# ChenWu98/cycle-diffusion

Hardware: AMD Instinct MI355X
Metric: images/sec, SD-v1.4 512px CycleDiffusion 100+100 steps, 1/2/4/8 MI355X (higher is better)
Workload: dtype fp16; 1 GPU; C2: Stable-Diffusion-v1.4-shaped U-Net + KL-f8 VAE, 512x512, custom_steps=99 white_box_steps=100 eta=0.1 skip 0, 1 trial, encoder scale 1, decoder CFG 3; batch_per_gpu=4, global_batch=4, parallelism=dp1, steps_per_launch_set=5, launch_set_cap=16, launch_sets_in_flight_per_gpu=1, images_in_flight_per_gpu=20, distributed=single process, weights=synthetic(seed=0)

## Files before the change

cycle-diffusion_amd/_ffi.py:

```python
import ctypes as C
import os

import numpy as np

_HERE = os.path.dirname(os.path.abspath(__file__))
LIB_PATH = os.path.join(_HERE, "lib", "libcyclediff.so")

CD_NET_UNET_OPENAI, CD_NET_UNET_HO, CD_NET_VAE_KL, CD_NET_CLIP_TEXT, CD_NET_BERT_XTR = 1, 2, 3, 4, 5
CD_NET_OCLIP_TEXT, CD_NET_OCLIP_VISION, CD_NET_INCEPTION_FID = 6, 7, 8
CD_SCHED_DDIM, CD_SCHED_DDPM = 0, 1
CD_PREC_16, CD_PREC_F32, CD_PREC_F32X3 = 0, 1, 2
CD_MASK_QSAMPLE, CD_MASK_ENCODER = 0, 1
MASK_SOURCES = {"q_sample": CD_MASK_QSAMPLE, "encoder": CD_MASK_ENCODER}
ACT_NONE, ACT_SILU, ACT_GELU, ACT_GEGLU, ACT_QGELU, ACT_RELU = 0, 1, 2, 3, 4, 5


class NetDesc(C.Structure):
    _fields_ = [
        ("kind", C.c_int), ("image_size", C.c_int), ("in_channels", C.c_int), ("out_channels", C.c_int),
        ("model_channels", C.c_int), ("num_res_blocks", C.c_int),
        ("n_mult", C.c_int), ("channel_mult", C.c_int * 8),
        ("n_attn", C.c_int), ("attn", C.c_int * 8),
        ("num_heads", C.c_int), ("num_head_channels", C.c_int),
        ("use_spatial_transformer", C.c_int), ("context_dim", C.c_int), ("transformer_depth", C.c_int),
        ("use_scale_shift_norm", C.c_int), ("resblock_updown", C.c_int), ("conv_resample", C.c_int),
        ("z_channels", C.c_int), ("embed_dim", C.c_int), ("double_z", C.c_int),
        ("precision", C.c_int), ("n_embed", C.c_int), ("reserved", C.c_int * 6),
    ]


class StepCoef(C.Structure):
    _fields_ = [("sa", C.c_float), ("s1a", C.c_float), ("sap", C.c_float), ("dirc", C.c_float),
                ("sigma", C.c_float), ("r", C.c_float), ("t_mask", C.c_float), ("t", C.c_int32)]


STEP_COEF_DTYPE = np.dtype([("sa", "<f4"), ("s1a", "<f4"), ("sap", "<f4"), ("dirc", "<f4"), ("sigma", "<f4"),
                            ("r", "<f4"), ("t_mask", "<f4"), ("t", "<i4")])

_VP, _I, _F, _U64, _SZ, _I64 = C.c_void_p, C.c_int, C.c_float, C.c_uint64, C.c_size_t, C.c_int64

SIGNATURES = {
    "cd_last_error": [],
    "cd_version": [],
    "cd_act_format": [],
    "cd_engine_create": [_VP, _SZ, C.POINTER(_VP)],
    "cd_engine_destroy": [_VP],
    "cd_engine_synchronize": [_VP],
    "cd_engine_workspace_high_water": [_VP, C.POINTER(_SZ)],
    "cd_prof_enable": [_VP, _I],
    "cd_prof_collect": [_VP, C.POINTER(_I), C.POINTER(C.c_double), C.POINTER(C.c_double)],
    "cd_net_create": [_VP, C.POINTER(NetDesc), C.POINTER(_I)],
    "cd_net_param_count": [_VP, _I, C.POINTER(_I)],
    "cd_net_param_info": [_VP, _I, _I, C.c_char_p, _I, C.POINTER(_I), C.POINTER(_I64)],
    "cd_net_load_param": [_VP, _I, C.c_char_p, _VP, _I, C.POINTER(_I64)],
    "cd_net_missing_params": [_VP, _I, C.POINTER(_I), C.c_char_p, _I],
    "cd_unet_forward": [_VP, _I, _VP, _VP, _VP, _I, _I, _VP],
    "cd_text_encode": [_VP, _I, _VP, _I, _I, _VP],
    "cd_clip_text_features": [_VP, _I, _VP, _I, _I, _VP],
    "cd_clip_image_features": [_VP, _I, _VP, _I, _VP],
    "cd_inception_features": [_VP, _I, _VP, _I, _I, _VP],
    "cd_vae_encode": [_VP, _I, _VP, _VP, _U64, _I, _I, _I, _F, _VP],
    "cd_vae_decode": [_VP, _I, _VP, _I, _I, _F, _F, _F, _VP],
    "cd_dpm_encode": [_VP, _I, _I, _VP, _VP, _VP, _I, _F, _I, _I, _VP, _VP, _U64, _I, _VP],
    "cd_ddim_decode": [_VP, _I, _I, _VP, _I, _I, _VP, _VP, _I, _F, _I, _I, _VP, _VP, _U64, _VP],
    "cd_ddim_decode_v": [_VP, _I, _I, _VP, _I, _I, _VP, _VP, _I, _VP, _I, _I, _VP, _VP, _U64, _VP],
    "cd_ddim_invert": [_VP, _I, _I, _VP, _VP, _VP, _I, _F, _I, _I, _VP, _VP, _VP],
    "cd_cycle_translate": [_VP, _I, _I, _VP, _VP, _VP, _F, _VP, _VP, _F, _VP, _I, _I, _I, _I, _VP, _VP, _VP, _U64, _I, _VP,
                           _VP],
    "cd_ddim_decode_masked": [_VP, _I, _I, _VP, _I, _I, _VP, _VP, _I, _F, _VP, _I, _I, _VP, _VP, _U64, _VP, _VP, _I, _I, _VP, _VP,
                              _U64, _VP],
    "cd_cycle_translate_masked": [_VP, _I, _I, _VP, _VP, _VP, _F, _VP, _VP, _F, _VP, _I, _I, _I, _I, _VP, _VP, _VP, _U64, _I,
                                  _VP, _VP, _I, _I, _VP, _VP, _U64, _VP, _VP],
    "cd_cycle_translate_ctrl": [_VP, _I, _I, _VP, _VP, _VP, _F, _VP, _VP, _F, _VP, _I, _I, _I, _I, _VP, _VP, _VP, _U64, _I,
                                _VP, _VP, _I, _I, _VP, _VP, _U64, _VP, _VP, _VP, _I, _I, _VP, _VP],
    "cd_ilvr_decode": [_VP, _I, _I, _VP, _I, _I, _I, _I, _VP, _VP, _U64, _VP, _I, _I, _I, _VP, _VP, _U64, _VP],
    "cd_pix_refine": [_VP, _I, _I, _VP, _I, _I, _VP, _VP, _U64],
    "cd_op_pack_conv_weight": [_VP, _VP, _I, _I, _I, _I, _I, C.POINTER(_VP), C.POINTER(_I), C.POINTER(_I)],
    "cd_op_free": [_VP, _VP],
    "cd_op_conv2d": [_VP, _VP, _I, _VP, _I, _I, _I, _I, _VP, _I, _I, _I, _I, _I, _I, _I, _VP, _VP, _VP, _I, _I, _VP],
    "cd_op_conv2d_16": [_VP, _VP, _I, _VP, _I, _I, _I, _I, _VP, _I, _I, _I, _I, _I, _I, _I, _VP, _VP, _VP, _I, _I, _VP,
                        _VP],
    "cd_op_last_gemm_config": [_VP] + [C.POINTER(_I)] * 5,
    "cd_op_up_phase_reorder": [_VP, _VP, _I, _I, _I, _I, _VP],
    "cd_op_groupnorm": [_VP, _VP, _I, _I, _I, _I, _I, _F, _VP, _VP, _VP, _I, _VP],
    "cd_op_groupnorm_ex": [_VP, _VP, _I, _I, _VP, _I, _I, _I, _I, _I, _F, _VP, _VP, _VP, _I, _I, _VP, _VP, _I, _VP],
    "cd_op_pack_conv_weight_prec": [_VP, _VP, _I, _I, _I, _I, _I, C.POINTER(_VP)],
    "cd_op_conv2d_prec": [_VP, _VP, _I, _I, _VP, _I, _I, _I, _I, _I, _VP, _I, _I, _I, _I, _I, _I, _I, _VP, _VP, _I, _VP, _I, _I,
                          _I, _I, _I, _I, _F, _VP, _VP],
    "cd_op_attention_prec": [_VP, _VP, _VP, _VP, _I, _I, _I, _I, _I, _I, _I, _I, _F, _I, _VP, _I, _I, _VP],
    "cd_op_rows_prec": [_VP, _I, _VP, _I64, _I, _I, _VP, _I, _I, _VP, _VP, _I, _VP],
    "cd_op_resample_prec": [_VP, _I, _VP, _I, _I, _I, _I, _I, _VP],
    "cd_op_layernorm": [_VP, _VP, _I, _I, _VP, _VP, _F, _VP],
    "cd_op_attention": [_VP, _VP, _VP, _VP, _I, _I, _I, _I, _I, _F, _I, _VP],
    "cd_op_cross_attention_ctrl": [_VP, _VP, _VP, _VP, _VP, _VP, _VP, _VP, _VP, _I, _I, _I, _I, _I, _I, _I, _I, _F, _VP],
    "cd_op_lowpass": [_VP, _VP, _I, _I, _I, _I, _VP],
    "cd_op_softmax_rows": [_VP, _VP, _I64, _I, _VP],
    "cd_op_timestep_embedding": [_VP, _VP, _I, _I, _I, _VP],
    "cd_op_sched_step": [_VP, _I, _I, _VP, _VP, _VP, _VP, _I, _F, _VP, _VP, _I, _I, _I, _I, _VP],
    "cd_op_sched_step_masked": [_VP, _I, _VP, _VP, _VP, _I, _F, _VP, _VP, _VP, _I, _I, _F, _F, _VP, _I, _I, _I, _I, _VP, _I],
    "cd_op_bench_conv": [_VP, _I, _I, _I, _I, _I, _I, _I, _I, _I, _I, _I, _I, C.POINTER(C.c_float)],
    "cd_op_bench_mfma_sustained": [_VP, _I, C.POINTER(C.c_float), C.POINTER(C.c_float)],
    "cd_op_probe": [_VP, _I, _VP, _VP, _SZ],
}
_RESTYPES = {"cd_last_error": C.c_char_p}

_lib = None


class EngineError(RuntimeError):
    pass


def load_library(build_if_missing=True):
    global _lib
    if _lib is not None:
        return _lib
    if not os.path.exists(LIB_PATH):
        if not build_if_missing:
            raise EngineError("libcyclediff.so has not been built: run `python -c 'import __graft_entry__ as g; g.build()'`")
        import importlib.util
        spec = importlib.util.spec_from_file_location("_cd_build", os.path.join(_HERE, "build.py"))
        mod = importlib.util.module_from_spec(spec)
        spec.loader.exec_module(mod)
        mod.build()
    os.environ.setdefault("CYCLEDIFF_TUNE_DEFAULT", os.path.join(_HERE, "tune_gfx950.txt"))
    lib = C.CDLL(os.environ.get("CYCLEDIFF_LIB") or LIB_PATH)
    for name, args in SIGNATURES.items():
        fn = getattr(lib, name)
        fn.argtypes = args
        fn.restype = _RESTYPES.get(name, C.c_int)
    _lib = lib
    return lib


def check(rc):
    if rc != 0:
        raise EngineError(load_library().cd_last_error().decode("utf-8", "replace"))


def ptr(t):
    if t is None:
        return None
    if not t.is_contiguous():
        raise EngineError("tensor crossing the C ABI must be contiguous")
    return C.c_void_p(t.data_ptr())


def coef_array(rows):
    arr = np.zeros(len(rows), dtype=STEP_COEF_DTYPE)
    for i, r in enumerate(rows):
        arr[i] = tuple(r)
    return arr
```

cycle-diffusion_amd/csrc/capi.hip:

```cpp
#include <stdlib.h>
#include <string.h>
#include <unistd.h>

#include <algorithm>

#include "engine.h"

using namespace cd;

struct StepPacer {
  static constexpr int kAhead = 2, kRing = kAhead + 1;
  hipEvent_t ev[kRing] = {nullptr, nullptr, nullptr};
  long n = 0;
  bool enabled = true;
  void init() {
    const char* e = getenv("CYCLEDIFF_HOST_PACING");
    enabled = !(e && e[0] == '0');
    for (auto& x : ev) HIP_CHECK(hipEventCreateWithFlags(&x, hipEventBlockingSync | hipEventDisableTiming));
  }
  static void sleep_until_done(hipEvent_t e) {
    for (;;) {
      const hipError_t q = hipEventQuery(e);
      if (q == hipSuccess) return;
      if (q != hipErrorNotReady) HIP_CHECK(q);
// ... 1021 lines not shown
    ConvW* pw = (ConvW*)const_cast<void*>(packed_w);
    h->op_params.add_up_phase(pw);
    h->op_params.refresh_up_phase(h->st, pw);
  }
  ConvW w = *(const ConvW*)packed_w;
  CD_CHECK(w.N == N && w.KH == KH && w.KW == KW, "packed weight does not match the call");
  w.b = const_cast<float*>(bias);
  const int c0p = x1 ? C0 : round_up(C0, 32);
  Act a0 = alloc_act(c, B, H, W, c0p);
  launch_nchw_to_nhwc(h->st, x0, a0.p, B, C0, H * W, c0p, 1.f, 0.f, 0);
  Act a1;
  if (x1) {
    a1 = alloc_act(c, B, H, W, C1);
    launch_nchw_to_nhwc(h->st, x1, a1.p, B, C1, H * W, C1, 1.f, 0.f, 0);
  }
  ConvOpts o; o.stride = stride; o.pad = pad; o.asym = asym_pad != 0; o.up = up != 0; o.tile = tile;
  if (act & 0x400) {
    CD_CHECK(out16 && conv_ln_fold_available(c, w, (int64_t)B * H * W) , "LayerNorm fold needs tile 30 shapes");
    o.ln_fold = true;
    act &= ~0x400;
  }
  o.act = act;
  o.out_f32 = !out16;
  o.want_stats = stats != nullptr;
  const int Hin = up ? 2 * H : H, Win = up ? 2 * W : W;
  const int Ho = asym_pad ? (Hin + 1 - KH) / stride + 1 : (Hin + 2 * pad - KH) / stride + 1;
  const int Wo = asym_pad ? (Win + 1 - KW) / stride + 1 : (Win + 2 * pad - KW) / stride + 1;
  const int Nout = w.geglu ? N / 2 : N;
  if (rowvec) { o.rowvec = rowvec; o.rowvec_ld = N; o.rows_per_vec = Ho * Wo; }
  Act r;
  if (resid) {
    r = alloc_act(c, B, Ho, Wo, Nout);
    launch_nchw_to_nhwc(h->st, resid, r.p, B, Nout, Ho * Wo, Nout, 1.f, 0.f, 0);
    o.resid = &r;
  }
  Act out = conv_fwd(c, w, a0, x1 ? &a1 : nullptr, o);
  launch_nhwc_to_nchw(h->st, out.p, out16 ? 0 : 1, out.ld, y, B, Nout, Ho * Wo, 1.f, 0.f);
  if (stats) {
    CD_CHECK(out.stats, "this convolution produces no GroupNorm statistics (GEGLU, or rows %% 32 != 0)");
    HIP_CHECK(hipMemcpyAsync(stats, out.stats, (size_t)(out.rows() / 32) * 2 * Nout * sizeof(float),
                             hipMemcpyDeviceToDevice, h->st));
  }
}

int cd_op_conv2d(cd_handle h, const float* x0, int C0, const float* x1, int C1, int B, int H, int W,
                 const void* packed_w, int N, int KH, int KW, int stride, int pad, int asym_pad, int up,
                 const float* bias, const float* rowvec, const float* resid, int act, int tile, float* y) {
  CD_API_BEGIN
  enter_engine(h);
  op_conv2d(h, x0, C0, x1, C1, B, H, W, packed_w, N, KH, KW, stride, pad, asym_pad, up, bias, rowvec, resid, act, tile,
            false, y, nullptr);
  CD_API_END
}

int cd_op_conv2d_16(cd_handle h, const float* x0, int C0, const float* x1, int C1, int B, int H, int W,
                    const void* packed_w, int N, int KH, int KW, int stride, int pad, int asym_pad, int up,
                    const float* bias, const float* rowvec, const float* resid, int act, int tile, float* y,
                    float* stats) {
  CD_API_BEGIN
  enter_engine(h);
  op_conv2d(h, x0, C0, x1, C1, B, H, W, packed_w, N, KH, KW, stride, pad, asym_pad, up, bias, rowvec, resid, act, tile,
            true, y, stats);
  CD_API_END
}

int cd_op_up_phase_reorder(cd_handle h, const float* x, int B, int C, int H, int W, float* y) {
  CD_API_BEGIN
  enter_engine(h);
  CD_CHECK(h && x && y && B > 0 && H > 0 && W > 0 && C > 0 && C % 8 == 0, "bad argument");
  ArenaScope arena_scope(h->arena);
  Ctx c = h->ctx();
  Act a = alloc_act(c, 4 * B, H, W, C);
  launch_nchw_to_nhwc(h->st, x, a.p, 4 * B, C, H * W, C, 1.f, 0.f, 0);
  Act o = alloc_act(c, B, 2 * H, 2 * W, C);
  launch_up_phase_reorder(h->st, a.p, o.p, B, H, W, C, o.ld);
  launch_nhwc_to_nchw(h->st, o.p, 0, o.ld, y, B, C, 4 * H * W, 1.f, 0.f);
  CD_API_END
}

int cd_op_last_gemm_config(cd_handle h, int* tile_id, int* bk, int* splitk, int* chm, int* tile_group) {
  CD_API_BEGIN
  CD_CHECK(h, "bad argument");
  const GemmLaunchInfo li = conv_gemm_last_launch();
  if (tile_id) *tile_id = li.tile_id;
  if (bk) *bk = li.bk;
  if (splitk) *splitk = li.splitk;
  if (chm) *chm = li.chm;
  if (tile_group) *tile_group = li.tile_group;
  CD_API_END
}

int cd_op_groupnorm(cd_handle h, const float* x, int B, int C, int H, int W, int G, float eps,
                    const float* gamma, const float* beta, const float* film, int silu, float* y) {
  CD_API_BEGIN
  enter_engine(h);
  CD_CHECK(h && x && y && G == 32, "bad argument (G must be 32)");
  ArenaScope arena_scope(h->arena);
  Ctx c = h->ctx();
  Act a = alloc_act(c, B, H, W, C);
  launch_nchw_to_nhwc(h->st, x, a.p, B, C, H * W, C, 1.f, 0.f, 0);
  GNW w; w.g = const_cast<float*>(gamma); w.b = const_cast<float*>(beta); w.C = C; w.eps = eps;
  Act o = groupnorm_fwd(c, w, a, nullptr, silu != 0, film, film ? 2 * C : 0);
  launch_nhwc_to_nchw(h->st, o.p, 0, o.ld, y, B, C, H * W, 1.f, 0.f);
  CD_API_END
}

int cd_op_groupnorm_ex(cd_handle h, const float* x0, int C0, int pad0, const float* x1, int C1, int pad1, int B, int H,
                       int W, float eps, const float* gamma, const float* beta, const float* film, int film_ld, int silu,
                       const float* stats0, const float* stats1, int precision, void* y) {
  CD_API_BEGIN
  enter_engine(h);
  CD_CHECK(h && x0 && gamma && beta && y && B > 0 && H > 0 && W > 0 && C0 > 0 && pad0 >= 0 && pad1 >= 0, "bad argument");
  CD_CHECK(x1 ? C1 > 0 : (C1 == 0 && !stats1), "bad argument (second source)");
  CD_CHECK(precision >= 0 && precision <= 2 && film_ld >= 0, "bad argument (precision 0 = 16-bit, 1 = fp32, 2 = fp32 split)");
  const int align = precision ? 4 : 8;
  CD_CHECK((C0 + pad0) % align == 0 && (C1 + pad1) % align == 0, "row strides must be multiples of %d elements", align);
  ArenaScope arena_scope(h->arena);
  Ctx c = h->ctx();
  c.f32 = precision != 0; c.x3 = precision == 2;
  const int HW = H * W, C = C0 + C1;
  auto upload = [&](const float* x, int Cs, int pad, const float* stats) {
    Act a; a.B = B; a.H = H; a.W = W; a.C = Cs; a.ld = Cs + pad; a.f32 = c.f32;
    a.p = (bf16_t*)h->arena.alloc((size_t)B * HW * a.ld * (c.f32 ? sizeof(float) : sizeof(bf16_t)));
    const float* src = x;
    if (pad) {
      const size_t n = (size_t)B * a.ld * HW;
      float* t = (float*)h->arena.alloc(n * sizeof(float));
      launch_fill_f32(h->st, t, __builtin_nanf(""), (int64_t)n);
      HIP_CHECK(hipMemcpy2DAsync(t, (size_t)a.ld * HW * 4, x, (size_t)Cs * HW * 4, (size_t)Cs * HW * 4, B,
                                 hipMemcpyDeviceToDevice, h->st));
      src = t;
    }
    if (c.f32) launch_nchw_to_nhwc_f32(h->st, src, a.pf(), B, a.ld, HW, a.ld, 1.f, 0.f);
    else launch_nchw_to_nhwc(h->st, src, a.p, B, a.ld, HW, a.ld, 1.f, 0.f, 0);
    a.stats = const_cast<float*>(stats);
    return a;
  };
  Act a0 = upload(x0, C0, pad0, stats0);
  Act a1;
  if (x1) a1 = upload(x1, C1, pad1, stats1);
  GNW w; w.g = const_cast<float*>(gamma); w.b = const_cast<float*>(beta); w.C = C; w.eps = eps;
  Act o = groupnorm_fwd(c, w, a0, x1 ? &a1 : nullptr, silu != 0, film, film_ld);
  if (precision == 2) {
    CD_CHECK(o.split && o.ld == 2 * C, "groupnorm: split output expected");
    HIP_CHECK(hipMemcpyAsync(y, o.p, (size_t)B * HW * 2 * C * sizeof(bf16_t), hipMemcpyDeviceToDevice, h->st));
    HIP_CHECK(hipStreamSynchronize(h->st));
    h->check_overflow();
  } else {
    launch_nhwc_to_nchw(h->st, o.p, c.f32 ? 1 : 0, o.ld, (float*)y, B, C, HW, 1.f, 0.f);
  }
  CD_API_END
}

int cd_op_layernorm(cd_handle h, const float* x, int rows, int C, const float* gamma, const float* beta,
                    float eps, float* y) {
  CD_API_BEGIN
  enter_engine(h);
  CD_CHECK(h && x && y, "bad argument");
  ArenaScope arena_scope(h->arena);
  bf16_t* a = (bf16_t*)h->arena.alloc((size_t)rows * C * 2);
  bf16_t* o = (bf16_t*)h->arena.alloc((size_t)rows * C * 2);
  launch_nchw_to_nhwc(h->st, x, a, rows, C, 1, C, 1.f, 0.f, 0);
  launch_layernorm(h->st, a, C, o, C, rows, C, gamma, beta, eps);
  launch_nhwc_to_nchw(h->st, o, 0, C, y, rows, C, 1, 1.f, 0.f);
  CD_API_END
}

int cd_op_attention(cd_handle h, const float* q, const float* k, const float* v, int B, int H, int Tq,
                    int Tk, int D, float scale, int use_transpose_kernel, float* o) {
  CD_API_BEGIN
  enter_engine(h);
  CD_CHECK(h && q && k && v && o, "bad argument");
  ArenaScope arena_scope(h->arena);
  const int C = H * D, Tpad = round_up(Tk, 64);
  bf16_t* qb = (bf16_t*)h->arena.alloc((size_t)B * Tq * C * 2);
  bf16_t* kb = (bf16_t*)h->arena.alloc((size_t)B * Tk * C * 2);
  bf16_t* vb = (bf16_t*)h->arena.alloc((size_t)B * Tk * C * 2);
  bf16_t* ob = (bf16_t*)h->arena.alloc((size_t)B * Tq * C * 2);
  launch_nchw_to_nhwc(h->st, q, qb, B * Tq, C, 1, C, 1.f, 0.f, 0);
  launch_nchw_to_nhwc(h->st, k, kb, B * Tk, C, 1, C, 1.f, 0.f, 0);
  launch_nchw_to_nhwc(h->st, v, vb, B * Tk, C, 1, C, 1.f, 0.f, 0);
  AttnParams p;
  p.q = qb; p.k = kb; p.o = ob; p.B = B; p.H = H; p.Tq = Tq; p.Tk = Tk; p.D = D;
  p.ldq = C; p.ldk = C; p.ldo = C; p.q_bs = (int64_t)Tq * C; p.k_bs = (int64_t)Tk * C; p.o_bs = (int64_t)Tq * C;
  p.scale = scale;
  if (use_transpose_kernel) {
    bf16_t* vt = (bf16_t*)h->arena.alloc((size_t)B * C * Tpad * 2);
    launch_transpose_v(h->st, vb, C, (int64_t)Tk * C, vt, B, H, Tk, D, D, Tpad);
    p.vt = vt; p.vt_dpad = D; p.vt_tpad = Tpad;
  } else {
    p.v = vb; p.ldv = C; p.v_bs = (int64_t)Tk * C;
  }
  launch_attention(h->st, p);
  launch_nhwc_to_nchw(h->st, ob, 0, C, o, B * Tq, C, 1, 1.f, 0.f);
  CD_API_END
}

int cd_op_cross_attention_ctrl(cd_handle h, const float* q_own, const float* q_src, const float* k_own, const float* k_src,
                               const float* v_own, const float* mapper, const float* alpha, const float* weight, int B,
                               int B_src, int B_ctrl, int H, int Tq, int L, int L_buf, int D, float scale, float* o) {
  CD_API_BEGIN
  enter_engine(h);
  CD_CHECK(h && q_own && q_src && k_own && k_src && v_own && mapper && alpha && weight && o, "bad argument");
  CD_CHECK(B > 0 && B_src > 0 && B_ctrl > 0 && H > 0 && Tq > 0 && D > 0 && L > 0 && L_buf >= L, "bad argument");
  ArenaScope arena_scope(h->arena);
  const int C = H * D;
  auto to16 = [&](const float* src, int64_t rows) {
    bf16_t* d = (bf16_t*)h->arena.alloc((size_t)rows * C * 2);
    launch_nchw_to_nhwc(h->st, src, d, (int)rows, C, 1, C, 1.f, 0.f, 0);
    return d;
  };
  CtrlAttnParams p;
  p.q_own = to16(q_own, (int64_t)B * Tq); p.q_src = to16(q_src, (int64_t)B_src * Tq);
  p.k_own = to16(k_own, (int64_t)B * L_buf); p.k_src = to16(k_src, (int64_t)B_src * L_buf);
  const bf16_t* vb16 = to16(v_own, (int64_t)B * L);
  bf16_t* va = (bf16_t*)h->arena.alloc((size_t)B * L * C * 2);
  bf16_t* vb = (bf16_t*)h->arena.alloc((size_t)B * L * C * 2);
  launch_ctrl_values(h->st, vb16, mapper, alpha, weight, B, B_ctrl, L, C, va, vb);
  bf16_t* ob = (bf16_t*)h->arena.alloc((size_t)B * Tq * C * 2);
  p.va = va; p.vb = vb; p.o = ob;
  p.B = B; p.B_src = B_src; p.H = H; p.Tq = Tq; p.L = L; p.D = D;
  p.ldq = C; p.ldk = C; p.ldv = C; p.ldo = C;
  p.q_bs = (int64_t)Tq * C; p.k_bs = (int64_t)L_buf * C; p.v_bs = (int64_t)L * C; p.o_bs = (int64_t)Tq * C;
  p.scale = scale;
  launch_cross_attention_ctrl(h->st, p);
  launch_nhwc_to_nchw(h->st, ob, 0, C, o, B * Tq, C, 1, 1.f, 0.f);
  CD_API_END
}

int cd_op_lowpass(cd_handle h, const float* x, int B, int C, int R, int down_n, float* y) {
  CD_API_BEGIN
  enter_engine(h);
  CD_CHECK(h && x && y && B > 0 && C > 0 && R > 0, "bad argument");
  check_lowpass_geometry(R, down_n);
  ArenaScope arena_scope(h->arena);
  const int r = R / down_n;
  IlvrArgs iv;
  iv.out = y; iv.y = x; iv.y_bmod = B;
  iv.B = B; iv.C = C; iv.R = R;
  iv.D = upload_taps(h, R, r);
  iv.U = upload_taps(h, r, R);
  iv.T = (float*)h->arena.alloc((size_t)B * C * r * r * sizeof(float));
  iv.vec4 = (R % 4 == 0 && aligned16(x) && aligned16(y)) ? 1 : 0;
  launch_ilvr_down(h->st, iv);
  launch_ilvr_up_add(h->st, iv);
  HIP_CHECK(hipStreamSynchronize(h->st));
  CD_API_END
}

int cd_op_softmax_rows(cd_handle h, const float* s, int64_t rows, int cols, float* p) {
  CD_API_BEGIN
  enter_engine(h);
  CD_CHECK(h && s && p, "bad argument");
  ArenaScope arena_scope(h->arena);
  bf16_t* pb = (bf16_t*)h->arena.alloc((size_t)rows * cols * 2);
  launch_softmax_rows(h->st, s, cols, pb, cols, rows, cols);
  launch_nhwc_to_nchw(h->st, pb, 0, cols, p, (int)rows, cols, 1, 1.f, 0.f);
  CD_API_END
}

int cd_op_timestep_embedding(cd_handle h, const float* t, int B, int dim, int mode, float* out) {
  CD_API_BEGIN
  enter_engine(h);
  CD_CHECK(h && t && out, "bad argument");
  launch_timestep_embedding(h->st, nullptr, 0, t, out, B, dim, mode);
  CD_API_END
}

int cd_op_sched_step(cd_handle h, int mode, int sched_kind, const cd_step_coef* coef_host, const float* x0,
                     float* xt, const float* eps_hat, int cfg, float guidance, const float* noise,
                     const float* eps_in, int is_last, int B, int C, int HW, float* z_slot) {
  CD_API_BEGIN
  enter_engine(h);
  CD_CHECK(h && coef_host && xt, "bad argument");
  ArenaScope arena_scope(h->arena);
  const int64_t chw = (int64_t)C * HW;
  StepArgs a;
  a.x0 = x0; a.xt = xt;
  a.eh.p = eps_hat; a.eh.sb = chw; a.eh.sc = HW; a.eh.sp = 1; a.eh.cfg = cfg; a.eh.g = guidance;
  a.geom.B = B; a.geom.C = C; a.geom.HW = HW; a.geom.tab = upload_coef(h, coef_host, 1);
  a.gauss.noise = noise;
  a.eps.p = eps_in; a.eps.bstride = chw;
  a.z.p = z_slot; a.z.bstride = chw;
  a.is_last = is_last;
  if (mode == 0) launch_init_xt(h->st, a);
  else if (mode == 1) launch_encode_step(h->st, sched_kind, a);
  else launch_decode_step(h->st, sched_kind, a);
  HIP_CHECK(hipStreamSynchronize(h->st));
  CD_API_END
}

int cd_op_sched_step_masked(cd_handle h, int mode, const cd_step_coef* coef_host, float* x, const float* eps_hat, int cfg,
                            float guidance, const float* eps_in, const float* mask, const float* src, int B_mask,
                            int mask_source, float qa, float qb, const float* mask_noise, int blend, int B, int C, int HW,
                            void* xin16_out, int cfg_dup) {
  CD_API_BEGIN
  enter_engine(h);
  CD_CHECK(h && x && mask && src && B > 0 && C > 0 && HW > 0, "bad argument");
  CD_CHECK(B_mask > 0 && B % B_mask == 0, "mask shape mismatch: %d mask rows for a batch of %d", B_mask, B);
  CD_CHECK(mode == 0 || (coef_host && eps_hat), "bad argument");
  ArenaScope arena_scope(h->arena);
  const int64_t chw = (int64_t)C * HW;
  MaskBlend mk;
  mk.mask = mask; mk.src = src; mk.mask_bmod = mk.src_bmod = B_mask; mk.gauss.noise = mask_noise;
  if (mask_source == CD_MASK_QSAMPLE) {
    CD_CHECK(mask_noise, "q_sample mode needs the noise tensor here");
// ... 412 lines not shown
```

cycle-diffusion_amd/csrc/engine.h:

```cpp
#pragma once
#include <map>
#include <memory>
#include <string>
#include <vector>

#include "common.h"
#include "kernels.h"
#include "../../include/cyclediff.h"

namespace cd {

class Arena {
 public:
  ~Arena();
  void init(size_t bytes);
  void* alloc(size_t bytes);
  size_t mark() const { return off_; }
  void release(size_t m) { off_ = m; }
  void reset() { off_ = 0; }
  size_t capacity() const { return cap_; }
  size_t high_water() const { return high_; }
 private:
  char* base_ = nullptr;
  size_t cap_ = 0, off_ = 0, high_ = 0;
};

struct Act {
  bf16_t* p = nullptr;
  int B = 0, H = 0, W = 0, C = 0;
  int ld = 0;
  bool f32 = false;
  bool split = false;
  float* pf() const { return (float*)p; }
  float* stats = nullptr;
  float* stats_buf = nullptr;
  int64_t rows() const { return (int64_t)B * H * W; }
};

struct ConvW {
  bf16_t* w = nullptr;
  bf16_t* wfrag = nullptr;
  bf16_t* w3 = nullptr;
  bf16_t* wphase = nullptr;
  int wphase_version = -1;
  bool f32 = false;
  float* b = nullptr;
  int N = 0, Cin = 0, Cpad = 0, KH = 1, KW = 1, Npad = 0;
  bool geglu = false;
  int Ktot() const { return KH * KW * Cpad; }
};

struct PackTarget {
  enum Kind { MATRIX_BF16, VECTOR_F32, MATRIX_F32 } kind;
  ConvW* conv = nullptr;
  int dst_row0 = 0, rows = 0, src_base = 0, grp = 0, grp_stride = 0;
  float* fdst = nullptr;
  int dst_off = 0, K = 1;
  bool geglu = false;
  int geglu_N = 0;
  float scale = 1.f;
};

struct ParamDecl {
  std::string name;
  std::vector<int64_t> shape;
  std::vector<PackTarget> targets;
  bool loaded = false;
  bool transposed = false;
};

class ParamStore {
 public:
  ~ParamStore();
  bool f32 = false;
  bool x3 = false;
  int* overflow = nullptr;
  int version = 0;
  ConvW* new_conv(int N, int Cin, int KH, int KW, bool bias, bool geglu = false);
  float* new_vec(int n, float init = 0.f);
  void add_up_phase(ConvW* c);
  void refresh_up_phase(hipStream_t st, ConvW* c);
  ParamDecl& declare(const std::string& name, std::vector<int64_t> shape);
  void conv_weight(const std::string& name, ConvW* c, int ref_ndim = 0, float scale = 1.f);
  void conv_weight_t(const std::string& name, ConvW* c);
  void conv_bias(const std::string& name, ConvW* c);
  void conv_rows(const std::string& name, std::vector<int64_t> shape, ConvW* c, int dst_row0, int rows,
                 int src_base, int grp, int grp_stride, float scale = 1.f);
  void bias_rows(const std::string& name, int64_t n_total, float* dst, int dst_off, int rows, int src_base,
                 int grp, int grp_stride);
  void vec(const std::string& name, float* dst, int n);
  void mat_f32(const std::string& name, float* dst, int N, int K, int dst_row0 = 0);

  void load(hipStream_t st, const std::string& name, const float* host, int ndim, const int64_t* shape);
  int missing(std::string* first = nullptr) const;
  const std::vector<std::unique_ptr<ParamDecl>>& decls() const { return decls_; }
  size_t device_bytes() const { return dev_bytes_; }
 private:
  std::vector<std::unique_ptr<ParamDecl>> decls_;
  std::map<std::string, ParamDecl*> by_name_;
  std::vector<std::unique_ptr<ConvW>> convs_;
  std::vector<void*> allocs_;
  float* staging_ = nullptr;
  size_t staging_bytes_ = 0;
  size_t dev_bytes_ = 0;
  void* dmalloc(size_t bytes);
};

struct Ctx {
  hipStream_t st = nullptr;
  Arena* arena = nullptr;
  const bf16_t* zeros = nullptr;
  float* gn_partial = nullptr;
  size_t gn_partial_floats = 0;
  bool f32 = false;
  bool x3 = false;
  int* overflow = nullptr;
};

struct ConvOpts {
  int stride = 1;
  int pad = 1;
  bool asym = false;
  bool up = false;
  const float* rowvec = nullptr; int rowvec_ld = 0; int rows_per_vec = 1;
  const Act* resid = nullptr;
  int act = ACT_NONE;
  float alpha = 1.f;
  bool out_f32 = false;
  void* out = nullptr;
  int out_ld = 0;
  bool ln_fold = false;
  float ln_eps = 1e-5f;
  bool raw_geglu = false;
  bool want_stats = false;
  float* out_stats = nullptr;
  int tile = 0;
};
Act attention_flash_f32_fwd(Ctx& c, const float* q, int ldq, const float* k, int ldk, int64_t k_bs, const float* v, int ldv,
                            int64_t v_bs, int B, int H, int Tq, int Tk, int D, float scale, int Himg, int Wimg, bool q_log2);
Act geglu_f32_fwd(Ctx& c, const Act& h);
Act split_rows_f32_fwd(Ctx& c, const Act& x, const Act* x2 = nullptr);
Act alloc_act(Ctx& c, int B, int H, int W, int C, bool with_stats = false);
Act conv_fwd(Ctx& c, const ConvW& w, const Act& x, const Act* x2, const ConvOpts& o);
bool conv_up_phase_taken(const Ctx& c, const ConvW& w, const Act& x, const Act* x2, const ConvOpts& o);
bool conv_ln_fold_available(const Ctx& c, const ConvW& w, int64_t rows);

struct GNW { float* g = nullptr; float* b = nullptr; int C = 0; float eps = 1e-5f; };
Act groupnorm_fwd(Ctx& c, const GNW& w, const Act& x, const Act* x2, bool silu, const float* film = nullptr,
                  int film_ld = 0);
struct LNW { float* g = nullptr; float* b = nullptr; int C = 0; };
Act layernorm_fwd(Ctx& c, const LNW& w, const Act& x);

Act avgpool2_fwd(Ctx& c, const Act& x);
Act upsample2_fwd(Ctx& c, const Act& x);
Act attention_f32_fwd(Ctx& c, const Act& qk, const Act& v, int H, int D, float scale, const float* obias);

Act attention_fwd(Ctx& c, const bf16_t* q, int ldq, const bf16_t* k, int ldk, const bf16_t* v, int ldv, int B,
                  int H, int Tq, int Tk, int D, float scale, int Himg, int Wimg, bool q_log2 = false);
Act attention_vt_fwd(Ctx& c, const bf16_t* q, int ldq, const bf16_t* k, int ldk, const bf16_t* vt, int B,
                     int H, int Tq, int Tk, int Tpad, int D, float scale, int Himg, int Wimg, bool q_log2 = false);

class Net {
 public:
  virtual ~Net() {}
  ParamStore params;
  cd_net_desc desc;
  bool f32 = false;
  bool x3 = false;
  virtual int kind() const = 0;
};

struct TimeEmb {
  int mode = 0, dim = 0, hidden = 0;
  float *w0 = nullptr, *b0 = nullptr, *w1 = nullptr, *b1 = nullptr;
  float* proj_w = nullptr; float* proj_b = nullptr;
  int proj_total = 0;
};

struct AttnCtrl {
  std::vector<const bf16_t*> va, vb;
  int row0 = 0, rows = 0;
  int src_b0 = 0, B_src = 0;
};

struct UNetIO {
  const bf16_t* xin = nullptr;
  int B = 0;
  const StepCoef* tab = nullptr; int step = 0;
  const float* t_explicit = nullptr;
  bool t_shared = true;
  bool cfg_dup = false;
  int dup_tail = 0;
  const AttnCtrl* ctrl = nullptr;
  float* out = nullptr;
  int out_ld = 0;
};

class UNet : public Net {
 public:
  virtual void forward(Ctx& c, const UNetIO& io) = 0;
  virtual void set_context(Ctx& c, const bf16_t* ctx, int B, int L) { (void)c; (void)ctx; (void)B; (void)L; }
  virtual void build_attn_control(Ctx&, const float*, const float*, const float*, int, AttnCtrl&) {
    CD_CHECK(false, "cross-attention control: the network has no text cross-attention");
  }
  int in_cpad = 32;
  int out_channels = 0;
  int image_size = 0;
  virtual size_t workspace_hint(int B) const = 0;
};

std::unique_ptr<UNet> make_unet_openai(const cd_net_desc& d);
std::unique_ptr<UNet> make_unet_ho(const cd_net_desc& d);

class VAE : public Net {
 public:
  int kind() const override { return CD_NET_VAE_KL; }
  virtual void encode_moments(Ctx& c, const bf16_t* img_nhwc, int B, int R, float* moments) = 0;
  virtual void decode(Ctx& c, const bf16_t* z_nhwc, int B, int h, float* img) = 0;
  int z_channels = 4, factor = 8;
  int moments_channels = 8;
  const float* codebook = nullptr;
  int n_embed = 0;
};
std::unique_ptr<VAE> make_vae_kl(const cd_net_desc& d);

class TextEncoder : public Net {
 public:
  virtual void encode(Ctx& c, const int* ids_dev, int B, int L, float* out) = 0;
  virtual void text_features(Ctx&, const int*, int, int, float*) { CD_CHECK(false, "net has no pooled text features"); }
  virtual void image_features(Ctx&, const float*, int, float*) { CD_CHECK(false, "net has no image tower"); }
  virtual int width() const = 0;
  virtual int max_positions() const = 0;
};
std::unique_ptr<TextEncoder> make_clip_text(const cd_net_desc& d);

std::unique_ptr<Net> make_inception_fid(const cd_net_desc& d);
void inception_fid_features(Net* n, Ctx& c, const float* img, int B, int stop_block, float* out);

}
```

cycle-diffusion_amd/csrc/engine.hip:

```cpp
#include <stdlib.h>

#include "engine.h"

#include <string.h>

namespace cd {

Arena::~Arena() { if (base_) (void)hipFree(base_); }
void Arena::init(size_t bytes) {
  if (base_) { (void)hipFree(base_); base_ = nullptr; }
  HIP_CHECK(hipMalloc((void**)&base_, bytes));
  cap_ = bytes; off_ = 0; high_ = 0;
}
void* Arena::alloc(size_t bytes) {
  size_t a = (off_ + 255) & ~(size_t)255;
  CD_CHECK(a + bytes <= cap_, "workspace arena exhausted: need %zu more bytes (capacity %zu); "
           "create the engine with a larger workspace", a + bytes - cap_, cap_);
  off_ = a + bytes;
  if (off_ > high_) high_ = off_;
  return base_ + a;
}

ParamStore::~ParamStore() {
  for (void* p : allocs_) (void)hipFree(p);
  if (staging_) (void)hipFree(staging_);
}
void* ParamStore::dmalloc(size_t bytes) {
  void* p = nullptr;
  HIP_CHECK(hipMalloc(&p, bytes < 256 ? 256 : bytes));
  HIP_CHECK(hipMemset(p, 0, bytes < 256 ? 256 : bytes));
  allocs_.push_back(p);
  dev_bytes_ += bytes;
  return p;
}
ConvW* ParamStore::new_conv(int N, int Cin, int KH, int KW, bool bias, bool geglu) {
  convs_.emplace_back(new ConvW());
  ConvW* c = convs_.back().get();
  c->N = N; c->Cin = Cin; c->KH = KH; c->KW = KW; c->geglu = geglu;
  c->Cpad = round_up(Cin, 32);
  c->Npad = round_up(N, 128);
  c->f32 = f32;
  c->w = (bf16_t*)dmalloc((size_t)c->Npad * c->Ktot() * (f32 ? sizeof(float) : sizeof(bf16_t)));
  if (!f32 && KH == 1 && KW == 1 && c->Cpad == 320)
    c->wfrag = (bf16_t*)dmalloc((size_t)c->Npad * c->Cpad * sizeof(bf16_t));
  if (f32 && x3) c->w3 = (bf16_t*)dmalloc((size_t)c->Npad * c->Ktot() * 3 * sizeof(bf16_t));
  if (bias) c->b = (float*)dmalloc((size_t)c->Npad * sizeof(float));
  return c;
}
void ParamStore::add_up_phase(ConvW* c) {
  if (f32 || c->wphase || c->KH != 3 || c->KW != 3 || c->geglu) return;
  c->wphase = (bf16_t*)dmalloc((size_t)4 * c->Npad * 4 * c->Cpad * sizeof(bf16_t));
  c->wphase_version = -1;
}
void ParamStore::refresh_up_phase(hipStream_t st, ConvW* c) {
  if (!c->wphase || c->wphase_version == version) return;
  launch_up_phase_weights(st, c->w, c->wphase, c->Npad, c->Cpad);
  c->wphase_version = version;
}
float* ParamStore::new_vec(int n, float init) {
  float* p = (float*)dmalloc((size_t)n * sizeof(float));
  if (init != 0.f) {
    std::vector<float> h(n, init);
    HIP_CHECK(hipMemcpy(p, h.data(), (size_t)n * sizeof(float), hipMemcpyHostToDevice));
  }
  return p;
}
ParamDecl& ParamStore::declare(const std::string& name, std::vector<int64_t> shape) {
  auto it = by_name_.find(name);
  if (it != by_name_.end()) {
    CD_CHECK(it->second->shape == shape, "parameter %s declared twice with different shapes", name.c_str());
    return *it->second;
  }
  decls_.emplace_back(new ParamDecl());
  ParamDecl* d = decls_.back().get();
  d->name = name; d->shape = std::move(shape);
  by_name_[name] = d;
  return *d;
}
void ParamStore::conv_weight(const std::string& name, ConvW* c, int ref_ndim, float scale) {
  std::vector<int64_t> shape;
  if (ref_ndim == 0) ref_ndim = (c->KH == 1 && c->KW == 1) ? 2 : 4;
  if (ref_ndim == 2) shape = {c->N, c->Cin};
  else if (ref_ndim == 3) shape = {c->N, c->Cin, 1};
  else shape = {c->N, c->Cin, c->KH, c->KW};
  ParamDecl& d = declare(name, shape);
  PackTarget t; t.kind = PackTarget::MATRIX_BF16; t.conv = c; t.dst_row0 = 0; t.rows = c->N;
  t.src_base = 0; t.grp = c->N; t.grp_stride = 0; t.geglu = c->geglu; t.scale = scale;
  d.targets.push_back(t);
}
void ParamStore::conv_weight_t(const std::string& name, ConvW* c) {
  CD_CHECK(c->KH == 1 && c->KW == 1, "transposed weights are linear layers");
  ParamDecl& d = declare(name, {c->Cin, c->N});
  d.transposed = true;
  PackTarget t; t.kind = PackTarget::MATRIX_BF16; t.conv = c; t.dst_row0 = 0; t.rows = c->N;
  t.src_base = 0; t.grp = c->N; t.grp_stride = 0; t.geglu = false;
  d.targets.push_back(t);
}
void ParamStore::conv_bias(const std::string& name, ConvW* c) {
  CD_CHECK(c->b, "conv %s has no bias storage", name.c_str());
  ParamDecl& d = declare(name, {c->N});
  PackTarget t; t.kind = PackTarget::VECTOR_F32; t.fdst = c->b; t.dst_off = 0; t.rows = c->N;
  t.src_base = 0; t.grp = c->N; t.grp_stride = 0; t.geglu = c->geglu; t.geglu_N = c->N;
  d.targets.push_back(t);
}
void ParamStore::conv_rows(const std::string& name, std::vector<int64_t> shape, ConvW* c, int dst_row0,
                           int rows, int src_base, int grp, int grp_stride, float scale) {
  ParamDecl& d = declare(name, std::move(shape));
  PackTarget t; t.kind = PackTarget::MATRIX_BF16; t.conv = c; t.dst_row0 = dst_row0; t.rows = rows;
  t.src_base = src_base; t.grp = grp; t.grp_stride = grp_stride; t.scale = scale;
  d.targets.push_back(t);
}
void ParamStore::bias_rows(const std::string& name, int64_t n_total, float* dst, int dst_off, int rows,
                           int src_base, int grp, int grp_stride) {
  ParamDecl& d = declare(name, {n_total});
  PackTarget t; t.kind = PackTarget::VECTOR_F32; t.fdst = dst; t.dst_off = dst_off; t.rows = rows;
  t.src_base = src_base; t.grp = grp; t.grp_stride = grp_stride;
  d.targets.push_back(t);
}
void ParamStore::vec(const std::string& name, float* dst, int n) {
  bias_rows(name, n, dst, 0, n, 0, n, 0);
}
void ParamStore::mat_f32(const std::string& name, float* dst, int N, int K, int dst_row0) {
  ParamDecl& d = declare(name, {N, K});
  PackTarget t; t.kind = PackTarget::MATRIX_F32; t.fdst = dst; t.dst_off = dst_row0; t.rows = N; t.K = K;
  t.src_base = 0; t.grp = N; t.grp_stride = 0;
  d.targets.push_back(t);
}

template <typename OutT>
__global__ void k_pack_rows(const float* __restrict__ w, OutT* __restrict__ out, int rows, int Cin,
                            int KH, int KW, int Cpad, int dst_row0, int src_base, int grp,
                            int grp_stride, int geglu, int Ntot, float scale) {
  const int64_t total = (int64_t)rows * KH * KW * Cpad;
  for (int64_t i = blockIdx.x * (int64_t)blockDim.x + threadIdx.x; i < total;
       i += (int64_t)gridDim.x * blockDim.x) {
    const int c = (int)(i % Cpad);
    int64_t t = i / Cpad;
    const int s = (int)(t % KW); t /= KW;
    const int r = (int)(t % KH); t /= KH;
    const int j = (int)t;
    int jj = j;
    if (geglu) {
      const int blk = j / 64, within = j % 64;
      jj = (within < 32) ? blk * 32 + within : Ntot / 2 + blk * 32 + (within - 32);
    }
    const int src = src_base + (jj / grp) * grp_stride + (jj % grp);
    float v = 0.f;
    if (c < Cin) v = w[(((int64_t)src * Cin + c) * KH + r) * KW + s] * scale;
    const int64_t o = ((int64_t)(dst_row0 + j) * KH * KW + (int64_t)r * KW + s) * Cpad + c;
    if constexpr (sizeof(OutT) == 4) out[o] = v;
    else out[o] = f2bf(v);
  }
}
// ... 9 lines not shown
  for (auto s : d.shape) nd *= s;
  bool ok = (n == nd) && ndim >= 1 && shape[0] == d.shape[0];
  if (ok && d.shape.size() >= 2 && ndim >= 2) ok = (shape[1] == d.shape[1]);
  CD_CHECK(ok, "parameter %s: shape mismatch (got %lld elements, ndim %d; expected %lld)", name.c_str(),
           (long long)n, ndim, (long long)nd);
  const size_t bytes = (size_t)n * sizeof(float);
  if (bytes > staging_bytes_) {
    if (staging_) HIP_CHECK(hipFree(staging_));
    staging_bytes_ = bytes < (1u << 20) ? (1u << 20) : bytes;
    HIP_CHECK(hipMalloc((void**)&staging_, staging_bytes_));
  }
  HIP_CHECK(hipStreamSynchronize(st));
  if (d.transposed) {
    const int64_t K = d.shape[0], N = d.shape[1];
    std::vector<float> tr((size_t)n);
    for (int64_t k = 0; k < K; ++k)
      for (int64_t j = 0; j < N; ++j) tr[(size_t)j * K + k] = host[(size_t)k * N + j];
    HIP_CHECK(hipMemcpy(staging_, tr.data(), bytes, hipMemcpyHostToDevice));
  } else {
    HIP_CHECK(hipMemcpy(staging_, host, bytes, hipMemcpyHostToDevice));
  }
  for (const PackTarget& t : d.targets) {
    if (t.kind == PackTarget::MATRIX_BF16) {
      const ConvW* c = t.conv;
      const int64_t total = (int64_t)t.rows * c->KH * c->KW * c->Cpad;
      int grid = (int)((total + 255) / 256);
      if (grid > 8192) grid = 8192;
      if (c->f32)
        hipLaunchKernelGGL(k_pack_rows<float>, dim3(grid), dim3(256), 0, st, staging_, (float*)c->w, t.rows, c->Cin,
                           c->KH, c->KW, c->Cpad, t.dst_row0, t.src_base, t.grp, t.grp_stride, t.geglu ? 1 : 0, c->N,
                           t.scale);
      else
        hipLaunchKernelGGL(k_pack_rows<bf16_t>, dim3(grid), dim3(256), 0, st, staging_, c->w, t.rows, c->Cin, c->KH,
                           c->KW, c->Cpad, t.dst_row0, t.src_base, t.grp, t.grp_stride, t.geglu ? 1 : 0, c->N, t.scale);
      if (c->wfrag) launch_pack_wfrag(st, c->w, c->Ktot(), c->wfrag, c->Npad);
      if (c->w3) launch_pack_w3(st, (const float*)c->w, c->w3, c->Npad, c->KH * c->KW, c->Cpad, overflow);
    } else {
      const int K = (t.kind == PackTarget::MATRIX_F32) ? t.K : 1;
      std::vector<float> tmp((size_t)t.rows * K);
      for (int j = 0; j < t.rows; ++j) {
        int jj = j;
        if (t.geglu) {
          const int blk = j / 64, within = j % 64;
          jj = (within < 32) ? blk * 32 + within : t.geglu_N / 2 + blk * 32 + (within - 32);
        }
        const int src = t.src_base + (jj / t.grp) * t.grp_stride + (jj % t.grp);
        memcpy(&tmp[(size_t)j * K], host + (size_t)src * K, (size_t)K * sizeof(float));
      }
      HIP_CHECK(hipMemcpy(t.fdst + (size_t)t.dst_off * K, tmp.data(), tmp.size() * sizeof(float),
                          hipMemcpyHostToDevice));
    }
  }
  HIP_CHECK(hipStreamSynchronize(st));
  d.loaded = true;
}

int ParamStore::missing(std::string* first) const {
  int n = 0;
  for (auto& d : decls_)
    if (!d->loaded) {
      if (n == 0 && first) *first = d->name;
      ++n;
    }
  return n;
}

Act alloc_act(Ctx& c, int B, int H, int W, int C, bool with_stats) {
  Act a; a.B = B; a.H = H; a.W = W; a.C = C; a.ld = C; a.f32 = c.f32;
  a.p = (bf16_t*)c.arena->alloc((size_t)B * H * W * C * (c.f32 ? sizeof(float) : sizeof(bf16_t)));
  if ((!c.f32 || c.x3) && with_stats && ((H * W) % 32) == 0)
    a.stats_buf = (float*)c.arena->alloc((size_t)(B * H * W / 32) * 2 * C * sizeof(float));
  return a;
}

static Act conv_split_fwd(Ctx& c, const ConvW& w, const Act& x, const ConvOpts& o) {
  CD_CHECK(c.f32 && c.x3 && w.w3 && (!w.geglu || o.raw_geglu), "conv: split input outside the split-fp16 mode");
  CD_CHECK(x.C == w.Cpad && x.ld == 2 * x.C, "conv: split input of %d channels (ld %d) against Cpad %d", x.C, x.ld, w.Cpad);
  CD_CHECK(!o.ln_fold && (!o.resid || (o.resid->f32 && !o.resid->split)), "conv: split-mode operands");
  ConvGemmParams p;
  p.src0 = x.p; p.C0 = 2 * x.C; p.ld0 = x.ld;
  p.src1 = x.p; p.C1 = x.C; p.ld1 = x.ld;
  p.B = x.B; p.Hs = x.H; p.Ws = x.W; p.up = o.up ? 1 : 0;
  p.Hin = o.up ? x.H * 2 : x.H; p.Win = o.up ? x.W * 2 : x.W;
  p.KH = w.KH; p.KW = w.KW; p.stride = o.stride;
  if (o.asym) { p.pad_t = 0; p.pad_l = 0; p.Hout = (p.Hin + 1 - w.KH) / o.stride + 1; p.Wout = (p.Win + 1 - w.KW) / o.stride + 1; }
  else {
    p.pad_t = o.pad; p.pad_l = o.pad;
    p.Hout = (p.Hin + 2 * o.pad - w.KH) / o.stride + 1;
    p.Wout = (p.Win + 2 * o.pad - w.KW) / o.stride + 1;
  }
  p.M = x.B * p.Hout * p.Wout;
  p.wgt = w.w3; p.Ktot = 3 * w.Ktot(); p.N = w.N;
  p.alpha = o.alpha * (1.0f / (kX3ActScale * kX3WgtScale)); p.bias = w.b;
  p.rowvec = o.rowvec; p.rowvec_ld = o.rowvec_ld; p.rows_per_vec = o.rows_per_vec;
  p.act = o.act;
  Act y; y.B = x.B; y.H = p.Hout; y.W = p.Wout; y.C = w.N; y.f32 = true;
  if (o.out) { y.p = (bf16_t*)o.out; y.ld = o.out_ld; }
  else { y.ld = w.N; y.p = (bf16_t*)c.arena->alloc((size_t)p.M * w.N * 4); }
  if (o.resid) {
    CD_CHECK(o.resid->rows() == p.M && o.resid->C == w.N, "conv: residual shape mismatch");
    p.resid = o.resid->p; p.resid_ld = o.resid->ld; p.resid_f32 = 1;
  }
  p.out = y.p; p.out_ld = y.ld; p.out_f32 = 1;
  p.zeros = c.zeros; p.tile = o.tile;
  p.prof_flop_scale = 1.0f / 3.0f;
  if (((p.Hout * p.Wout) % 32) == 0) {
    if (o.out && o.out_stats) y.stats_buf = o.out_stats;
    else if (!o.out && o.want_stats)
      y.stats_buf = (float*)c.arena->alloc((size_t)(p.M / 32) * 2 * w.N * sizeof(float));
    p.stats = y.stats_buf;
    y.stats = y.stats_buf;
  }
  launch_conv_gemm(c.st, p);
  return y;
}

bool conv_up_phase_taken(const Ctx& c, const ConvW& w, const Act& x, const Act* x2, const ConvOpts& o) {
  if (!o.up || c.f32 || x.split || x2 || !w.wphase || w.KH != 3 || w.KW != 3 || o.stride != 1 || o.pad != 1 || o.asym ||
      o.resid || o.out_f32 || o.ln_fold || w.geglu || o.act != ACT_NONE)
    return false;
  if ((x.H * x.W) % 256 != 0 || w.N % 8 != 0 || (o.out && o.out_ld % 8 != 0)) return false;
  const char* e = getenv("CYCLEDIFF_UP_PHASE");
  return !(e && e[0] == '0');
}

static Act conv_up_phase_fwd(Ctx& c, const ConvW& w, const Act& x, const ConvOpts& o) {
  ConvGemmParams p;
  p.src0 = x.p; p.C0 = round_up(x.C, 32); p.ld0 = x.ld;
  CD_CHECK(p.C0 == w.Cpad && x.ld >= p.C0, "conv: input channels %d do not match weight Cpad %d", p.C0, w.Cpad);
  p.B = x.B; p.Hs = x.H; p.Ws = x.W; p.Hin = x.H; p.Win = x.W; p.Hout = x.H; p.Wout = x.W;
  p.KH = 2; p.KW = 2; p.stride = 1; p.pad_t = 1; p.pad_l = 1;
  p.up_phase = 1; p.w_ps = w.Npad * 4 * w.Cpad;
  p.M = 4 * x.B * x.H * x.W;
  p.wgt = w.wphase; p.Ktot = 4 * w.Cpad; p.N = w.N;
  p.alpha = o.alpha; p.bias = w.b;
  p.rowvec = o.rowvec; p.rowvec_ld = o.rowvec_ld; p.rows_per_vec = o.rows_per_vec;
  Act y; y.B = x.B; y.H = 2 * x.H; y.W = 2 * x.W; y.C = w.N; y.f32 = false;
  if (o.out) { y.p = (bf16_t*)o.out; y.ld = o.out_ld; }
  else { y.ld = w.N; y.p = (bf16_t*)c.arena->alloc((size_t)p.M * w.N * 2); }
  if (o.out && o.out_stats) y.stats_buf = o.out_stats;
  else if (!o.out && o.want_stats) y.stats_buf = (float*)c.arena->alloc((size_t)(p.M / 32) * 2 * w.N * sizeof(float));
  p.stats = y.stats_buf;
  y.stats = y.stats_buf;
  const size_t mk = c.arena->mark();
  bf16_t* tmp = (bf16_t*)c.arena->alloc((size_t)p.M * w.N * 2);
  p.out = tmp; p.out_ld = w.N;
  p.zeros = c.zeros; p.tile = o.tile;
  launch_conv_gemm(c.st, p);
  launch_up_phase_reorder(c.st, tmp, y.p, x.B, x.H, x.W, w.N, y.ld);
  c.arena->release(mk);
  return y;
}

Act conv_fwd(Ctx& c, const ConvW& w, const Act& x, const Act* x2, const ConvOpts& o) {
  if (conv_up_phase_taken(c, w, x, x2, o)) return conv_up_phase_fwd(c, w, x, o);
  if (x.split) {
    CD_CHECK(!x2, "conv: a split activation cannot be concatenated");
    return conv_split_fwd(c, w, x, o);
  }
  ConvGemmParams p;
  CD_CHECK(w.f32 == c.f32 && x.f32 == c.f32 && (!x2 || x2->f32 == c.f32) && (!o.resid || o.resid->f32 == c.f32),
           "conv: operand precision does not match the running network");
  CD_CHECK((!x2 || !x2->split) && (!o.resid || !o.resid->split), "conv: split activation as a second source / residual");
  p.src0 = x.p; p.C0 = round_up(x.C, 32); p.ld0 = x.ld;
  if (x2) {
    CD_CHECK(x2->B == x.B && x2->H == x.H && x2->W == x.W, "conv: concat sources differ in shape");
    p.src1 = x2->p; p.C1 = x2->C; p.ld1 = x2->ld;
    CD_CHECK(x.C % 32 == 0 && x2->C % 32 == 0, "conv: concat channels must be multiples of 32");
  }
  CD_CHECK(p.C0 + p.C1 == w.Cpad, "conv: input channels %d+%d do not match weight Cpad %d", p.C0, p.C1, w.Cpad);
  CD_CHECK(x.ld >= p.C0, "conv: source row shorter than padded channel count");
  p.B = x.B; p.Hs = x.H; p.Ws = x.W; p.up = o.up ? 1 : 0;
  p.Hin = o.up ? x.H * 2 : x.H; p.Win = o.up ? x.W * 2 : x.W;
  p.KH = w.KH; p.KW = w.KW; p.stride = o.stride;
  if (o.asym) { p.pad_t = 0; p.pad_l = 0; p.Hout = (p.Hin + 1 - w.KH) / o.stride + 1; p.Wout = (p.Win + 1 - w.KW) / o.stride + 1; }
  else {
    p.pad_t = o.pad; p.pad_l = o.pad;
    p.Hout = (p.Hin + 2 * o.pad - w.KH) / o.stride + 1;
    p.Wout = (p.Win + 2 * o.pad - w.KW) / o.stride + 1;
  }
  p.M = x.B * p.Hout * p.Wout;
  p.wgt = w.w; p.wgt_frag = w.wfrag; p.Ktot = w.Ktot(); p.N = w.N;
  p.alpha = o.alpha; p.bias = w.b;
  p.rowvec = o.rowvec; p.rowvec_ld = o.rowvec_ld; p.rows_per_vec = o.rows_per_vec;
  const bool fuse_geglu = w.geglu && !o.raw_geglu;
  p.act = fuse_geglu ? ACT_GEGLU : o.act;
  const int Nout = fuse_geglu ? w.N / 2 : w.N;
  Act y; y.B = x.B; y.H = p.Hout; y.W = p.Wout; y.C = Nout; y.f32 = c.f32;
  if (o.out) { y.p = (bf16_t*)o.out; y.ld = o.out_ld; }
  else {
    y.ld = Nout;
    y.p = (bf16_t*)c.arena->alloc((size_t)p.M * Nout * ((o.out_f32 || c.f32) ? 4 : 2));
  }
  if (o.resid) {
    CD_CHECK(o.resid->rows() == p.M && o.resid->C == Nout, "conv: residual shape mismatch");
    p.resid = o.resid->p; p.resid_ld = o.resid->ld;
  }
  p.out = y.p; p.out_ld = y.ld; p.out_f32 = o.out_f32 ? 1 : 0;
  p.zeros = c.zeros; p.tile = o.tile;
  if (o.ln_fold) { p.ln_fold = 1; p.ln_eps = o.ln_eps; p.tile = kLinStreamTile; }
  if (c.f32) {
    p.out_f32 = 1;
    launch_conv_gemm_f32(c.st, p);
    return y;
  }
  if (!w.geglu && !o.out_f32 && ((p.Hout * p.Wout) % 32) == 0) {
    if (o.out && o.out_stats) y.stats_buf = o.out_stats;
    else if (!o.out && o.want_stats)
      y.stats_buf = (float*)c.arena->alloc((size_t)(p.M / 32) * 2 * Nout * sizeof(float));
    p.stats = y.stats_buf;
    y.stats = y.stats_buf;
  }
  launch_conv_gemm(c.st, p);
  return y;
}

bool conv_ln_fold_available(const Ctx& c, const ConvW& w, int64_t rows) {
  static const bool on = [] { const char* e = getenv("CYCLEDIFF_LN_FOLD"); return !(e && e[0] == '0'); }();
  static const int64_t min_rows = [] { const char* e = getenv("CYCLEDIFF_LN_FOLD_MIN_ROWS"); return e ? atoll(e) : 32768ll; }();
  return on && !c.f32 && w.wfrag && w.KH == 1 && w.KW == 1 && w.Cpad == 320 && rows >= min_rows && rows % 32 == 0 &&
         w.N % 64 == 0 && w.N <= 2560;
}

Act groupnorm_fwd(Ctx& c, const GNW& w, const Act& x, const Act* x2, bool silu, const float* film,
                  int film_ld) {
  GroupNormParams p;
  p.x = x.p; p.C0 = x.C; p.ld0 = x.ld;
  if (x2) { p.x1 = x2->p; p.C1 = x2->C; p.ld1 = x2->ld; }
  const int C = p.C0 + p.C1;
  CD_CHECK(C == w.C, "groupnorm: channels %d != weight %d", C, w.C);
  p.B = x.B; p.HW = x.H * x.W; p.G = 32; p.eps = w.eps; p.gamma = w.g; p.beta = w.b;
  p.film = film; p.film_ld = film_ld; p.silu = silu ? 1 : 0;
  Act y = alloc_act(c, x.B, x.H, x.W, C);
  p.y = y.p;
  if (c.f32) {
    CD_CHECK(x.f32 && (!x2 || x2->f32) && !x.split && (!x2 || !x2->split), "groupnorm: operand precision");
    if (c.x3) { p.split_out = 1; p.overflow = c.overflow; y.split = true; y.ld = 2 * C; }
    if (x.stats && x.ld == x.C && (!x2 || (x2->stats && x2->ld == x2->C))) {
      p.pre0 = x.stats;
      p.pre1 = x2 ? x2->stats : nullptr;
    }
    const size_t mk = c.arena->mark();
    void* ws = c.arena->alloc(groupnorm_f32_workspace(p.B, p.HW, C));
    launch_groupnorm_f32(c.st, p, ws);
    c.arena->release(mk);
    return y;
  }
  p.S = groupnorm_slabs(p.B, p.HW, C);
  const size_t part_floats = round_up((size_t)p.B * p.S * p.G * 2, (size_t)64);
  CD_CHECK(part_floats + (size_t)p.B * 2 * C <= c.gn_partial_floats, "groupnorm: workspace too small");
  p.partial = c.gn_partial;
  p.coef = c.gn_partial + part_floats;
  if (x.stats && x.ld == x.C && (!x2 || (x2->stats && x2->ld == x2->C))) {
    p.pre0 = x.stats;
    p.pre1 = x2 ? x2->stats : nullptr;
  }
  launch_groupnorm(c.st, p);
  return y;
}

Act avgpool2_fwd(Ctx& c, const Act& x) {
  if (x.split) {
    Act y = alloc_act(c, x.B, x.H / 2, x.W / 2, x.C);
    y.split = true; y.ld = 2 * x.C;
    launch_avgpool2_split(c.st, x.p, y.p, x.B, x.H, x.W, x.C, c.overflow);
    return y;
  }
  CD_CHECK(x.ld == x.C, "avgpool: dense input expected");
  Act y = alloc_act(c, x.B, x.H / 2, x.W / 2, x.C);
  if (c.f32) launch_avgpool2_f32(c.st, x.pf(), y.pf(), x.B, x.H, x.W, x.C);
  else launch_avgpool2(c.st, x.p, y.p, x.B, x.H, x.W, x.C);
  return y;
}
Act upsample2_fwd(Ctx& c, const Act& x) {
  CD_CHECK(x.ld == x.C && !x.split, "upsample: dense input expected");
  Act y = alloc_act(c, x.B, x.H * 2, x.W * 2, x.C);
  if (c.f32) launch_upsample2_f32(c.st, x.pf(), y.pf(), x.B, x.H, x.W, x.C);
  else launch_upsample2(c.st, x.p, y.p, x.B, x.H, x.W, x.C);
  return y;
}
Act attention_f32_fwd(Ctx& c, const Act& qk, const Act& v, int H, int D, float scale, const float* obias) {
  CD_CHECK(c.f32 && qk.f32 && v.f32 && !qk.split && !v.split && qk.C == 2 * H * D && v.C == H * D,
           "attention_f32: operands");
  Act o = alloc_act(c, qk.B, qk.H, qk.W, H * D);
  const int T = qk.H * qk.W;
  if (D <= 160 && (D % 4) == 0 && (qk.ld % 4) == 0 && (v.ld % 4) == 0) {
    launch_flash_f32(c.st, qk.pf(), qk.ld, (int64_t)T * qk.ld, qk.pf() + H * D, qk.ld, (int64_t)T * qk.ld, v.pf(), v.ld,
                     (int64_t)T * v.ld, o.pf(), o.ld, (int64_t)T * o.ld, qk.B, H, T, T, D, scale * 1.44269504088896340736f, 0,
                     c.overflow, obias);
    return o;
  }
  launch_attention_f32(c.st, qk.pf(), qk.ld, qk.pf() + H * D, qk.ld, v.pf(), v.ld, o.pf(), o.ld, qk.B, H, T, D, scale, obias);
  return o;
}

Act layernorm_fwd(Ctx& c, const LNW& w, const Act& x) {
  CD_CHECK(x.C == w.C, "layernorm: channels");
  if (c.f32) {
    CD_CHECK(x.f32 && !x.split, "layernorm_f32: operand precision");
    Act y = alloc_act(c, x.B, x.H, x.W, x.C);
    if (c.x3) { y.split = true; y.ld = 2 * x.C; }
    launch_layernorm_f32(c.st, x.pf(), x.ld, y.pf(), x.rows(), x.C, w.g, w.b, 1e-5f, c.x3 ? 1 : 0, c.overflow);
    return y;
  }
  Act y = alloc_act(c, x.B, x.H, x.W, x.C);
  launch_layernorm(c.st, x.p, x.ld, y.p, y.ld, (int)x.rows(), x.C, w.g, w.b, 1e-5f);
  return y;
}

Act attention_fwd(Ctx& c, const bf16_t* q, int ldq, const bf16_t* k, int ldk, const bf16_t* v, int ldv, int B,
                  int H, int Tq, int Tk, int D, float scale, int Himg, int Wimg, bool q_log2) {
  CD_CHECK(!c.f32, "attention: 16-bit kernel called on the fp32 path");
  Act o = alloc_act(c, B, Himg, Wimg, H * D);
  AttnParams p;
  p.q = q; p.k = k; p.v = v; p.o = o.p;
  p.B = B; p.H = H; p.Tq = Tq; p.Tk = Tk; p.D = D;
  p.ldq = ldq; p.ldk = ldk; p.ldv = ldv; p.ldo = o.ld;
  p.q_bs = (int64_t)Tq * ldq; p.k_bs = (int64_t)Tk * ldk; p.v_bs = (int64_t)Tk * ldv; p.o_bs = (int64_t)Tq * o.ld;
  p.scale = scale; p.q_log2 = q_log2 ? 1 : 0;
  launch_attention(c.st, p);
  return o;
}

Act attention_vt_fwd(Ctx& c, const bf16_t* q, int ldq, const bf16_t* k, int ldk, const bf16_t* vt, int B,
                     int H, int Tq, int Tk, int Tpad, int D, float scale, int Himg, int Wimg, bool q_log2) {
  CD_CHECK(!c.f32, "attention: 16-bit kernel called on the fp32 path");
  Act o = alloc_act(c, B, Himg, Wimg, H * D);
  AttnParams p;
  p.q = q; p.k = k; p.vt = vt; p.o = o.p;
  p.B = B; p.H = H; p.Tq = Tq; p.Tk = Tk; p.D = D;
  p.ldq = ldq; p.ldk = ldk; p.ldo = o.ld;
  p.q_bs = (int64_t)Tq * ldq; p.k_bs = (int64_t)Tk * ldk; p.o_bs = (int64_t)Tq * o.ld;
  p.vt_dpad = D; p.vt_tpad = Tpad;
  p.scale = scale; p.q_log2 = q_log2 ? 1 : 0;
  launch_attention(c.st, p);
  return o;
}

Act attention_flash_f32_fwd(Ctx& c, const float* q, int ldq, const float* k, int ldk, int64_t k_bs, const float* v, int ldv,
                            int64_t v_bs, int B, int H, int Tq, int Tk, int D, float scale, int Himg, int Wimg, bool q_log2) {
  CD_CHECK(c.f32, "attention_flash_f32: fp32 path only");
  Act o = alloc_act(c, B, Himg, Wimg, H * D);
  launch_flash_f32(c.st, q, ldq, (int64_t)Tq * ldq, k, ldk, k_bs, v, ldv, v_bs, o.pf(), o.ld, (int64_t)Tq * o.ld, B, H, Tq,
                   Tk, D, q_log2 ? 1.0f : scale * 1.44269504088896340736f, c.x3 ? 1 : 0, c.overflow);
  if (c.x3) { o.split = true; o.ld = 2 * o.C; }
  return o;
}

Act geglu_f32_fwd(Ctx& c, const Act& h) {
  CD_CHECK(c.f32 && h.f32 && !h.split && h.ld == h.C && (h.C % 64) == 0, "geglu_f32: operand");
  Act y = alloc_act(c, h.B, h.H, h.W, h.C / 2);
  launch_geglu_f32(c.st, h.pf(), y.pf(), h.rows(), h.C / 2, c.x3 ? 1 : 0, c.overflow);
  if (c.x3) { y.split = true; y.ld = 2 * y.C; }
  return y;
}

Act split_rows_f32_fwd(Ctx& c, const Act& x, const Act* x2) {
  CD_CHECK(c.f32 && c.x3 && x.f32 && !x.split && (!x2 || (x2->f32 && !x2->split && x2->rows() == x.rows())),
           "split_rows_f32: operand");
  const int C = x.C + (x2 ? x2->C : 0);
  Act y = alloc_act(c, x.B, x.H, x.W, C);
  launch_split_rows_f32(c.st, x.pf(), x.ld, x.C, x2 ? x2->pf() : nullptr, x2 ? x2->ld : 4, x2 ? x2->C : 0, y.p, x.rows(),
                        c.overflow);
  y.split = true; y.ld = 2 * C;
  return y;
}

}
```

cycle-diffusion_amd/csrc/kernels.h:

```cpp
#pragma once
#include <map>
#include <string>
#include <vector>

#include "common.h"

namespace cd {

struct StepCoef {
  float sa, s1a, sap, dirc, sigma, r, t_mask;
  int t;
};
enum { SCHED_DDIM = 0, SCHED_DDPM = 1 };

struct EpsHat {
  const float* p = nullptr;
  int64_t sb = 0, sc = 0, sp = 0;
  int cfg = 0;
  float g = 1.f;
  const float* gvec = nullptr;
};

struct StepGeom {
  int B = 0, C = 0, HW = 0;
  const StepCoef* tab = nullptr;
  int step = 0;
};
struct GaussSrc {
  const float* noise = nullptr;
  uint64_t seed = 0;
  uint32_t stream = 0;
};
struct XinOut {
  bf16_t* xin = nullptr;
  int cpad = 0;
  int dup = 0;
};
struct EpsIn {
  const float* p = nullptr;
  int64_t bstride = 0;
  int bmod = 0;
};
struct ZSlot {
  float* p = nullptr;
  int64_t bstride = 0;
};
struct StepArgs {
  const float* x0 = nullptr;
  float* xt = nullptr;
  EpsHat eh;
  StepGeom geom;
  GaussSrc gauss;
  XinOut xin;
  EpsIn eps;
  ZSlot z;
  int is_last = 0;
};

struct MaskBlend {
  const float* mask = nullptr;
  const float* src = nullptr;
  int mask_bmod = 1, src_bmod = 1;
  const float2* qtab = nullptr;
  int qrow = 0;
  GaussSrc gauss;
};

void launch_init_xt(hipStream_t st, const StepArgs& a);
void launch_encode_step(hipStream_t st, int kind, const StepArgs& a);
void launch_decode_step(hipStream_t st, int kind, const StepArgs& a, const MaskBlend* mk = nullptr, bool blend = false);
void launch_mask_blend_init(hipStream_t st, const StepArgs& a, const MaskBlend& mk);

struct LowpassTaps {
  const float* w = nullptr;
  const int* first = nullptr;
  int n_out = 0, n_in = 0, P = 0;
};
struct IlvrArgs {
  const float* xp = nullptr;
  float* out = nullptr;
  const float* y = nullptr;
  int y_bmod = 1;
  const float2* qtab = nullptr;
  int qrow = 0;
  GaussSrc gauss;
  float* T = nullptr;
  int B = 0, C = 0, R = 0;
  LowpassTaps D, U;
  XinOut xin;
  int vec4 = 0;
};
constexpr int kIlvrMaxR = 1024;
void build_lowpass_taps(int n_in, int n_out, std::vector<float>& w, std::vector<int>& first, int& P);
void launch_ilvr_down(hipStream_t st, const IlvrArgs& a);
void launch_ilvr_up_add(hipStream_t st, const IlvrArgs& a);

enum { ACT_NONE = 0, ACT_SILU = 1, ACT_GELU = 2, ACT_GEGLU = 3, ACT_QGELU = 4, ACT_RELU = 5 };

struct ConvGemmParams {
  const bf16_t* src0 = nullptr;
  const bf16_t* src1 = nullptr;
  int C0 = 0, C1 = 0;
  int ld0 = 0, ld1 = 0;
  int B = 1, Hs = 1, Ws = 1;
  int up = 0;
  int Hin = 1, Win = 1;
  int KH = 1, KW = 1, stride = 1, pad_t = 0, pad_l = 0;
  int Hout = 1, Wout = 1;
  int M = 0;
  const bf16_t* wgt = nullptr;
  const bf16_t* wgt_frag = nullptr;
  int Ktot = 0, N = 0;
  int ldw = 0;
  int nbatch = 1;
  int64_t a_bs = 0, w_bs = 0, o_bs = 0;
  float alpha = 1.0f;
  const float* bias = nullptr;
  const float* rowvec = nullptr;
  int rowvec_ld = 0, rows_per_vec = 1;
  const bf16_t* resid = nullptr;
  int resid_ld = 0;
  int resid_f32 = 0;
  int act = ACT_NONE;
  void* out = nullptr;
  int out_ld = 0;
  int out_f32 = 0;
  float* stats = nullptr;
  const bf16_t* zeros = nullptr;
  int ln_fold = 0;
  float ln_eps = 1e-5f;
  int tile = 0;
  float prof_flop_scale = 1.f;
  int splitk = 0;
  float* sk_scratch = nullptr;
  int* sk_flags = nullptr;
  unsigned long long* probe = nullptr;
  int korder = 1;
  int tile_group = 0;
  int dephase_ticks = 0;
  int num_cus = 256;
  int dbg = 0;
  int up_phase = 0;
  int w_ps = 0;
};
constexpr int kProbeWords = 48;
extern thread_local unsigned long long* g_conv_probe;
struct SplitKWorkspace {
  float* scratch = nullptr;
  size_t scratch_bytes = 0;
  int* flags = nullptr;
  int nflags = 0;
};
extern thread_local SplitKWorkspace g_conv_splitk;
void launch_conv_gemm(hipStream_t st, const ConvGemmParams& p);
const char* conv_gemm_last_config();
struct GemmLaunchInfo {
  int tile_id = 0;
  int bk = 0;
  int splitk = 1;
  int chm = 0;
  int tile_group = 0;
};
GemmLaunchInfo conv_gemm_last_launch();
void launch_up_phase_weights(hipStream_t st, const bf16_t* w, bf16_t* out, int Npad, int Cpad);
int conv_gemm_num_configs();
const char* conv_gemm_config_name(int id);

struct LinStreamParams {
  const bf16_t* a = nullptr; int lda = 0;
  const bf16_t* wfrag = nullptr;
  const float* bias = nullptr;
  const bf16_t* resid = nullptr; int ldr = 0;
  bf16_t* out = nullptr; int ldo = 0;
  float* stats = nullptr;
  int M = 0, N = 0;
  float ln_eps = 1e-5f;
  int geglu_direct = 0;
};
constexpr int kLinStreamTile = 30;
bool lin_stream_supports(const ConvGemmParams& p);
void launch_lin_stream(hipStream_t st, const ConvGemmParams& p);
void launch_fold_ln(hipStream_t st, const bf16_t* w, int ldw, const float* gamma, const float* beta, const float* bias,
                    bf16_t* w_out, float* bias_out, int N, int Kc);
void launch_pack_wfrag(hipStream_t st, const bf16_t* w, int ldw, bf16_t* out, int N);

struct KernelProfiler {
  bool enabled = false;
  std::vector<hipEvent_t> events;
  std::vector<double> flops;
  std::vector<std::string> labels;
  int used = 0;
  bool verbose = false;
  struct Entry { int n = 0; double ms = 0, flops = 0; };
  std::map<std::string, Entry> per_shape;
  void next_pair(hipEvent_t* a, hipEvent_t* b, double fl, const std::string& what);
  void collect(int* launches, double* total_ms, double* total_flops);
  ~KernelProfiler();
};
extern thread_local KernelProfiler* g_conv_prof;

struct ConvTuner {
  bool enabled = false;
  void* scratch = nullptr;
  size_t scratch_bytes = 0;
  int shapes_tuned = 0;
};
extern ConvTuner g_conv_tuner;

void launch_repack_weight(hipStream_t st, const float* w, bf16_t* out, int N, int Cin, int KH,
                          int KW, int Npad, int Cpad, int geglu, int64_t src_row_offset);

struct GroupNormParams {
  const bf16_t* x = nullptr;
  const bf16_t* x1 = nullptr;
  int C0 = 0, C1 = 0, ld0 = 0, ld1 = 0;
  int B = 0, HW = 0, G = 32;
  float eps = 1e-5f;
  const float* gamma = nullptr;
  const float* beta = nullptr;
  const float* film = nullptr;
  int film_ld = 0;
  int silu = 0;
  int split_out = 0;
  int* overflow = nullptr;
  bf16_t* y = nullptr;
  float* partial = nullptr;
  int S = 0;
  float* coef = nullptr;
  const float* pre0 = nullptr;
  const float* pre1 = nullptr;
};
int groupnorm_slabs(int B, int HW, int C);
void launch_groupnorm(hipStream_t st, const GroupNormParams& p);

void launch_layernorm(hipStream_t st, const bf16_t* x, int ldx, bf16_t* y, int ldy, int rows,
                      int C, const float* gamma, const float* beta, float eps);
void launch_softmax_rows(hipStream_t st, const float* s, int lds, bf16_t* p, int ldp, int64_t rows,
                         int cols);

struct AttnParams {
  const bf16_t* q = nullptr;
  const bf16_t* k = nullptr;
  const bf16_t* v = nullptr;
  const bf16_t* vt = nullptr;
  int ldv = 0; int64_t v_bs = 0;
  bf16_t* o = nullptr;
  int B = 0, H = 0, Tq = 0, Tk = 0, D = 0;
  int ldq = 0, ldk = 0, ldo = 0;
  int64_t q_bs = 0, k_bs = 0, o_bs = 0;
  int vt_dpad = 0, vt_tpad = 0;
  float scale = 1.0f;
  int q_log2 = 0;
  const float* obias = nullptr;
  int causal = 0;
};
void launch_attention(hipStream_t st, const AttnParams& p);
constexpr int kCtrlKeys = 96;
struct CtrlAttnParams {
  const bf16_t* q_own = nullptr;
  const bf16_t* q_src = nullptr;
  const bf16_t* k_own = nullptr;
  const bf16_t* k_src = nullptr;
  const bf16_t* va = nullptr;
  const bf16_t* vb = nullptr;
  bf16_t* o = nullptr;
  int B = 0, B_src = 0, H = 0, Tq = 0, L = 0, D = 0;
  int ldq = 0, ldk = 0, ldv = 0, ldo = 0;
  int64_t q_bs = 0, k_bs = 0, v_bs = 0, o_bs = 0;
  float scale = 1.0f;
  int q_log2 = 0;
};
void launch_cross_attention_ctrl(hipStream_t st, const CtrlAttnParams& p);
void launch_ctrl_values(hipStream_t st, const bf16_t* v, const float* M, const float* alpha, const float* w, int rows,
                        int B_ctrl, int L, int C, bf16_t* va, bf16_t* vb);
void launch_transpose_v(hipStream_t st, const bf16_t* v, int ldv, int64_t v_bs, bf16_t* vt, int B,
                        int H, int Tk, int D, int Dpad, int Tpad);

void launch_mfma_sustained(hipStream_t st, int target_ms, float* tflops, float* ghz);

void launch_nchw_to_nhwc(hipStream_t st, const float* x, bf16_t* y, int B, int C, int HW, int Cpad,
                         float scale, float shift, int dup);
void launch_nhwc_to_nchw(hipStream_t st, const void* x, int x_f32, int ldx, float* y, int B, int C,
                         int HW, float scale, float shift);
void launch_timestep_embedding(hipStream_t st, const StepCoef* tab, int step, const float* t_explicit,
                               float* out, int B, int dim, int mode);
void launch_vec_linear(hipStream_t st, const float* x, int ldx, const float* W, const float* bias,
                       float* y, int ldy, int B, int K, int N, int silu_in, int silu_out);
void launch_avgpool2(hipStream_t st, const bf16_t* x, bf16_t* y, int B, int H, int W, int C);
void launch_upsample2(hipStream_t st, const bf16_t* x, bf16_t* y, int B, int H, int W, int C);
void launch_up_phase_reorder(hipStream_t st, const bf16_t* x, bf16_t* y, int B, int H, int W, int C, int ldy);
void launch_posterior_sample(hipStream_t st, const float* mom, int ld, const float* noise,
                             uint64_t seed, float* z, int B, int zc, int HW, float scale,
                             int use_mean);
void launch_vq_quantize(hipStream_t st, const float* z, float in_mul, const float* codebook, int n_embed, int zc,
                        int B, int HW, bf16_t* out, int Cpad);
void launch_fill_f32(hipStream_t st, float* p, float v, int64_t n);
void launch_vit_tokens(hipStream_t st, const bf16_t* patch, const float* cls, const float* pos, bf16_t* out, int B,
                       int T, int D);
void launch_gather_eot(hipStream_t st, const bf16_t* x, const int* ids, bf16_t* out, int B, int L, int D);
void launch_embed_tokens(hipStream_t st, const int* ids, const float* tok, const float* pos, bf16_t* out, int B,
                         int L, int D, int vocab);
void launch_conv_gemm_f32(hipStream_t st, const ConvGemmParams& p);
size_t groupnorm_f32_workspace(int B, int HW, int C);
void launch_groupnorm_f32(hipStream_t st, const GroupNormParams& p, void* workspace);
void launch_attention_f32(hipStream_t st, const float* q, int ldq, const float* k, int ldk, const float* v, int ldv,
                          float* o, int ldo, int B, int H, int T, int D, float scale, const float* obias);
void launch_nchw_to_nhwc_f32(hipStream_t st, const float* x, float* y, int B, int C, int HW, int Cpad, float scale,
                             float shift, int split = 0, int* overflow = nullptr);
void launch_avgpool2_f32(hipStream_t st, const float* x, float* y, int B, int H, int W, int C);
void launch_flash_f32(hipStream_t st, const float* q, int ldq, int64_t q_bs, const float* k, int ldk, int64_t k_bs,
                      const float* v, int ldv, int64_t v_bs, float* o, int ldo, int64_t o_bs, int B, int H, int Tq, int Tk,
                      int D, float qmul, int split, int* overflow, const float* obias = nullptr);
void launch_layernorm_f32(hipStream_t st, const float* x, int ldx, float* y, int64_t rows, int C, const float* gamma,
                          const float* beta, float eps, int split, int* overflow);
void launch_geglu_f32(hipStream_t st, const float* h, float* y, int64_t rows, int Nout, int split, int* overflow);
void launch_split_rows_f32(hipStream_t st, const float* x0, int ld0, int C0, const float* x1, int ld1, int C1, bf16_t* y,
                           int64_t rows, int* overflow);
void launch_upsample2_f32(hipStream_t st, const float* x, float* y, int B, int H, int W, int C);
constexpr float kX3ActScale = 16.f;
constexpr float kX3WgtScale = 256.f;
void launch_pack_w3(hipStream_t st, const float* w, bf16_t* w3, int Npad, int taps, int Cpad, int* overflow);
void launch_avgpool2_split(hipStream_t st, const bf16_t* x, bf16_t* y, int B, int H, int W, int C, int* overflow);

void launch_copy_strided_bf16(hipStream_t st, const bf16_t* src, int lds, bf16_t* dst, int ldd,
                              int64_t rows, int cols);

}
```

cycle-diffusion_amd/csrc/lin_stream.hip:

```cpp
#include <stdlib.h>

#include <mutex>

#include "common.h"
#include "kernels.h"

namespace cd {
namespace lin_detail {

typedef __attribute__((address_space(3))) void* lptr_t;
typedef __attribute__((ext_vector_type(4))) unsigned int u32x4;

constexpr int K = 320, NKS = K / 16, KSH = NKS / 2;
constexpr int WPIECE = 2 * KSH * 1024, WSLOTS = 3;
constexpr int APIECE = 128 * 128, ASLOTS = 3;
constexpr int NAP = 10;
constexpr int ST_LD = 36, ST_BYTES = 32 * ST_LD * 4;
constexpr int BIAS_MAX = 2560;
constexpr int OFF_A = WSLOTS * WPIECE, OFF_ST = OFF_A + ASLOTS * APIECE, OFF_BIAS = OFF_ST + 8 * ST_BYTES;
constexpr int LDS_BYTES = OFF_BIAS + BIAS_MAX * 4;
static_assert(LDS_BYTES <= 160 * 1024, "LDS");
constexpr unsigned kNoLoad = 0x80000000u;
constexpr int kGegluDirectDefault = 1;

__device__ __forceinline__ void wait_vmcnt_le(int n) {
  n = n < 0 ? 0 : (n > 60 ? 60 : n);
  switch (n >> 2) {
    case 0: asm volatile("s_waitcnt vmcnt(0)" ::: "memory"); break;
    case 1: asm volatile("s_waitcnt vmcnt(4)" ::: "memory"); break;
    case 2: asm volatile("s_waitcnt vmcnt(8)" ::: "memory"); break;
    case 3: asm volatile("s_waitcnt vmcnt(12)" ::: "memory"); break;
    case 4: asm volatile("s_waitcnt vmcnt(16)" ::: "memory"); break;
    case 5: asm volatile("s_waitcnt vmcnt(20)" ::: "memory"); break;
    case 6: asm volatile("s_waitcnt vmcnt(24)" ::: "memory"); break;
    case 7: asm volatile("s_waitcnt vmcnt(28)" ::: "memory"); break;
    case 8: asm volatile("s_waitcnt vmcnt(32)" ::: "memory"); break;
    case 9: asm volatile("s_waitcnt vmcnt(36)" ::: "memory"); break;
    case 10: asm volatile("s_waitcnt vmcnt(40)" ::: "memory"); break;
    case 11: asm volatile("s_waitcnt vmcnt(44)" ::: "memory"); break;
    case 12: asm volatile("s_waitcnt vmcnt(48)" ::: "memory"); break;
    case 13: asm volatile("s_waitcnt vmcnt(52)" ::: "memory"); break;
    case 14: asm volatile("s_waitcnt vmcnt(56)" ::: "memory"); break;
    default: asm volatile("s_waitcnt vmcnt(60)" ::: "memory"); break;
  }
}

__device__ __forceinline__ u32x4 load16_hidden(u32x4 rsrc, unsigned voff) {
  u32x4 r;
  asm volatile("buffer_load_dwordx4 %0, %1, %2, 0 offen" : "=v"(r) : "v"(voff), "s"(rsrc) : "memory");
  return r;
}
__device__ __forceinline__ uint4 pack8_sat(const float* f) {
#if CD_ACT_FP16
  typedef __attribute__((ext_vector_type(2))) _Float16 h2;
  uint32_t w[4];
#pragma unroll
  for (int i = 0; i < 4; ++i) {
    const h2 v = {(_Float16)__builtin_amdgcn_fmed3f(f[2 * i], -65504.0f, 65504.0f),
                  (_Float16)__builtin_amdgcn_fmed3f(f[2 * i + 1], -65504.0f, 65504.0f)};
    w[i] = __builtin_bit_cast(uint32_t, v);
  }
  return make_uint4(w[0], w[1], w[2], w[3]);
#else
  return pack8(f);
#endif
}
__device__ __forceinline__ void touch4(u32x4& a, u32x4& b, u32x4& c, u32x4& d) {
  asm volatile("" : "+v"(a), "+v"(b), "+v"(c), "+v"(d)::"memory");
}

template <int ACT, bool RESID, bool STATS, bool LNF = false>
__global__ __launch_bounds__(512, 2) void k_lin_stream(LinStreamParams p) {
#if defined(__HIP_DEVICE_COMPILE__)
  constexpr bool GEGLU = (ACT == ACT_GEGLU);
  static_assert(!(GEGLU && (RESID || STATS)), "GEGLU has neither residual nor statistics");
  extern __shared__ __attribute__((aligned(16))) char smem[];
  char* wring = smem;
  char* aring = smem + OFF_A;
  const int tid = threadIdx.x, lane = tid & 63;
  const int wave = __builtin_amdgcn_readfirstlane(tid >> 6);
  float* stage = (float*)(smem + OFF_ST + wave * ST_BYTES);
  float* bias_s = (float*)(smem + OFF_BIAS);
  const int mi = lane & 31, half = lane >> 5;
  const bool w_issuer = wave < 4;
  const int wq = wave & 3;

  const int NT = p.N >> 6;
  const int I = 2 * NT;
  const int nstrips = (p.M + 255) >> 8;
  const int G = gridDim.x;
  const int my_count = (nstrips - (int)blockIdx.x + G - 1) / G;
  if (my_count <= 0) return;
  const int cs = I >= 80 ? 4 : (I >= 40 ? 2 : 1);

  const __amdgpu_buffer_rsrc_t rs_a =
      __builtin_amdgcn_make_buffer_rsrc((void*)p.a, 0, (unsigned)((size_t)p.M * p.lda * 2), 0x00020000);
  const __amdgpu_buffer_rsrc_t rs_w =
      __builtin_amdgcn_make_buffer_rsrc((void*)p.wfrag, 0, (unsigned)((size_t)p.N * K * 2), 0x00020000);
  const __amdgpu_buffer_rsrc_t rs_o = __builtin_amdgcn_make_buffer_rsrc(
      (void*)p.out, 0, (unsigned)((size_t)p.M * p.ldo * 2), 0x00020000);
  u32x4 rs_r = {0u, 0u, 0u, 0x00020000u};
  if (RESID) {
    const uint64_t ra = (uint64_t)p.resid;
    rs_r[0] = (unsigned)ra; rs_r[1] = (unsigned)(ra >> 32) & 0xffffu;
    rs_r[2] = (unsigned)((size_t)p.M * p.ldr * 2);
  }

  for (int i = tid; i < p.N; i += 512) bias_s[i] = p.bias ? p.bias[i] : 0.f;

  auto issue_a = [&](int row0, int j, int slot) {
    const unsigned a_row = (unsigned)((lane >> 3) * p.lda * 2);
#pragma unroll
    for (int u = 0; u < 4; ++u) {
      const int x = wq * 4 + u;
      const unsigned a_lane = a_row + (unsigned)(((lane & 7) ^ ((4 * u + (lane >> 4)) & 7)) * 16);
      const unsigned base = (unsigned)(((row0 + 128 * (j & 1) + 8 * x) * p.lda + (j >> 1) * 64) * 2);
      __builtin_amdgcn_raw_ptr_buffer_load_lds(rs_a, (lptr_t)(aring + slot * APIECE + x * 1024), 16, a_lane + base, 0,
                                               0, 0);
    }
  };
  int w_boff[5];
#pragma unroll
  for (int u = 0; u < 5; ++u) {
    const int x = wq + 4 * u;
    w_boff[u] = ((x / KSH) * NKS + (x % KSH)) * 1024;
  }
  auto issue_w = [&](int piece, bool valid, int slot) {
    const int base = ((piece >> 1) * 2 * NKS + (piece & 1) * KSH) * 1024;
    const unsigned voff = valid ? (unsigned)(lane * 16) : kNoLoad;
#pragma unroll
    for (int u = 0; u < 5; ++u)
      __builtin_amdgcn_raw_ptr_buffer_load_lds(rs_w, (lptr_t)(wring + slot * WPIECE + (wq + 4 * u) * 1024), 16, voff,
                                               base + w_boff[u], 0, 0);
  };

  bf16x8 af[NKS], afn[NKS];
  auto normalise_rows = [&]() __attribute__((always_inline)) {
    float s1 = 0.f, s2 = 0.f;
#pragma unroll
    for (int ks = 0; ks < NKS; ++ks) {
      float f[8];
      unpack8(__builtin_bit_cast(uint4, af[ks]), f);
#pragma unroll
      for (int e = 0; e < 8; ++e) { s1 += f[e]; s2 = __builtin_fmaf(f[e], f[e], s2); }
      __builtin_amdgcn_sched_barrier(0);
    }
    s1 += __shfl_xor(s1, 32);
    s2 += __shfl_xor(s2, 32);
    const float mean = s1 * (1.0f / K);
    const float var = fmaxf(s2 * (1.0f / K) - mean * mean, 0.f);
    const float rstd = __builtin_amdgcn_rsqf(var + p.ln_eps);
    const float nmr = -mean * rstd;
#pragma unroll
    for (int ks = 0; ks < NKS; ++ks) {
      float f[8];
      unpack8(__builtin_bit_cast(uint4, af[ks]), f);
#pragma unroll
      for (int e = 0; e < 8; ++e) f[e] = __builtin_fmaf(f[e], rstd, nmr);
      af[ks] = __builtin_bit_cast(bf16x8, pack8_sat(f));
      __builtin_amdgcn_sched_barrier(0);
    }
  };
  auto take_a = [&](int j, int slot) {
    if ((j & 1) != (wave >> 2)) return;
    const int row = wq * 32 + mi;
    const int sw = (row >> 1) & 7;
    unsigned base = (unsigned)(OFF_A + slot * APIECE + row * 128 + ((half ^ sw) << 4));
    asm volatile("" : "+v"(base));
    const int kb = j >> 1;
#pragma unroll
    for (int c = 0; c < 5; ++c) {
      if (kb == c) {
#pragma unroll
        for (int f = 0; f < 4; ++f) afn[4 * c + f] = *(const bf16x8*)(smem + (base ^ (unsigned)(32 * f)));
        asm volatile("" ::: "memory");
      }
    }
  };

  int seq = 0;
  int wm0 = 0, wm1 = 0;
  int am0 = 0, am1 = 0, a_fly = 0;
  int rmark = 0;

  int e_issue = 0, e_cons = 0;
  int is_o = 0, is_j = 0, is_gi = -NAP - 2;
  int is_slot = 0, is_row0 = (int)blockIdx.x * 256;
  int cn_o = 0, cn_j = 0, cn_gi = -NAP, cn_slot = 0;
  auto a_step_issue = [&](int gi) {
    if (is_o < my_count && is_gi <= gi) {
      if (!w_issuer) {
        issue_a(is_row0, is_j, is_slot);
        seq += 4;
        am0 = a_fly == 0 ? seq : am0;
        am1 = a_fly == 0 ? am1 : seq;
      }
      const bool wrap = is_j == NAP - 1;
      const int step_in = is_o == 0 ? 1 : cs, step_wrap = is_o == 0 ? I - 12 * cs + 3 : I - 9 * cs;
      ++a_fly;
      ++e_issue;
      is_slot = is_slot == ASLOTS - 1 ? 0 : is_slot + 1;
      is_gi += wrap ? step_wrap : step_in;
      is_j = wrap ? 0 : is_j + 1;
      is_o += wrap ? 1 : 0;
      is_row0 += wrap ? G * 256 : 0;
    }
  };
  auto a_due = [&](int gi) { return e_cons < e_issue && cn_gi <= gi; };
  int ce_j = 0, ce_slot = 0;
  auto a_consume_step = [&]() {
    const bool wrap = cn_j == NAP - 1;
    const int step_in = cn_o == 0 ? 1 : cs, step_wrap = cn_o == 0 ? I - 10 * cs + 1 : I - 9 * cs;
    ce_j = cn_j; ce_slot = cn_slot;
    am0 = am1; --a_fly; ++e_cons;
    cn_slot = cn_slot == ASLOTS - 1 ? 0 : cn_slot + 1;
    cn_gi += wrap ? step_wrap : step_in;
    cn_j = wrap ? 0 : cn_j + 1;
    cn_o += wrap ? 1 : 0;
  };

  if (w_issuer) {
    issue_w(0, true, 0); seq += 5; wm0 = seq;
    issue_w(1, true, 1); seq += 5; wm1 = seq;
  }
  a_step_issue(-NAP - 2);
  a_step_issue(-NAP - 1);
  for (int gi = -NAP; gi < 0; ++gi) {
    const bool due = a_due(gi);
    if (due && !w_issuer) wait_vmcnt_le(seq - am0);
    asm volatile("s_waitcnt lgkmcnt(0)\n\ts_barrier" ::: "memory");
    if (due) a_consume_step();
    a_step_issue(gi);
    if (due) take_a(ce_j, ce_slot);
  }
#pragma unroll
  for (int ks = 0; ks < NKS; ++ks) af[ks] = afn[ks];
  if (LNF) normalise_rows();

  f32x16 acc[2];
  u32x4 rres[4];
  auto issue_resid = [&](int row0, int t) {
    if (!RESID || row0 + wave * 32 >= p.M) return;
    int l2 = lane;
    asm volatile("" : "+v"(l2));
    const unsigned r_lane = (unsigned)(((wave * 32 + (l2 >> 2)) * p.ldr + (l2 & 3) * 8) * 2);
#pragma unroll
    for (int nb = 0; nb < 2; ++nb)
#pragma unroll
      for (int ps = 0; ps < 2; ++ps) {
        const int soff = ((row0 + 16 * ps) * p.ldr + t * 64 + nb * 32) * 2;
        asm volatile("buffer_load_dwordx4 %0, %1, %2, %3 offen"
                     : "=v"(rres[nb * 2 + ps]) : "v"(r_lane), "s"(rs_r), "s"(soff) : "memory");
      }
    seq += 4;
    rmark = seq;
  };
  issue_resid((int)blockIdx.x * 256, 0);

  int gi = 0;
  int wslot = 0;
  for (int ord = 0; ord < my_count; ++ord) {
    const int row0 = ((int)blockIdx.x + ord * G) * 256;
    const bool has_next = ord + 1 < my_count;
    const bool rows_ok = row0 + wave * 32 < p.M;
    for (int t = 0; t < NT; ++t) {
#pragma unroll
      for (int r = 0; r < 16; ++r) { acc[0][r] = 0.f; acc[1][r] = 0.f; }
#pragma unroll
      for (int kh = 0; kh < 2; ++kh) {
        const int i = 2 * t + kh;
        if (w_issuer) wait_vmcnt_le(seq - wm0);
        const bool due = a_due(gi);
        if (due && !w_issuer) wait_vmcnt_le(seq - am0);
        asm volatile("s_waitcnt lgkmcnt(0)\n\ts_barrier" ::: "memory");
        if (w_issuer) {
          const int nxt = i + 2;
          const int slot2 = wslot == 0 ? 2 : wslot - 1;
          issue_w(nxt < I ? nxt : nxt - I, nxt < I || has_next, slot2);
          seq += 5;
          wm0 = wm1; wm1 = seq;
        }
        if (due) a_consume_step();
        a_step_issue(gi);
        const char* wp = wring + wslot * WPIECE + lane * 16;
        if (RESID) {
#pragma unroll
          for (int ksl = 0; ksl < KSH; ++ksl) {
            const bf16x8 w0 = *(const bf16x8*)(wp + ksl * 1024), w1 = *(const bf16x8*)(wp + (KSH + ksl) * 1024);
            acc[0] = CD_MFMA_32x32x16(w0, af[kh * KSH + ksl], acc[0]);
            acc[1] = CD_MFMA_32x32x16(w1, af[kh * KSH + ksl], acc[1]);
            __builtin_amdgcn_sched_barrier(0);
          }
        } else {
          constexpr int PFD = 2;
          bf16x8 wf[PFD + 1][2];
#pragma unroll
          for (int d = 0; d < PFD; ++d) {
            wf[d][0] = *(const bf16x8*)(wp + d * 1024);
            wf[d][1] = *(const bf16x8*)(wp + (KSH + d) * 1024);
          }
#pragma unroll
          for (int ksl = 0; ksl < KSH; ++ksl) {
            if (ksl + PFD < KSH) {
              wf[(ksl + PFD) % (PFD + 1)][0] = *(const bf16x8*)(wp + (ksl + PFD) * 1024);
              wf[(ksl + PFD) % (PFD + 1)][1] = *(const bf16x8*)(wp + (KSH + ksl + PFD) * 1024);
            }
            acc[0] = CD_MFMA_32x32x16(wf[ksl % (PFD + 1)][0], af[kh * KSH + ksl], acc[0]);
            acc[1] = CD_MFMA_32x32x16(wf[ksl % (PFD + 1)][1], af[kh * KSH + ksl], acc[1]);
            __builtin_amdgcn_sched_barrier(0);
          }
        }
        if (due) take_a(ce_j, ce_slot);
        wslot = wslot == 2 ? 0 : wslot + 1;
        ++gi;
      }
      if (RESID && rows_ok) {
        wait_vmcnt_le(seq - rmark);
        touch4(rres[0], rres[1], rres[2], rres[3]);
      }
      float vv[2][8];
      int l2 = lane;
      asm volatile("" : "+v"(l2));
      const int prow = l2 >> 2, pcol = (l2 & 3) * 8, mi2 = l2 & 31, half2 = l2 >> 5;
      const unsigned o_lane = (unsigned)(((wave * 32 + prow) * p.ldo + pcol) * 2);
      if (GEGLU && p.geglu_direct) {
        const unsigned od_lane = (unsigned)(((wave * 32 + mi2) * p.ldo + 4 * half2) * 2);
#pragma unroll
        for (int q = 0; q < 4; ++q) {
          const float* bp = bias_s + t * 64 + 8 * q + 4 * half2;
          const f32x4 bv = *(const f32x4*)bp, bg = *(const f32x4*)(bp + 32);
          float val[4], gate[4], o4[4];
#pragma unroll
          for (int j = 0; j < 4; ++j) { val[j] = acc[0][4 * q + j] + bv[j]; gate[j] = acc[1][4 * q + j] + bg[j]; }
          mul_gelu4(val, gate, o4);
          if (rows_ok) {
            typedef __attribute__((ext_vector_type(2))) unsigned int u32x2;
            const u32x2 o = {pack2(o4[0], o4[1]), pack2(o4[2], o4[3])};
            __builtin_amdgcn_raw_buffer_store_b64(o, rs_o, od_lane, (row0 * p.ldo + t * 32 + 8 * q) * 2, 0);
          }
          __builtin_amdgcn_sched_barrier(0);
        }
      } else {
#pragma unroll
      for (int nb = 0; nb < 2; ++nb) {
        __builtin_amdgcn_wave_barrier();
#pragma unroll
        for (int q = 0; q < 4; ++q) {
          const f32x4 v4 = {acc[nb][4 * q], acc[nb][4 * q + 1], acc[nb][4 * q + 2], acc[nb][4 * q + 3]};
          *(f32x4*)(stage + mi2 * ST_LD + 8 * q + 4 * half2) = v4;
        }
        asm volatile("s_waitcnt lgkmcnt(0)" ::: "memory");
        __builtin_amdgcn_wave_barrier();
        const int ncol0 = t * 64 + nb * 32;
        const f32x4 b0 = *(const f32x4*)(bias_s + ncol0 + pcol), b1 = *(const f32x4*)(bias_s + ncol0 + pcol + 4);
#pragma unroll
        for (int ps = 0; ps < 2; ++ps) {
          float* srow = stage + (prow + 16 * ps) * ST_LD + pcol;
          const f32x4 lo = *(const f32x4*)srow, hi = *(const f32x4*)(srow + 4);
          float v[8] = {lo[0] + b0[0], lo[1] + b0[1], lo[2] + b0[2], lo[3] + b0[3],
                        hi[0] + b1[0], hi[1] + b1[1], hi[2] + b1[2], hi[3] + b1[3]};
          if (GEGLU) {
            if (nb == 0) {
#pragma unroll
              for (int e = 0; e < 8; ++e) vv[ps][e] = v[e];
            } else {
              mul_gelu8(vv[ps], v, v);
              if (rows_ok) {
                const uint4 o = pack8_sat(v);
                __builtin_amdgcn_raw_buffer_store_b128(__builtin_bit_cast(u32x4, o), rs_o, o_lane,
                                                       ((row0 + 16 * ps) * p.ldo + t * 32) * 2, 0);
              }
            }
          } else {
            if (RESID && rows_ok) {
              float rr[8];
              unpack8(__builtin_bit_cast(uint4, rres[nb * 2 + ps]), rr);
#pragma unroll
              for (int e = 0; e < 8; ++e) v[e] += rr[e];
            }
            if (rows_ok) {
              const uint4 o = pack8_sat(v);
              __builtin_amdgcn_raw_buffer_store_b128(__builtin_bit_cast(u32x4, o), rs_o, o_lane,
                                                     ((row0 + 16 * ps) * p.ldo + ncol0) * 2, 0);
            }
            if (STATS) {
              *(f32x4*)srow = (f32x4){v[0], v[1], v[2], v[3]};
              *(f32x4*)(srow + 4) = (f32x4){v[4], v[5], v[6], v[7]};
              asm volatile("s_waitcnt lgkmcnt(0)" ::: "memory");
            }
          }
          __builtin_amdgcn_sched_barrier(0);
        }
        if (STATS) {
          __builtin_amdgcn_wave_barrier();
          float s1 = 0.f, s2 = 0.f;
#pragma unroll
          for (int r = 0; r < 16; ++r) {
            const float x = stage[(16 * half2 + r) * ST_LD + mi2];
            s1 += x; s2 += x * x;
          }
          s1 += __shfl_xor(s1, 32); s2 += __shfl_xor(s2, 32);
          if (rows_ok && half2 == 0) {
            float* sp = p.stats + (int64_t)((row0 + wave * 32) >> 5) * 2 * p.N + ncol0 + mi2;
            sp[0] = s1; sp[p.N] = s2;
          }
        }
      }
      }
      if (RESID) {
        const bool last = t + 1 == NT;
        if (!last || has_next) issue_resid(last ? row0 + G * 256 : row0, last ? 0 : t + 1);
      }
    }
    if (has_next) {
#pragma unroll
      for (int ks = 0; ks < NKS; ++ks) af[ks] = afn[ks];
      if (LNF) normalise_rows();
    }
  }
  asm volatile("s_waitcnt vmcnt(0)" ::: "memory");
#endif
}

__global__ void k_pack_wfrag(const bf16_t* __restrict__ w, int ldw, bf16_t* __restrict__ out, int N) {
  const int64_t total = (int64_t)(N / 32) * NKS * 64;
  for (int64_t i = blockIdx.x * (int64_t)blockDim.x + threadIdx.x; i < total; i += (int64_t)gridDim.x * blockDim.x) {
    const int l = (int)(i & 63);
    const int ks = (int)((i >> 6) % NKS), nb = (int)((i >> 6) / NKS);
    const uint4 v = *(const uint4*)(w + (int64_t)(32 * nb + (l & 31)) * ldw + 16 * ks + 8 * (l >> 5));
    *(uint4*)(out + i * 8) = v;
  }
}

__global__ void k_fold_ln(const bf16_t* __restrict__ w, int ldw, const float* __restrict__ gamma,
                          const float* __restrict__ beta, const float* __restrict__ bias, bf16_t* __restrict__ w_out,
                          float* __restrict__ bias_out, int N, int Kc) {
  const int n = blockIdx.x * (blockDim.x >> 6) + (threadIdx.x >> 6), lane = threadIdx.x & 63;
  if (n >= N) return;
  float acc = 0.f;
  for (int k = lane; k < Kc; k += 64) {
    const float x = bf2f(w[(int64_t)n * ldw + k]);
    acc = __builtin_fmaf(x, beta[k], acc);
    w_out[(int64_t)n * ldw + k] = f2bf(x * gamma[k]);
  }
  acc = wave_allsum(acc);
  if (lane == 0) bias_out[n] = (bias ? bias[n] : 0.f) + acc;
}

template <int ACT, bool RESID, bool STATS, bool LNF = false>
void launch_variant(hipStream_t st, const LinStreamParams& p, int grid) {
  static PerDeviceOnce attr_once;
  auto kern = k_lin_stream<ACT, RESID, STATS, LNF>;
  attr_once([&]() {
    HIP_CHECK(hipFuncSetAttribute((const void*)kern, hipFuncAttributeMaxDynamicSharedMemorySize, LDS_BYTES));
  });
  hipLaunchKernelGGL(kern, dim3(grid), dim3(512), LDS_BYTES, st, p);
}

}

bool lin_stream_supports(const ConvGemmParams& p) {
  if (p.KH != 1 || p.KW != 1 || p.stride != 1 || p.up || p.src1 || p.C1 != 0) return false;
  if (p.Ktot != lin_detail::K || p.C0 != lin_detail::K || p.nbatch != 1 || p.out_f32 || p.rowvec) return false;
  if (p.alpha != 1.0f || p.splitk > 1 || !p.wgt_frag) return false;
  if (p.N % 64 != 0 || p.N > lin_detail::BIAS_MAX || p.N < 320) return false;
  if (p.act != ACT_NONE && p.act != ACT_GEGLU) return false;
  if (p.act == ACT_GEGLU && (p.resid || p.stats)) return false;
  if (p.M % 32 != 0) return false;
  if ((p.ld0 % 8) != 0 || (p.out_ld % 8) != 0 || (p.resid && (p.resid_ld % 8) != 0)) return false;
  const int nout = p.act == ACT_GEGLU ? p.N / 2 : p.N;
  if ((int64_t)p.M * p.ld0 * 2 >= (1ll << 31) || (int64_t)p.M * p.out_ld * 2 >= (1ll << 31)) return false;
  if (p.resid && (int64_t)p.M * p.resid_ld * 2 >= (1ll << 31)) return false;
  (void)nout;
  return true;
}

void launch_lin_stream(hipStream_t st, const ConvGemmParams& c) {
  using namespace lin_detail;
  CD_CHECK(lin_stream_supports(c), "lin_stream: unsupported problem (M %d N %d K %d)", c.M, c.N, c.Ktot);
  LinStreamParams p;
  p.a = c.src0; p.lda = c.ld0; p.wfrag = c.wgt_frag; p.bias = c.bias;
  p.resid = c.resid; p.ldr = c.resid_ld; p.out = (bf16_t*)c.out; p.ldo = c.out_ld;
  p.stats = c.stats; p.M = c.M; p.N = c.N;
  static std::atomic<int> ncu_of[64];
  int dev = 0;
  HIP_CHECK(hipGetDevice(&dev));
  int ncu = ncu_of[dev & 63].load(std::memory_order_relaxed);
  if (!ncu) {
    hipDeviceProp_t prop;
    HIP_CHECK(hipGetDeviceProperties(&prop, dev));
    ncu = prop.multiProcessorCount > 0 ? prop.multiProcessorCount : 256;
    ncu_of[dev & 63].store(ncu, std::memory_order_relaxed);
  }
  const int nstrips = (p.M + 255) / 256;
  const int grid = nstrips < ncu ? nstrips : ncu;
  static const int geglu_direct = [] { const char* e = getenv("CYCLEDIFF_GEGLU_DIRECT"); return e && e[0] ? atoi(e) : kGegluDirectDefault; }();
  p.geglu_direct = geglu_direct;
  if (c.ln_fold) {
    p.ln_eps = c.ln_eps;
    CD_CHECK(!c.resid && !c.stats, "lin_stream: a LayerNorm-folded layer has neither residual nor statistics");
    if (c.act == ACT_GEGLU) launch_variant<ACT_GEGLU, false, false, true>(st, p, grid);
    else launch_variant<ACT_NONE, false, false, true>(st, p, grid);
    return;
  }
  if (c.act == ACT_GEGLU) launch_variant<ACT_GEGLU, false, false>(st, p, grid);
  else if (c.resid && c.stats) launch_variant<ACT_NONE, true, true>(st, p, grid);
  else if (c.resid) launch_variant<ACT_NONE, true, false>(st, p, grid);
  else if (c.stats) launch_variant<ACT_NONE, false, true>(st, p, grid);
  else launch_variant<ACT_NONE, false, false>(st, p, grid);
}

void launch_fold_ln(hipStream_t st, const bf16_t* w, int ldw, const float* gamma, const float* beta, const float* bias,
                    bf16_t* w_out, float* bias_out, int N, int Kc) {
  hipLaunchKernelGGL(lin_detail::k_fold_ln, dim3((N + 3) / 4), dim3(256), 0, st, w, ldw, gamma, beta, bias, w_out,
                     bias_out, N, Kc);
}

void launch_pack_wfrag(hipStream_t st, const bf16_t* w, int ldw, bf16_t* out, int N) {
  CD_CHECK(N % 32 == 0 && ldw >= lin_detail::K, "pack_wfrag: N %% 32, ldw >= 320");
  const int64_t total = (int64_t)(N / 32) * lin_detail::NKS * 64;
  int grid = (int)((total + 255) / 256);
  if (grid > 2048) grid = 2048;
  hipLaunchKernelGGL(lin_detail::k_pack_wfrag, dim3(grid), dim3(256), 0, st, w, ldw, out, N);
}

}
```

cycle-diffusion_amd/csrc/norm.hip:

```cpp
#include "common.h"
#include "kernels.h"

namespace cd {

namespace {

constexpr int GN_MAX_VPT = 4;

__device__ inline const bf16_t* gn_src(const GroupNormParams& p, int b, int row, int c, int& off) {
  if (c < p.C0) { off = c; return p.x + ((int64_t)b * p.HW + row) * p.ld0; }
  off = c - p.C0;
  return p.x1 + ((int64_t)b * p.HW + row) * p.ld1;
}

__device__ inline void gn_write_coef(const GroupNormParams& p, int b, int c, float sum, float sumsq, int cpg) {
  const int C = p.C0 + p.C1;
  const float n = (float)cpg * (float)p.HW;
  const float mean = sum / n;
  float var = sumsq / n - mean * mean;
  var = var < 0.f ? 0.f : var;
  const float rstd = 1.0f / sqrtf(var + p.eps);
  float a = rstd * p.gamma[c];
  float bb = p.beta[c] - mean * a;
  if (p.film) {
// ... 132 lines not shown
  int rif, vpt;
  if (nvec <= 256) { rif = 256 / nvec; vpt = 1; }
  else { rif = 1; vpt = (nvec + 255) >> 8; }
  const int r0 = (nvec <= 256) ? tid / nvec : 0;
  const int v0 = (nvec <= 256) ? tid % nvec : tid;
  if (nvec <= 256 && tid >= nvec * rif) return;
  const float* coef = p.coef + (int64_t)b * 2 * C;
  for (int j = 0; j < vpt; ++j) {
    const int v = v0 + j * 256;
    if (v >= nvec) break;
    const int c = v * 8;
    float ca[8], cb[8];
    {
      const f32x4 a0 = *(const f32x4*)(coef + c), a1 = *(const f32x4*)(coef + c + 4);
      const f32x4 b0 = *(const f32x4*)(coef + C + c), b1 = *(const f32x4*)(coef + C + c + 4);
#pragma unroll
      for (int e = 0; e < 4; ++e) { ca[e] = a0[e]; ca[4 + e] = a1[e]; cb[e] = b0[e]; cb[4 + e] = b1[e]; }
    }
    for (int row = row_begin + r0; row < row_end; row += 4 * rif) {
      uint4 raw[4];
#pragma unroll
      for (int u = 0; u < 4; ++u) {
        const int r = row + u * rif;
        raw[u] = make_uint4(0, 0, 0, 0);
        if (r < row_end) {
          int off;
          const bf16_t* base = gn_src(p, b, r, c, off);
          raw[u] = *(const uint4*)(base + off);
        }
      }
#pragma unroll
      for (int u = 0; u < 4; ++u) {
        const int r = row + u * rif;
        if (r < row_end) {
          float f[8];
          unpack8(raw[u], f);
#pragma unroll
          for (int e = 0; e < 8; ++e) {
            float y = f[e] * ca[e] + cb[e];
            if (p.silu) y = silu_f(y);
            f[e] = y;
          }
          *(uint4*)(p.y + ((int64_t)b * p.HW + r) * C + c) = pack8(f);
        }
      }
    }
  }
}

template <int VPL, int R>
__global__ __launch_bounds__(256) void k_layernorm(const bf16_t* __restrict__ x, int ldx,
                                                   bf16_t* __restrict__ y, int ldy, int rows, int C,
                                                   const float* __restrict__ gamma,
                                                   const float* __restrict__ beta, float eps) {
  const int lane = threadIdx.x & 63;
  const int row0 = (blockIdx.x * 4 + (threadIdx.x >> 6)) * R;
  if (row0 >= rows) return;
  const int nvec = C >> 3;
  uint4 raw[R][VPL];
#pragma unroll
  for (int r = 0; r < R; ++r)
#pragma unroll
    for (int j = 0; j < VPL; ++j) {
      const int v = lane + j * 64 < nvec ? lane + j * 64 : 0;
      const int row = row0 + r < rows ? row0 + r : rows - 1;
      raw[r][j] = *(const uint4*)(x + (int64_t)row * ldx + v * 8);
    }
  float ga[VPL][8], be[VPL][8];
#pragma unroll
  for (int j = 0; j < VPL; ++j) {
    const int v = lane + j * 64 < nvec ? lane + j * 64 : 0;
    {
      const f32x4 g0 = *(const f32x4*)(gamma + v * 8), g1 = *(const f32x4*)(gamma + v * 8 + 4);
      const f32x4 b0 = *(const f32x4*)(beta + v * 8), b1 = *(const f32x4*)(beta + v * 8 + 4);
#pragma unroll
      for (int e = 0; e < 4; ++e) { ga[j][e] = g0[e]; ga[j][4 + e] = g1[e]; be[j][e] = b0[e]; be[j][4 + e] = b1[e]; }
    }
  }
#pragma unroll
  for (int r = 0; r < R; ++r) {
    const int row = row0 + r;
    if (row >= rows) break;
    float f[VPL][8];
    float s = 0.f;
#pragma unroll
    for (int j = 0; j < VPL; ++j) {
      unpack8(raw[r][j], f[j]);
      if (lane + j * 64 < nvec) {
#pragma unroll
        for (int e = 0; e < 8; ++e) s += f[j][e];
      }
    }
    s = wave_allsum(s);
    const float mean = s / (float)C;
    float q = 0.f;
#pragma unroll
    for (int j = 0; j < VPL; ++j) {
      if (lane + j * 64 < nvec) {
#pragma unroll
        for (int e = 0; e < 8; ++e) { const float d = f[j][e] - mean; q += d * d; }
      }
    }
    q = wave_allsum(q);
    const float rstd = 1.0f / sqrtf(q / (float)C + eps);
#pragma unroll
    for (int j = 0; j < VPL; ++j) {
      const int v = lane + j * 64;
      if (v < nvec) {
        float o8[8];
#pragma unroll
        for (int e = 0; e < 8; ++e) o8[e] = (f[j][e] - mean) * rstd * ga[j][e] + be[j][e];
        *(uint4*)(y + (int64_t)row * ldy + v * 8) = pack8(o8);
      }
    }
  }
}

__global__ __launch_bounds__(256) void k_softmax_rows(const float* __restrict__ s, int lds_,
                                                      bf16_t* __restrict__ p, int ldp, int cols) {
  __shared__ float red[4];
  const int64_t row = blockIdx.x;
  const float* sr = s + row * lds_;
  bf16_t* pr = p + row * ldp;
  const int tid = threadIdx.x, lane = tid & 63, w = tid >> 6;
  float mx = -INFINITY;
  for (int i = tid; i < cols; i += 256) mx = fmaxf(mx, sr[i]);
#pragma unroll
  for (int o = 32; o > 0; o >>= 1) mx = fmaxf(mx, __shfl_xor(mx, o));
  if (lane == 0) red[w] = mx;
  __syncthreads();
  mx = fmaxf(fmaxf(red[0], red[1]), fmaxf(red[2], red[3]));
  __syncthreads();
  float sum = 0.f;
  for (int i = tid; i < cols; i += 256) sum += __expf(sr[i] - mx);
#pragma unroll
  for (int o = 32; o > 0; o >>= 1) sum += __shfl_xor(sum, o);
  if (lane == 0) red[w] = sum;
  __syncthreads();
  sum = (red[0] + red[1]) + (red[2] + red[3]);
  const float inv = 1.0f / sum;
  for (int i = tid; i < cols; i += 256) pr[i] = f2bf(__expf(sr[i] - mx) * inv);
}

}

int groupnorm_slabs(int B, int HW, int C) {
  (void)B; (void)C;
  int S = HW / 64;
  if (S < 1) S = 1;
  if (S > 64) S = 64;
  return S;
}

void launch_groupnorm(hipStream_t st, const GroupNormParams& p) {
  const int C = p.C0 + p.C1;
  CD_CHECK(C % 8 == 0 && C % p.G == 0 && p.G <= 64, "groupnorm: C=%d G=%d unsupported", C, p.G);
  CD_CHECK(p.C0 % 8 == 0, "groupnorm: concat split must be a multiple of 8");
  CD_CHECK((C >> 3) <= 256 * GN_MAX_VPT, "groupnorm: C too large");
  CD_CHECK(p.partial && p.S > 0, "groupnorm: workspace missing");
  const int nvec = C >> 3;
  const int rif = nvec <= 256 ? 256 / nvec : 1;
  CD_CHECK(p.coef, "groupnorm: coefficient workspace missing");
  CD_CHECK(C / p.G <= 256, "groupnorm: more than 256 channels per group");
  GroupNormParams q = p;
  if (p.pre0 && (p.C1 == 0 || p.pre1) && (p.HW % 32) == 0) {
    q.S = 1;
    hipLaunchKernelGGL(k_gn_fold, dim3(p.G, p.B), dim3(256), 0, st, q);
  } else {
    const int rows_per_slab = ceil_div(p.HW, p.S);
    const size_t lds = (size_t)rif * C * 2 * sizeof(float);
    hipLaunchKernelGGL(k_gn_stats, dim3(p.S, p.B), dim3(256), lds, st, p, rows_per_slab);
    hipLaunchKernelGGL(k_gn_coef, dim3(p.B), dim3(256), 0, st, p);
  }
  int rows_per_block = (int)(((int64_t)p.HW * p.B + 2047) / 2048);
  const int unit = 4 * rif;
  rows_per_block = ceil_div(rows_per_block, unit) * unit;
  hipLaunchKernelGGL(k_gn_apply, dim3(ceil_div(p.HW, rows_per_block), p.B), dim3(256), 0, st, q, rows_per_block);
}

void launch_layernorm(hipStream_t st, const bf16_t* x, int ldx, bf16_t* y, int ldy, int rows,
                      int C, const float* gamma, const float* beta, float eps) {
  CD_CHECK(C % 8 == 0 && C <= 2048, "layernorm: C=%d unsupported", C);
  CD_CHECK((ldx & 7) == 0 && (ldy & 7) == 0, "layernorm: row strides must be multiples of 8 elements");
#define CD_LN(VPL, R)                                                                                              \
  hipLaunchKernelGGL((k_layernorm<VPL, R>), dim3(ceil_div(rows, 4 * R)), dim3(256), 0, st, x, ldx, y, ldy, rows, C, \
                     gamma, beta, eps)
  if (C <= 512) CD_LN(1, 4);
  else if (C <= 1024) CD_LN(2, 4);
  else if (C <= 1536) CD_LN(3, 2);
  else CD_LN(4, 2);
#undef CD_LN
}

void launch_softmax_rows(hipStream_t st, const float* s, int lds_, bf16_t* p, int ldp, int64_t rows,
                         int cols) {
  hipLaunchKernelGGL(k_softmax_rows, dim3((unsigned)rows), dim3(256), 0, st, s, lds_, p, ldp, cols);
}

}
```

cycle-diffusion_amd/csrc/unet_openai.hip:

```cpp
#include <limits.h>

#include <algorithm>

#include "engine.h"

namespace cd {

namespace {

struct ResW {
  int cin = 0, cout = 0;
  bool up = false, down = false, film = false;
  GNW gn1, gn2;
  ConvW *conv1 = nullptr, *conv2 = nullptr, *skip = nullptr;
  int emb_off = 0;
};

struct STW {
  int C = 0, heads = 0, dh = 0, ctx = 0;
  GNW norm;
  ConvW *proj_in = nullptr, *proj_out = nullptr;
  LNW ln1, ln2, ln3;
  ConvW *qkv1 = nullptr, *qk1 = nullptr, *v1 = nullptr, *o1 = nullptr;
  ConvW *q2 = nullptr, *k2 = nullptr, *v2 = nullptr, *o2 = nullptr;
  ConvW *ff1 = nullptr, *ff2 = nullptr;
  ConvW *q2_ln = nullptr, *ff1_ln = nullptr;
  bf16_t* k2c = nullptr;
  bf16_t* v2c = nullptr;
};

struct ABW {
  int C = 0, heads = 0, dh = 0;
  GNW norm;
  ConvW *qk = nullptr, *v = nullptr, *proj = nullptr;
  float* vbias = nullptr;
};

struct Layer {
  enum Kind { CONV_IN, RES, ST, AB, DOWN_CONV, UP_CONV } kind;
  int idx = 0;
  ConvW* conv = nullptr;
};
struct Block { std::vector<Layer> layers; };

class UNetOpenAI : public UNet {
 public:
  explicit UNetOpenAI(const cd_net_desc& d);
  int kind() const override { return CD_NET_UNET_OPENAI; }
  void forward(Ctx& c, const UNetIO& io) override;
  void set_context(Ctx& c, const bf16_t* ctx, int B, int L) override;
  void build_attn_control(Ctx& c, const float* mapper, const float* alpha, const float* weight, int B_ctrl,
                          AttnCtrl& ctrl) override;
  size_t workspace_hint(int B) const override;

 private:
  int mc_, hidden_;
  TimeEmb te_;
  std::vector<ResW> res_;
  std::vector<STW> st_;
  std::vector<ABW> ab_;
  std::vector<Block> in_blocks_, out_blocks_;
  Block mid_;
  GNW out_norm_;
  ConvW* out_conv_ = nullptr;
  int ctx_B_ = 0, ctx_L_ = 0;
  std::vector<void*> ctx_allocs_;
  const AttnCtrl* ctrl_ = nullptr;

  int add_res(const std::string& pfx, int cin, int cout, bool up, bool down);
  int add_st(const std::string& pfx, int C, int heads, int dh);
  int add_ab(const std::string& pfx, int C, int heads);
  int folded_version_ = -1;
  void refresh_ln_folds(Ctx& c);
  Act run_block(Ctx& c, const Block& b, Act h, const Act* skip, const float* proj, int proj_ld, bool t_shared);
  Act res_fwd(Ctx& c, const ResW& r, const Act& x, const Act* x2, const float* proj, int proj_ld, bool t_shared);
  Act st_fwd(Ctx& c, STW& s, const Act& x, int dup_tail = 0);
  void st_core16(Ctx& c, STW& s, const Act& x_in, const Act& x_resid, Act& out, int b0, int dup_tail);
  Act ab_fwd(Ctx& c, const ABW& a, const Act& x);
 public:
  ~UNetOpenAI() override { for (void* p : ctx_allocs_) (void)hipFree(p); }
};

GNW make_gn(ParamStore& ps, const std::string& pfx, int C, float eps) {
  GNW g; g.C = C; g.eps = eps;
  g.g = ps.new_vec(C, 1.f); g.b = ps.new_vec(C, 0.f);
  ps.vec(pfx + ".weight", g.g, C);
  ps.vec(pfx + ".bias", g.b, C);
  return g;
}
LNW make_ln(ParamStore& ps, const std::string& pfx, int C) {
  LNW g; g.C = C;
  g.g = ps.new_vec(C, 1.f); g.b = ps.new_vec(C, 0.f);
  ps.vec(pfx + ".weight", g.g, C);
  ps.vec(pfx + ".bias", g.b, C);
  return g;
}
ConvW* make_conv(ParamStore& ps, const std::string& pfx, int N, int Cin, int k, bool bias, bool geglu = false,
                 int ref_ndim = 4, float wscale = 1.f) {
  CD_CHECK(!(bias && wscale != 1.f), "a folded weight scale needs the bias scaled too");
  ConvW* c = ps.new_conv(N, Cin, k, k, bias, geglu);
  ps.conv_weight(pfx + ".weight", c, ref_ndim, wscale);
  if (bias) ps.conv_bias(pfx + ".bias", c);
  return c;
}

int UNetOpenAI::add_res(const std::string& pfx, int cin, int cout, bool up, bool down) {
  ResW r; r.cin = cin; r.cout = cout; r.up = up; r.down = down; r.film = desc.use_scale_shift_norm != 0;
  r.gn1 = make_gn(params, pfx + ".in_layers.0", cin, 1e-5f);
  r.conv1 = make_conv(params, pfx + ".in_layers.2", cout, cin, 3, true);
  r.gn2 = make_gn(params, pfx + ".out_layers.0", cout, 1e-5f);
  r.conv2 = make_conv(params, pfx + ".out_layers.3", cout, cout, 3, true);
  if (cin != cout) r.skip = make_conv(params, pfx + ".skip_connection", cout, cin, 1, true);
  r.emb_off = te_.proj_total;
  te_.proj_total += r.film ? 2 * cout : cout;
  res_.push_back(r);
  return (int)res_.size() - 1;
}

int UNetOpenAI::add_st(const std::string& pfx, int C, int heads, int dh) {
  STW s; s.C = C; s.heads = heads; s.dh = dh; s.ctx = desc.context_dim;
  CD_CHECK(heads * dh == C, "spatial transformer: inner dim %d != channels %d", heads * dh, C);
  CD_CHECK(desc.transformer_depth == 1, "only transformer_depth=1 is supported");
  s.norm = make_gn(params, pfx + ".norm", C, 1e-6f);
  s.proj_in = make_conv(params, pfx + ".proj_in", C, C, 1, true);
  s.proj_out = make_conv(params, pfx + ".proj_out", C, C, 1, true);
  const std::string tb = pfx + ".transformer_blocks.0";
  s.ln1 = make_ln(params, tb + ".norm1", C);
  s.ln2 = make_ln(params, tb + ".norm2", C);
  s.ln3 = make_ln(params, tb + ".norm3", C);
  const float qscale = 1.44269504088896340736f / sqrtf((float)dh);
  if (dh == 40) {
    s.qk1 = params.new_conv(2 * C, C, 1, 1, false);
    params.conv_rows(tb + ".attn1.to_q.weight", {C, C}, s.qk1, 0, C, 0, C, 0, qscale);
    params.conv_rows(tb + ".attn1.to_k.weight", {C, C}, s.qk1, C, C, 0, C, 0);
    s.v1 = make_conv(params, tb + ".attn1.to_v", C, C, 1, false, false, 2);
  } else {
    s.qkv1 = params.new_conv(3 * C, C, 1, 1, false);
    params.conv_rows(tb + ".attn1.to_q.weight", {C, C}, s.qkv1, 0, C, 0, C, 0, qscale);
    params.conv_rows(tb + ".attn1.to_k.weight", {C, C}, s.qkv1, C, C, 0, C, 0);
    params.conv_rows(tb + ".attn1.to_v.weight", {C, C}, s.qkv1, 2 * C, C, 0, C, 0);
  }
  s.o1 = make_conv(params, tb + ".attn1.to_out.0", C, C, 1, true, false, 2);
  s.q2 = make_conv(params, tb + ".attn2.to_q", C, C, 1, false, false, 2, qscale);
  s.k2 = make_conv(params, tb + ".attn2.to_k", C, s.ctx, 1, false, false, 2);
  s.v2 = make_conv(params, tb + ".attn2.to_v", C, s.ctx, 1, false, false, 2);
  s.o2 = make_conv(params, tb + ".attn2.to_out.0", C, C, 1, true, false, 2);
  s.ff1 = make_conv(params, tb + ".ff.net.0.proj", 8 * C, C, 1, true, true, 2);
  s.ff2 = make_conv(params, tb + ".ff.net.2", C, 4 * C, 1, true, false, 2);
  if (s.q2->wfrag) {
    s.q2_ln = params.new_conv(C, C, 1, 1, true);
    s.ff1_ln = params.new_conv(8 * C, C, 1, 1, true, true);
  }
  st_.push_back(s);
  return (int)st_.size() - 1;
}

int UNetOpenAI::add_ab(const std::string& pfx, int C, int heads) {
  ABW a; a.C = C; a.heads = heads; a.dh = C / heads;
  a.norm = make_gn(params, pfx + ".norm", C, 1e-5f);
  const int ch = a.dh;
  a.qk = params.new_conv(2 * C, C, 1, 1, true);
  a.v = params.new_conv(C, C, 1, 1, false);
  a.vbias = params.new_vec(C);
  const std::string wn = pfx + ".qkv.weight", bn = pfx + ".qkv.bias";
  params.conv_rows(wn, {3 * C, C, 1}, a.qk, 0, C, 0, ch, 3 * ch);
  params.conv_rows(wn, {3 * C, C, 1}, a.qk, C, C, ch, ch, 3 * ch);
  params.conv_rows(wn, {3 * C, C, 1}, a.v, 0, C, 2 * ch, ch, 3 * ch);
  params.bias_rows(bn, 3 * C, a.qk->b, 0, C, 0, ch, 3 * ch);
  params.bias_rows(bn, 3 * C, a.qk->b, C, C, ch, ch, 3 * ch);
  params.bias_rows(bn, 3 * C, a.vbias, 0, C, 2 * ch, ch, 3 * ch);
  a.proj = make_conv(params, pfx + ".proj_out", C, C, 1, true, false, 3);
  ab_.push_back(a);
  return (int)ab_.size() - 1;
}

UNetOpenAI::UNetOpenAI(const cd_net_desc& d) {
  desc = d;
  f32 = d.precision == CD_PREC_F32 || d.precision == CD_PREC_F32X3;
  x3 = d.precision == CD_PREC_F32X3;
  params.f32 = f32; params.x3 = x3;

  mc_ = d.model_channels; hidden_ = 4 * mc_;
  image_size = d.image_size; out_channels = d.out_channels;
  in_cpad = round_up(d.in_channels, 32);
  CD_CHECK(mc_ % 32 == 0, "model_channels must be a multiple of 32");
  const bool use_st = d.use_spatial_transformer != 0;
  auto has_attn = [&](int ds) { for (int i = 0; i < d.n_attn; ++i) if (d.attn[i] == ds) return true; return false; };
  auto heads_for = [&](int ch, int& heads, int& dh) {
    if (d.num_head_channels == -1) { heads = d.num_heads; dh = ch / heads; }
    else { heads = ch / d.num_head_channels; dh = d.num_head_channels; }
  };
  std::vector<std::string> res_pfx;
  auto add_res_named = [&](const std::string& pfx, int cin, int cout, bool up, bool down) {
    res_pfx.push_back(pfx);
    return add_res(pfx, cin, cout, up, down);
  };
  auto add_attn = [&](Block& blk, const std::string& pfx, int ch) {
    int heads, dh; heads_for(ch, heads, dh);
    Layer l;
    if (use_st) { l.kind = Layer::ST; l.idx = add_st(pfx, ch, heads, dh); }
    else { l.kind = Layer::AB; l.idx = add_ab(pfx, ch, heads); }
    blk.layers.push_back(l);
  };

  {
    Block b; Layer l; l.kind = Layer::CONV_IN;
    l.conv = make_conv(params, "input_blocks.0.0", mc_, d.in_channels, 3, true);
    b.layers.push_back(l); in_blocks_.push_back(b);
  }
  std::vector<int> chans{mc_};
  int ch = mc_, ds = 1, bi = 1;
  for (int level = 0; level < d.n_mult; ++level) {
    const int mult = d.channel_mult[level];
    for (int r = 0; r < d.num_res_blocks; ++r) {
      Block b; Layer l; l.kind = Layer::RES;
      const std::string pfx = "input_blocks." + std::to_string(bi);
      l.idx = add_res_named(pfx + ".0", ch, mult * mc_, false, false);
      b.layers.push_back(l);
      ch = mult * mc_;
      if (has_attn(ds)) add_attn(b, pfx + ".1", ch);
      in_blocks_.push_back(b); chans.push_back(ch); ++bi;
    }
    if (level != d.n_mult - 1) {
      Block b; Layer l;
      const std::string pfx = "input_blocks." + std::to_string(bi) + ".0";
      if (d.resblock_updown) { l.kind = Layer::RES; l.idx = add_res_named(pfx, ch, ch, false, true); }
      else {
        CD_CHECK(d.conv_resample, "Downsample without conv (avg-pool) only exists inside resblock_updown");
        l.kind = Layer::DOWN_CONV; l.conv = make_conv(params, pfx + ".op", ch, ch, 3, true);
      }
      b.layers.push_back(l); in_blocks_.push_back(b); chans.push_back(ch); ++bi; ds *= 2;
    }
  }
  {
    Layer l; l.kind = Layer::RES; l.idx = add_res_named("middle_block.0", ch, ch, false, false);
    mid_.layers.push_back(l);
    add_attn(mid_, "middle_block.1", ch);
    Layer l2; l2.kind = Layer::RES; l2.idx = add_res_named("middle_block.2", ch, ch, false, false);
    mid_.layers.push_back(l2);
  }
  int oi = 0;
  for (int level = d.n_mult - 1; level >= 0; --level) {
    const int mult = d.channel_mult[level];
    for (int i = 0; i <= d.num_res_blocks; ++i) {
      const int ich = chans.back(); chans.pop_back();
      Block b; Layer l; l.kind = Layer::RES;
      const std::string pfx = "output_blocks." + std::to_string(oi);
      l.idx = add_res_named(pfx + ".0", ch + ich, mc_ * mult, false, false);
      b.layers.push_back(l);
      ch = mc_ * mult;
      int sub = 1;
      if (has_attn(ds)) { add_attn(b, pfx + "." + std::to_string(sub), ch); ++sub; }
      if (level && i == d.num_res_blocks) {
        Layer u;
        const std::string up = pfx + "." + std::to_string(sub);
        if (d.resblock_updown) { u.kind = Layer::RES; u.idx = add_res_named(up, ch, ch, true, false); }
        else { u.kind = Layer::UP_CONV; u.conv = make_conv(params, up + ".conv", ch, ch, 3, true); params.add_up_phase(u.conv); }
        b.layers.push_back(u);
        ds /= 2;
      }
      out_blocks_.push_back(b); ++oi;
    }
  }
  out_norm_ = make_gn(params, "out.0", ch, 1e-5f);
  out_conv_ = make_conv(params, "out.2", d.out_channels, mc_, 3, true);
  CD_CHECK(ch == mc_, "channel bookkeeping: final channels %d != model_channels %d", ch, mc_);

  te_.mode = 0; te_.dim = mc_; te_.hidden = hidden_;
  te_.w0 = params.new_vec(hidden_ * mc_); te_.b0 = params.new_vec(hidden_);
  te_.w1 = params.new_vec(hidden_ * hidden_); te_.b1 = params.new_vec(hidden_);
  params.mat_f32("time_embed.0.weight", te_.w0, hidden_, mc_);
  params.vec("time_embed.0.bias", te_.b0, hidden_);
  params.mat_f32("time_embed.2.weight", te_.w1, hidden_, hidden_);
  params.vec("time_embed.2.bias", te_.b1, hidden_);
  te_.proj_w = params.new_vec(te_.proj_total * hidden_);
  te_.proj_b = params.new_vec(te_.proj_total);
  for (size_t i = 0; i < res_.size(); ++i) {
    const int n = res_[i].film ? 2 * res_[i].cout : res_[i].cout;
    params.mat_f32(res_pfx[i] + ".emb_layers.1.weight", te_.proj_w, n, hidden_, res_[i].emb_off);
    params.bias_rows(res_pfx[i] + ".emb_layers.1.bias", n, te_.proj_b, res_[i].emb_off, n, 0, n, 0);
  }
}

size_t UNetOpenAI::workspace_hint(int B) const {
  const size_t hw = (size_t)image_size * image_size;
  size_t widest = 0;
  for (auto& r : res_) widest = std::max(widest, (size_t)std::max(r.cin, r.cout));
  return (size_t)B * hw * std::max(widest, (size_t)8 * mc_) * 2 * 24 + (64u << 20);
}

Act UNetOpenAI::res_fwd(Ctx& c, const ResW& r, const Act& x, const Act* x2, const float* proj, int proj_ld,
                        bool t_shared) {
  const int Ho = r.up ? x.H * 2 : (r.down ? x.H / 2 : x.H);
  const int Wo = r.up ? x.W * 2 : (r.down ? x.W / 2 : x.W);
  Act out = alloc_act(c, x.B, Ho, Wo, r.cout, true);
  const int rpv = t_shared ? INT_MAX : Ho * Wo;
  const size_t mk = c.arena->mark();
  Act h = groupnorm_fwd(c, r.gn1, x, x2, true);
  Act xs = x;
  const Act* xs2 = x2;
  bool up_in_conv = false;
  if (r.down) {
    CD_CHECK(!x2, "resblock_updown with concat input is not produced by the reference");
    h = avgpool2_fwd(c, h);
    xs = avgpool2_fwd(c, x); xs2 = nullptr;
  } else if (r.up) {
    CD_CHECK(!x2, "resblock_updown with concat input is not produced by the reference");
    up_in_conv = true;
    xs = upsample2_fwd(c, x); xs2 = nullptr;
  }
  ConvOpts o1; o1.up = up_in_conv; o1.want_stats = true;
  const float* pr = proj + r.emb_off;
  if (!r.film) { o1.rowvec = pr; o1.rowvec_ld = proj_ld; o1.rows_per_vec = rpv; }
  Act h2 = conv_fwd(c, *r.conv1, h, nullptr, o1);
  Act h3;
  if (r.film) h3 = groupnorm_fwd(c, r.gn2, h2, nullptr, true, pr, t_shared ? 0 : proj_ld);
  else h3 = groupnorm_fwd(c, r.gn2, h2, nullptr, true);
  Act skip;
  if (r.skip) {
    ConvOpts os; os.pad = 0;
    skip = conv_fwd(c, *r.skip, xs, xs2, os);
  } else {
    CD_CHECK(!xs2, "identity skip with concat input");
    skip = xs;
  }
  ConvOpts o2; o2.resid = &skip; o2.out = out.p; o2.out_ld = out.ld; o2.out_stats = out.stats_buf;
  conv_fwd(c, *r.conv2, h3, nullptr, o2);
  out.stats = out.stats_buf;
  c.arena->release(mk);
  return out;
}

static void vt_gemm(Ctx& c, const ConvW& wv, const bf16_t* x, int ldx, int B, int T, int Tpad, bf16_t* vt) {
  ConvGemmParams p;
  p.src0 = wv.w; p.C0 = wv.Cpad; p.ld0 = wv.Cpad;
  p.B = 1; p.Hs = wv.N; p.Ws = 1; p.Hin = wv.N; p.Win = 1; p.Hout = wv.N; p.Wout = 1;
  p.M = wv.N;
  p.wgt = x; p.Ktot = wv.Cpad; p.N = T;
  CD_CHECK(ldx == wv.Cpad, "vt_gemm: token row stride %d must equal K %d", ldx, wv.Cpad);
  p.nbatch = B; p.a_bs = 0; p.w_bs = (int64_t)T * ldx; p.o_bs = (int64_t)wv.N * Tpad;
  p.out = vt; p.out_ld = Tpad; p.zeros = c.zeros;
  launch_conv_gemm(c.st, p);
}

void UNetOpenAI::set_context(Ctx& c, const bf16_t* ctx, int B, int L) {
  if (st_.empty()) return;
  if (B != ctx_B_ || L != ctx_L_) {
    for (void* p : ctx_allocs_) (void)hipFree(p);
    ctx_allocs_.clear();
    const size_t esz = f32 ? 4 : 2;
    for (auto& s : st_) {
      HIP_CHECK(hipMalloc((void**)&s.k2c, (size_t)B * L * s.C * esz + 256));
      HIP_CHECK(hipMalloc((void**)&s.v2c, (size_t)B * L * s.C * esz + 256));
      ctx_allocs_.push_back(s.k2c); ctx_allocs_.push_back(s.v2c);
    }
    ctx_B_ = B; ctx_L_ = L;
  }
  const bool keep_f32 = c.f32, keep_x3 = c.x3;
  c.f32 = f32; c.x3 = x3;
  Act cx; cx.p = (bf16_t*)ctx; cx.B = 1; cx.H = B * L; cx.W = 1; cx.C = st_[0].ctx; cx.ld = cx.C; cx.f32 = f32;
  for (auto& s : st_) {
    ConvOpts o; o.pad = 0; o.out = s.k2c; o.out_ld = s.C;
    conv_fwd(c, *s.k2, cx, nullptr, o);
    o.out = s.v2c;
    conv_fwd(c, *s.v2, cx, nullptr, o);
  }
  c.f32 = keep_f32; c.x3 = keep_x3;
}

void UNetOpenAI::build_attn_control(Ctx& c, const float* mapper, const float* alpha, const float* weight, int B_ctrl,
                                    AttnCtrl& ctrl) {
  CD_CHECK(!st_.empty() && st_[0].k2c, "cross-attention control: the network has no cross-attention context set");
  CD_CHECK(!f32, "cross-attention control is not built for fp32 / fp32x3 networks (their transformer blocks run the fp32 "
                 "attention of st_f32.hip): use the 16-bit precision");
  CD_CHECK(ctx_L_ <= kCtrlKeys, "cross-attention control: context length %d above the %d keys the kernel keeps resident",
           ctx_L_, kCtrlKeys);
  CD_CHECK(ctrl.rows > 0 && ctrl.row0 >= 0 && ctrl.row0 + ctrl.rows == ctx_B_, "cross-attention control: rows %d + %d of a "
           "batch of %d (the controlled rows are the tail of the batch)", ctrl.row0, ctrl.rows, ctx_B_);
  CD_CHECK(ctrl.B_src > 0 && ctrl.src_b0 >= 0 && ctrl.src_b0 + ctrl.B_src <= ctrl.row0, "cross-attention control: source rows");
  CD_CHECK(mapper && alpha && weight && B_ctrl > 0, "cross-attention control: mapper / alpha / weight");
  ctrl.va.clear(); ctrl.vb.clear();
  for (auto& s : st_) {
    const size_t bytes = (size_t)ctrl.rows * ctx_L_ * s.C * 2;
    bf16_t* va = (bf16_t*)c.arena->alloc(bytes);
    bf16_t* vb = (bf16_t*)c.arena->alloc(bytes);
    launch_ctrl_values(c.st, s.v2c + (int64_t)ctrl.row0 * ctx_L_ * s.C, mapper, alpha, weight, ctrl.rows, B_ctrl, ctx_L_, s.C,
                       va, vb);
    ctrl.va.push_back(va); ctrl.vb.push_back(vb);
  }
}

static void dup_rows(Ctx& c, const bf16_t* src, bf16_t* dst, int64_t n, int64_t tail, int cols) {
  launch_copy_strided_bf16(c.st, src, cols, dst, cols, n, cols);
  launch_copy_strided_bf16(c.st, src + (n - tail) * cols, cols, dst + n * cols, cols, tail, cols);
}

Act UNetOpenAI::st_fwd(Ctx& c, STW& s, const Act& x_in, int dup_tail) {
  int B = x_in.B;
  const bool dup = dup_tail > 0;
  const int T = x_in.H * x_in.W, C = s.C;
  CD_CHECK(dup_tail >= 0 && dup_tail <= B, "transformer block: %d repeated samples of %d", dup_tail, B);
  Act out = alloc_act(c, B + dup_tail, x_in.H, x_in.W, C, true);
  Act x = x_in;
  if (dup) {
    CD_CHECK(x_in.ld == C, "transformer block: dense input expected");
    x = alloc_act(c, B + dup_tail, x_in.H, x_in.W, C);
    dup_rows(c, x_in.p, x.p, (int64_t)B * T, (int64_t)dup_tail * T, C);
  }
  const size_t mk = c.arena->mark();
  CD_CHECK(s.k2c && ctx_B_ == B + dup_tail, "cross-attention context not set for batch %d", B + dup_tail);
  if (c.f32) {
    ConvOpts p0; p0.pad = 0;
    Act n = groupnorm_fwd(c, s.norm, x_in, nullptr, false);
    Act h = conv_fwd(c, *s.proj_in, n, nullptr, p0);
    const float scale = 1.0f / sqrtf((float)s.dh);
    CD_CHECK(!dup, "transformer block: prefix sharing is a 16-bit path feature");
    const float* ck = (const float*)s.k2c;
    const float* cv = (const float*)s.v2c;
    {
      const size_t m2 = c.arena->mark();
      Act n1 = layernorm_fwd(c, s.ln1, h);
      Act a;
      if (s.qkv1) {
        Act qkv = conv_fwd(c, *s.qkv1, n1, nullptr, p0);
        a = attention_flash_f32_fwd(c, qkv.pf(), qkv.ld, qkv.pf() + C, qkv.ld, (int64_t)T * qkv.ld, qkv.pf() + 2 * C, qkv.ld,
                                    (int64_t)T * qkv.ld, B, s.heads, T, T, s.dh, scale, x.H, x.W, true);
      } else {
        Act qk = conv_fwd(c, *s.qk1, n1, nullptr, p0);
        Act vv = conv_fwd(c, *s.v1, n1, nullptr, p0);
        a = attention_flash_f32_fwd(c, qk.pf(), qk.ld, qk.pf() + C, qk.ld, (int64_t)T * qk.ld, vv.pf(), vv.ld,
                                    (int64_t)T * vv.ld, B, s.heads, T, T, s.dh, scale, x.H, x.W, true);
      }
      ConvOpts o; o.pad = 0; o.resid = &h; o.out = h.p; o.out_ld = h.ld;
      conv_fwd(c, *s.o1, a, nullptr, o);
      c.arena->release(m2);
    }
    {
      const size_t m2 = c.arena->mark();
      Act n2 = layernorm_fwd(c, s.ln2, h);
      Act q = conv_fwd(c, *s.q2, n2, nullptr, p0);
      Act a = attention_flash_f32_fwd(c, q.pf(), q.ld, ck, C, (int64_t)ctx_L_ * C, cv, C, (int64_t)ctx_L_ * C, B, s.heads, T,
                                      ctx_L_, s.dh, scale, x.H, x.W, true);
      ConvOpts o; o.pad = 0; o.resid = &h; o.out = h.p; o.out_ld = h.ld;
      conv_fwd(c, *s.o2, a, nullptr, o);
      c.arena->release(m2);
    }
    {
      const int64_t rows = h.rows();
      int64_t chunk = ((int64_t)1 << 30) / ((int64_t)8 * C * 4);
      chunk = std::max<int64_t>(4096, chunk & ~(int64_t)4095);
      for (int64_t r0 = 0; r0 < rows; r0 += chunk) {
        const int64_t n = std::min(chunk, rows - r0);
        const size_t m2 = c.arena->mark();
        Act hv = h;
        hv.p = (bf16_t*)(h.pf() + r0 * h.ld); hv.B = 1; hv.H = (int)n; hv.W = 1;
        Act n3 = layernorm_fwd(c, s.ln3, hv);
        ConvOpts pg; pg.pad = 0; pg.raw_geglu = true;
        Act g8 = conv_fwd(c, *s.ff1, n3, nullptr, pg);
        Act g = geglu_f32_fwd(c, g8);
        ConvOpts o; o.pad = 0; o.resid = &hv; o.out = hv.p; o.out_ld = hv.ld;
        conv_fwd(c, *s.ff2, g, nullptr, o);
        c.arena->release(m2);
      }
    }
    ConvOpts po; po.pad = 0; po.resid = &x; po.out = out.p; po.out_ld = out.ld; po.out_stats = out.stats_buf;
    if (c.x3) {
      Act hs = split_rows_f32_fwd(c, h);
      Act y = conv_fwd(c, *s.proj_out, hs, nullptr, po);
      out.stats = y.stats;
    } else {
      conv_fwd(c, *s.proj_out, h, nullptr, po);
    }
    c.arena->release(mk);
    return out;
  }
  static const int st_chunk = [] { const char* e = getenv("CYCLEDIFF_ST_CHUNK"); return e ? atoi(e) : 0; }();
  c.arena->release(mk);
  if (!dup && !ctrl_ && st_chunk > 0 && T >= 4096 && B >= 2 * st_chunk) {
    for (int b0 = 0; b0 < B; b0 += st_chunk) {
      const int n = std::min(st_chunk, B - b0);
      auto view = [&](const Act& a) {
        Act v = a; v.B = n;
        v.p = a.p + (int64_t)b0 * T * a.ld;
        if (a.stats) v.stats = a.stats + ((int64_t)b0 * T / 32) * 2 * a.C;
        if (a.stats_buf) v.stats_buf = a.stats_buf + ((int64_t)b0 * T / 32) * 2 * a.C;
        return v;
      };
      Act xv = view(x_in), ov = view(out);
      st_core16(c, s, xv, xv, ov, b0, 0);
    }
  } else {
    st_core16(c, s, x_in, x, out, 0, dup_tail);
  }
  out.stats = out.stats_buf;
  return out;
}

void UNetOpenAI::st_core16(Ctx& c, STW& s, const Act& x_in, const Act& x, Act& out, int b0, int dup_tail) {
  const bool dup = dup_tail > 0;
  int B = x_in.B;
  const int T = x_in.H * x_in.W, C = s.C;
  const size_t mk = c.arena->mark();
  ConvOpts p0; p0.pad = 0;
  const float scale = 1.0f / sqrtf((float)s.dh);
  const bf16_t* k2c = s.k2c + (int64_t)b0 * ctx_L_ * C;
  const bf16_t* v2c = s.v2c + (int64_t)b0 * ctx_L_ * C;
  Act n = groupnorm_fwd(c, s.norm, x_in, nullptr, false);
  Act h = conv_fwd(c, *s.proj_in, n, nullptr, p0);
  {
    const size_t m2 = c.arena->mark();
    Act n1 = layernorm_fwd(c, s.ln1, h);
    Act a;
    if (s.qkv1) {
      Act qkv = conv_fwd(c, *s.qkv1, n1, nullptr, p0);
      a = attention_fwd(c, qkv.p, qkv.ld, qkv.p + C, qkv.ld, qkv.p + 2 * C, qkv.ld, B, s.heads, T, T, s.dh, scale,
                        x.H, x.W, true);
    } else {
      Act qk = conv_fwd(c, *s.qk1, n1, nullptr, p0);
      const int Tpad = round_up(T, 64);
      bf16_t* vt = (bf16_t*)c.arena->alloc((size_t)B * C * Tpad * 2);
      if (Tpad != T) HIP_CHECK(hipMemsetAsync(vt, 0, (size_t)B * C * Tpad * 2, c.st));
      vt_gemm(c, *s.v1, n1.p, n1.ld, B, T, Tpad, vt);
      a = attention_vt_fwd(c, qk.p, qk.ld, qk.p + C, qk.ld, vt, B, s.heads, T, T, Tpad, s.dh, scale, x.H, x.W,
                           true);
    }
    ConvOpts o; o.pad = 0; o.resid = &h; o.out = h.p; o.out_ld = h.ld;
    conv_fwd(c, *s.o1, a, nullptr, o);
    c.arena->release(m2);
  }
  if (dup) {
    Act h2 = alloc_act(c, B + dup_tail, x_in.H, x_in.W, C);
    dup_rows(c, h.p, h2.p, (int64_t)B * T, (int64_t)dup_tail * T, C);
    h = h2;
    B += dup_tail;
  }
  {
    const size_t m2 = c.arena->mark();
    Act q;
    if (s.q2_ln && conv_ln_fold_available(c, *s.q2_ln, h.rows())) {
      ConvOpts pl; pl.pad = 0; pl.ln_fold = true;
      q = conv_fwd(c, *s.q2_ln, h, nullptr, pl);
    } else {
      Act n2 = layernorm_fwd(c, s.ln2, h);
      q = conv_fwd(c, *s.q2, n2, nullptr, p0);
    }
    Act a;
    if (!ctrl_) {
      a = attention_fwd(c, q.p, q.ld, k2c, C, v2c, C, B, s.heads, T, ctx_L_, s.dh, scale, x.H, x.W, true);
    } else {
      const int Bu = ctrl_->row0;
      CD_CHECK(b0 == 0 && Bu + ctrl_->rows == B, "cross-attention control: rows %d + %d of a batch of %d", Bu, ctrl_->rows, B);
      const size_t bi = (size_t)(&s - st_.data());
      CD_CHECK(bi < ctrl_->va.size(), "cross-attention control: no values for transformer block %d", (int)bi);
      a = alloc_act(c, B, x.H, x.W, C);
      AttnParams pu;
      pu.q = q.p; pu.k = k2c; pu.v = v2c; pu.o = a.p;
      pu.B = Bu; pu.H = s.heads; pu.Tq = T; pu.Tk = ctx_L_; pu.D = s.dh;
      pu.ldq = q.ld; pu.ldk = C; pu.ldv = C; pu.ldo = a.ld;
      pu.q_bs = (int64_t)T * q.ld; pu.k_bs = (int64_t)ctx_L_ * C; pu.v_bs = (int64_t)ctx_L_ * C; pu.o_bs = (int64_t)T * a.ld;
      pu.scale = scale; pu.q_log2 = 1;
      launch_attention(c.st, pu);
      CtrlAttnParams p;
      p.q_own = q.p + (int64_t)Bu * pu.q_bs; p.q_src = q.p + (int64_t)ctrl_->src_b0 * pu.q_bs;
      p.k_own = k2c + (int64_t)Bu * pu.k_bs; p.k_src = k2c + (int64_t)ctrl_->src_b0 * pu.k_bs;
      p.va = ctrl_->va[bi]; p.vb = ctrl_->vb[bi]; p.o = a.p + (int64_t)Bu * pu.o_bs;
      p.B = ctrl_->rows; p.B_src = ctrl_->B_src; p.H = s.heads; p.Tq = T; p.L = ctx_L_; p.D = s.dh;
      p.ldq = q.ld; p.ldk = C; p.ldv = C; p.ldo = a.ld;
      p.q_bs = pu.q_bs; p.k_bs = pu.k_bs; p.v_bs = pu.v_bs; p.o_bs = pu.o_bs;
      p.scale = scale; p.q_log2 = 1;
      launch_cross_attention_ctrl(c.st, p);
    }
    ConvOpts o; o.pad = 0; o.resid = &h; o.out = h.p; o.out_ld = h.ld;
    conv_fwd(c, *s.o2, a, nullptr, o);
    c.arena->release(m2);
  }
  {
    const size_t m2 = c.arena->mark();
    Act g;
    if (s.ff1_ln && conv_ln_fold_available(c, *s.ff1_ln, h.rows())) {
      ConvOpts pl; pl.pad = 0; pl.ln_fold = true;
      g = conv_fwd(c, *s.ff1_ln, h, nullptr, pl);
    } else {
      Act n3 = layernorm_fwd(c, s.ln3, h);
      g = conv_fwd(c, *s.ff1, n3, nullptr, p0);
    }
    ConvOpts o; o.pad = 0; o.resid = &h; o.out = h.p; o.out_ld = h.ld;
    conv_fwd(c, *s.ff2, g, nullptr, o);
    c.arena->release(m2);
  }
  ConvOpts po; po.pad = 0; po.resid = &x; po.out = out.p; po.out_ld = out.ld; po.out_stats = out.stats_buf;
  conv_fwd(c, *s.proj_out, h, nullptr, po);
  c.arena->release(mk);
}

Act UNetOpenAI::ab_fwd(Ctx& c, const ABW& a, const Act& x) {
  const int B = x.B, T = x.H * x.W, C = a.C;
  Act out = alloc_act(c, B, x.H, x.W, C, true);
  const size_t mk = c.arena->mark();
  ConvOpts p0; p0.pad = 0;
  Act n = groupnorm_fwd(c, a.norm, x, nullptr, false);
  Act qk = conv_fwd(c, *a.qk, n, nullptr, p0);
  if (c.f32) {
    Act v = conv_fwd(c, *a.v, n, nullptr, p0);
    Act o = attention_f32_fwd(c, qk, v, a.heads, a.dh, 1.0f / sqrtf((float)a.dh), a.vbias);
    ConvOpts po; po.pad = 0; po.resid = &x; po.out = out.p; po.out_ld = out.ld;
    conv_fwd(c, *a.proj, o, nullptr, po);
    c.arena->release(mk);
    return out;
  }
  const int Tpad = round_up(T, 64);
  bf16_t* vt = (bf16_t*)c.arena->alloc((size_t)B * C * Tpad * 2);
  if (Tpad != T) HIP_CHECK(hipMemsetAsync(vt, 0, (size_t)B * C * Tpad * 2, c.st));
  vt_gemm(c, *a.v, n.p, n.ld, B, T, Tpad, vt);
  Act o = alloc_act(c, B, x.H, x.W, C);
  AttnParams p;
  p.q = qk.p; p.k = qk.p + C; p.vt = vt; p.o = o.p;
  p.B = B; p.H = a.heads; p.Tq = T; p.Tk = T; p.D = a.dh;
  p.ldq = qk.ld; p.ldk = qk.ld; p.ldo = o.ld;
  p.q_bs = (int64_t)T * qk.ld; p.k_bs = (int64_t)T * qk.ld; p.o_bs = (int64_t)T * o.ld;
  p.vt_dpad = a.dh; p.vt_tpad = Tpad; p.scale = 1.0f / sqrtf((float)a.dh); p.obias = a.vbias;
  launch_attention(c.st, p);
  ConvOpts po; po.pad = 0; po.resid = &x; po.out = out.p; po.out_ld = out.ld; po.out_stats = out.stats_buf;
  conv_fwd(c, *a.proj, o, nullptr, po);
  out.stats = out.stats_buf;
  c.arena->release(mk);
  return out;
}

Act UNetOpenAI::run_block(Ctx& c, const Block& b, Act h, const Act* skip, const float* proj, int proj_ld,
                          bool t_shared) {
  bool first = true;
  for (const Layer& l : b.layers) {
    const Act* x2 = first ? skip : nullptr;
    switch (l.kind) {
      case Layer::CONV_IN: { ConvOpts o; o.want_stats = true; h = conv_fwd(c, *l.conv, h, nullptr, o); break; }
      case Layer::RES: h = res_fwd(c, res_[l.idx], h, x2, proj, proj_ld, t_shared); break;
      case Layer::ST: h = st_fwd(c, st_[l.idx], h); break;
      case Layer::AB: h = ab_fwd(c, ab_[l.idx], h); break;
      case Layer::DOWN_CONV: { ConvOpts o; o.stride = 2; o.want_stats = true; h = conv_fwd(c, *l.conv, h, nullptr, o); break; }
      case Layer::UP_CONV: { ConvOpts o; o.up = true; o.want_stats = true; h = conv_fwd(c, *l.conv, h, nullptr, o); break; }
    }
    first = false;
  }
  return h;
}

void UNetOpenAI::refresh_ln_folds(Ctx& c) {
  if (folded_version_ == params.version) return;
  for (const Block& b : out_blocks_)
    for (const Layer& l : b.layers)
      if (l.kind == Layer::UP_CONV) params.refresh_up_phase(c.st, l.conv);
  for (STW& s : st_) {
    if (!s.q2_ln) continue;
    struct { const ConvW* src; ConvW* dst; const LNW* ln; } jobs[2] = {{s.q2, s.q2_ln, &s.ln2}, {s.ff1, s.ff1_ln, &s.ln3}};
    for (auto& j : jobs) {
      launch_fold_ln(c.st, j.src->w, j.src->Ktot(), j.ln->g, j.ln->b, j.src->b, j.dst->w, j.dst->b, j.src->Npad,
                     j.src->Cpad);
      launch_pack_wfrag(c.st, j.dst->w, j.dst->Ktot(), j.dst->wfrag, j.dst->Npad);
    }
  }
  folded_version_ = params.version;
}

void UNetOpenAI::forward(Ctx& c, const UNetIO& io) {
  const size_t mk0 = c.arena->mark();
  c.f32 = f32; c.x3 = x3;
// ... 69 lines not shown
```

include/cyclediff.h:

```cpp
#ifndef CYCLEDIFF_H
#define CYCLEDIFF_H
#include <stddef.h>
#include <stdint.h>

#ifdef __cplusplus
extern "C" {
#endif

typedef struct cd_engine* cd_handle;

enum { CD_NET_UNET_OPENAI = 1, CD_NET_UNET_HO = 2, CD_NET_VAE_KL = 3, CD_NET_CLIP_TEXT = 4, CD_NET_BERT_XTR = 5,
       CD_NET_OCLIP_TEXT = 6, CD_NET_OCLIP_VISION = 7, CD_NET_INCEPTION_FID = 8 };
enum { CD_SCHED_DDIM = 0, CD_SCHED_DDPM = 1 };
enum { CD_PREC_16 = 0, CD_PREC_F32 = 1, CD_PREC_F32X3 = 2 };
enum { CD_MASK_QSAMPLE = 0, CD_MASK_ENCODER = 1 };

typedef struct cd_net_desc {
  int kind;
  int image_size;
  int in_channels, out_channels;
  int model_channels;
  int num_res_blocks;
  int n_mult;  int channel_mult[8];
  int n_attn;  int attn[8];
  int num_heads;
  int num_head_channels;
  int use_spatial_transformer, context_dim, transformer_depth;
  int use_scale_shift_norm, resblock_updown, conv_resample;
  int z_channels, embed_dim, double_z;
  int precision;
  int n_embed;
  int reserved[6];
} cd_net_desc;

typedef struct cd_step_coef {
  float sa, s1a, sap, dirc, sigma, r, t_mask;
  int32_t t;
} cd_step_coef;

const char* cd_last_error(void);
int cd_version(void);
int cd_act_format(void);

int cd_engine_create(void* hip_stream, size_t workspace_bytes, cd_handle* out);
int cd_engine_destroy(cd_handle h);
int cd_engine_workspace_high_water(cd_handle h, size_t* bytes);
int cd_engine_synchronize(cd_handle h);
int cd_prof_enable(cd_handle h, int on);
int cd_prof_collect(cd_handle h, int* launches, double* total_ms, double* total_flops);

int cd_net_create(cd_handle h, const cd_net_desc* desc, int* net_id);
int cd_net_param_count(cd_handle h, int net, int* n);
int cd_net_param_info(cd_handle h, int net, int index, char* name, int name_cap, int* ndim, int64_t shape[4]);
int cd_net_load_param(cd_handle h, int net, const char* name, const float* data_host, int ndim,
                      const int64_t* shape);
int cd_net_missing_params(cd_handle h, int net, int* n_missing, char* first_name, int name_cap);

int cd_unet_forward(cd_handle h, int net, const float* x, const float* t, const float* ctx, int B,
                    int ctx_len, float* eps_out);

int cd_text_encode(cd_handle h, int net, const int32_t* tokens, int B, int L, float* out);

int cd_inception_features(cd_handle h, int net, const float* img, int B, int stop_block, float* out);
int cd_clip_text_features(cd_handle h, int net, const int32_t* tokens, int B, int L, float* out);
int cd_clip_image_features(cd_handle h, int net, const float* img, int B, float* out);

int cd_vae_encode(cd_handle h, int net, const float* img, const float* noise, uint64_t seed, int B, int R,
                  int sample, float scale, float* z0);
int cd_vae_decode(cd_handle h, int net, const float* z0, int B, int hlat, float scale, float out_mul,
                  float out_add, float* img);

int cd_dpm_encode(cd_handle h, int net, int sched_kind, const float* x0, const float* ctx_c,
                  const float* ctx_uc, int ctx_len, float guidance, int B, int K,
                  const cd_step_coef* coef_host, const float* noise, uint64_t seed,
                  int last_uses_x0, float* z_out);

int cd_ddim_decode(cd_handle h, int net, int sched_kind, const float* z, int z_slots, int n_eps,
                   const float* ctx_c, const float* ctx_uc, int ctx_len, float guidance, int B, int K,
                   const cd_step_coef* coef_host, const float* noise_tail, uint64_t seed, float* x_out);

int cd_ddim_decode_v(cd_handle h, int net, int sched_kind, const float* z, int z_slots, int n_eps,
                     const float* ctx_c, const float* ctx_uc, int ctx_len, const float* guidance_per_sample, int B,
                     int K, const cd_step_coef* coef_host, const float* noise_tail, uint64_t seed, float* x_out);

int cd_ddim_invert(cd_handle h, int net, int sched_kind, const float* x0, const float* ctx_c, const float* ctx_uc,
                   int ctx_len, float guidance, int B, int K, const cd_step_coef* coef_host, float* x_out,
                   float* traj_out);

int cd_cycle_translate(cd_handle h, int net, int sched_kind, const float* x0, const float* enc_ctx_c,
                       const float* enc_ctx_uc, float enc_guidance, const float* dec_ctx_c, const float* dec_ctx_uc,
                       float dec_guidance, const float* dec_guidance_per_sample, int ctx_len, int B, int n_dec, int K,
                       const cd_step_coef* coef_enc_host, const cd_step_coef* coef_dec_host, const float* noise,
                       uint64_t seed, int last_uses_x0, float* z_out, float* x_out);

int cd_ddim_decode_masked(cd_handle h, int net, int sched_kind, const float* z, int z_slots, int n_eps, const float* ctx_c,
                          const float* ctx_uc, int ctx_len, float guidance, const float* guidance_per_sample, int B, int K,
                          const cd_step_coef* coef_host, const float* noise_tail, uint64_t seed, const float* mask,
                          const float* x0, int B_mask, int mask_source, const float* qsample_coef_host,
                          const float* mask_noise, uint64_t mask_seed, float* x_out);

int cd_cycle_translate_masked(cd_handle h, int net, int sched_kind, const float* x0, const float* enc_ctx_c,
                              const float* enc_ctx_uc, float enc_guidance, const float* dec_ctx_c, const float* dec_ctx_uc,
                              float dec_guidance, const float* dec_guidance_per_sample, int ctx_len, int B, int n_dec, int K,
                              const cd_step_coef* coef_enc_host, const cd_step_coef* coef_dec_host, const float* noise,
                              uint64_t seed, int last_uses_x0, const float* mask, const float* mask_x0, int B_mask,
                              int mask_source, const float* qsample_coef_host, const float* mask_noise, uint64_t mask_seed,
                              float* z_out, float* x_out);

int cd_cycle_translate_ctrl(cd_handle h, int net, int sched_kind, const float* x0, const float* enc_ctx_c,
                            const float* enc_ctx_uc, float enc_guidance, const float* dec_ctx_c, const float* dec_ctx_uc,
                            float dec_guidance, const float* dec_guidance_per_sample, int ctx_len, int B, int n_dec, int K,
                            const cd_step_coef* coef_enc_host, const cd_step_coef* coef_dec_host, const float* noise,
                            uint64_t seed, int last_uses_x0, const float* mask, const float* mask_x0, int B_mask,
                            int mask_source, const float* qsample_coef_host, const float* mask_noise, uint64_t mask_seed,
                            const float* mapper, const float* alpha, const float* weight, int B_ctrl, int n_ctrl,
                            float* z_out, float* x_out);

int cd_ilvr_decode(cd_handle h, int net, int sched_kind, const float* z, int z_slots, int n_eps, int B, int K,
                   const cd_step_coef* coef_host, const float* noise_tail, uint64_t seed, const float* ref, int B_ref,
                   int down_n, int range_t, const float* qsample_coef_host, const float* ref_noise, uint64_t ref_seed,
                   float* x_out);

int cd_pix_refine(cd_handle h, int net, int sched_kind, float* x, int B, int R,
                  const cd_step_coef* coef_host, const float* noise, uint64_t seed);

int cd_op_pack_conv_weight(cd_handle h, const float* w_host, int N, int Cin, int KH, int KW, int geglu,
                           void** packed_dev, int* Npad, int* Cpad);
int cd_op_free(cd_handle h, void* dev);
int cd_op_conv2d(cd_handle h, const float* x0, int C0, const float* x1, int C1, int B, int H, int W,
                 const void* packed_w, int N, int KH, int KW, int stride, int pad, int asym_pad, int up,
                 const float* bias, const float* rowvec, const float* resid, int act, int tile, float* y);
int cd_op_conv2d_16(cd_handle h, const float* x0, int C0, const float* x1, int C1, int B, int H, int W,
                    const void* packed_w, int N, int KH, int KW, int stride, int pad, int asym_pad, int up,
                    const float* bias, const float* rowvec, const float* resid, int act, int tile, float* y,
                    float* stats);
int cd_op_last_gemm_config(cd_handle h, int* tile_id, int* bk, int* splitk, int* chm, int* tile_group);
int cd_op_up_phase_reorder(cd_handle h, const float* x, int B, int C, int H, int W, float* y);
int cd_op_groupnorm(cd_handle h, const float* x, int B, int C, int H, int W, int G, float eps,
                    const float* gamma, const float* beta, const float* film, int silu, float* y);
int cd_op_groupnorm_ex(cd_handle h, const float* x0, int C0, int pad0, const float* x1, int C1, int pad1, int B, int H,
                       int W, float eps, const float* gamma, const float* beta, const float* film, int film_ld, int silu,
                       const float* stats0, const float* stats1, int precision, void* y);
int cd_op_pack_conv_weight_prec(cd_handle h, const float* w_host, int N, int Cin, int KH, int KW, int geglu,
                                void** packed_dev);
int cd_op_conv2d_prec(cd_handle h, const float* x0, int C0, int pad0, const float* x1, int C1, int pad1, int B, int H, int W,
                      const void* packed_w, int N, int KH, int KW, int stride, int pad, int asym_pad, int up,
                      const float* bias, const float* rowvec, int rowvec_shared, const float* resid, int resid_pad, int act,
                      int raw_geglu, int tile, int precision, int via_split_rows, float alpha, float* y, float* stats);
int cd_op_attention_prec(cd_handle h, const float* q, const float* k, const float* v, int B, int H, int Tq, int Tk, int D,
                         int padq, int padk, int padv, float scale, int q_log2, const float* obias, int mode, int precision,
                         void* o);
int cd_op_rows_prec(cd_handle h, int op, const float* x0, int64_t rows, int C0, int pad0, const float* x1, int C1, int pad1,
                    const float* gamma, const float* beta, int precision, void* y);
int cd_op_resample_prec(cd_handle h, int op, const float* x, int B, int C, int H, int W, int precision, void* y);
int cd_op_layernorm(cd_handle h, const float* x, int rows, int C, const float* gamma, const float* beta,
                    float eps, float* y);
int cd_op_attention(cd_handle h, const float* q, const float* k, const float* v, int B, int H, int Tq,
                    int Tk, int D, float scale, int use_transpose_kernel, float* o);
int cd_op_cross_attention_ctrl(cd_handle h, const float* q_own, const float* q_src, const float* k_own, const float* k_src,
                               const float* v_own, const float* mapper, const float* alpha, const float* weight, int B,
                               int B_src, int B_ctrl, int H, int Tq, int L, int L_buf, int D, float scale, float* o);
int cd_op_lowpass(cd_handle h, const float* x, int B, int C, int R, int down_n, float* y);
int cd_op_softmax_rows(cd_handle h, const float* s, int64_t rows, int cols, float* p);
int cd_op_timestep_embedding(cd_handle h, const float* t, int B, int dim, int mode, float* out);
int cd_op_sched_step(cd_handle h, int mode, int sched_kind, const cd_step_coef* coef_host, const float* x0,
                     float* xt, const float* eps_hat, int cfg, float guidance, const float* noise,
                     const float* eps_in, int is_last, int B, int C, int HW, float* z_slot);
int cd_op_sched_step_masked(cd_handle h, int mode, const cd_step_coef* coef_host, float* x, const float* eps_hat, int cfg,
                            float guidance, const float* eps_in, const float* mask, const float* src, int B_mask,
                            int mask_source, float qa, float qb, const float* mask_noise, int blend, int B, int C, int HW,
                            void* xin16_out, int cfg_dup);
int cd_op_bench_conv(cd_handle h, int B, int H, int W, int C0, int C1, int N, int k, int stride, int up,
                     int act, int tile, int iters, float* ms_out);
int cd_op_bench_mfma_sustained(cd_handle h, int target_ms, float* tflops_out, float* ghz_out);
int cd_op_probe(cd_handle h, int which, const void* in, void* out, size_t n);

#ifdef __cplusplus
}
#endif
#endif
```

Measured before the change: 3.565 images/s.

## Fold GroupNorm into proj_in and fuse q|k|v with transposed V output

At the 320-channel, high-resolution spatial transformer entry, GroupNorm is now computed only as per-image coefficients and applied inside the streaming proj_in GEMM's A-operand load. This removes the separate normalised-activation write and read. The self-attention q/k/v projection is also merged into one streaming GEMM that writes q|k normally and V directly in transposed layout, replacing a separate V^T GEMM pass. Both paths are gated by shape checks and env switches, and the change adds LDS use and new kernel template variants.

Result: no change. 3.588 images/s, median of 6 (+0.6%).

```diff
diff --git a/cycle-diffusion_amd/_ffi.py b/cycle-diffusion_amd/_ffi.py
--- a/cycle-diffusion_amd/_ffi.py
+++ b/cycle-diffusion_amd/_ffi.py
@@ -90,6 +90,10 @@
     "cd_op_attention_prec": [_VP, _VP, _VP, _VP, _I, _I, _I, _I, _I, _I, _I, _I, _F, _I, _VP, _I, _I, _VP],
     "cd_op_rows_prec": [_VP, _I, _VP, _I64, _I, _I, _VP, _I, _I, _VP, _VP, _I, _VP],
     "cd_op_resample_prec": [_VP, _I, _VP, _I, _I, _I, _I, _I, _VP],
+    "cd_op_st_entry_mode": [_I, C.POINTER(_I)],
+    "cd_op_st_entry_available": [_I, _I, _I, _I, _I, _I, _I, C.POINTER(_I)],
+    "cd_op_gn_proj_16": [_VP, _VP, _I, _I, _I, _F, _VP, _VP, _VP, _VP, _I, _VP, _I, _VP, _VP],
+    "cd_op_qkv_vt_16": [_VP, _VP, _I, _I, _I, _VP, _VP, _VP, _I, _VP, _VP],
     "cd_op_layernorm": [_VP, _VP, _I, _I, _VP, _VP, _F, _VP],
     "cd_op_attention": [_VP, _VP, _VP, _VP, _I, _I, _I, _I, _I, _F, _I, _VP],
     "cd_op_cross_attention_ctrl": [_VP, _VP, _VP, _VP, _VP, _VP, _VP, _VP, _VP, _I, _I, _I, _I, _I, _I, _I, _I, _F, _VP],
diff --git a/cycle-diffusion_amd/csrc/capi.hip b/cycle-diffusion_amd/csrc/capi.hip
--- a/cycle-diffusion_amd/csrc/capi.hip
+++ b/cycle-diffusion_amd/csrc/capi.hip
@@ -1197,6 +1197,92 @@
   CD_API_END
 }
 
+int cd_op_st_entry_mode(int mode, int* previous) {
+  CD_API_BEGIN
+  const int prev = st_entry_override(mode);
+  if (previous) *previous = prev;
+  CD_API_END
+}
+
+int cd_op_st_entry_available(int part, int precision, int C, int N, int B, int H, int W, int* available) {
+  CD_API_BEGIN
+  CD_CHECK((part == 0 || part == 1) && available && B > 0 && H > 0 && W > 0 && C > 0 && N > 0, "bad argument");
+  Ctx c; c.f32 = precision != CD_PREC_16;
+  ConvW w; w.N = N; w.Cin = C; w.Cpad = round_up(C, 32); w.Npad = round_up(N, 128);
+  bf16_t dummy = 0;
+  if (!c.f32 && w.Cpad == 320) w.wfrag = &dummy;
+  Act x; x.B = B; x.H = H; x.W = W; x.C = C; x.ld = C; x.f32 = c.f32;
+  *available = (part == 0 ? conv_gn_fold_available(c, w, x) : conv_vt_fuse_available(c, w, x)) ? 1 : 0;
+  CD_API_END
+}
+
+int cd_op_gn_proj_16(cd_handle h, const float* x, int B, int H, int W, float eps, const float* gamma, const float* beta,
+                     const float* stats_in, const void* packed_w, int N, const float* bias, int fold, float* y,
+                     float* stats_out) {
+  CD_API_BEGIN
+  enter_engine(h);
+  CD_CHECK(h && x && gamma && beta && packed_w && y && B > 0 && H > 0 && W > 0, "bad argument");
+  ArenaScope arena_scope(h->arena);
+  Ctx c = h->ctx();
+  const int C = 320, HW = H * W;
+  ConvW w = *(const ConvW*)packed_w;
+  CD_CHECK(w.N == N && w.KH == 1 && w.KW == 1 && w.Cpad == C, "packed weight does not match the call");
+  w.b = const_cast<float*>(bias);
+  Act a = alloc_act(c, B, H, W, C);
+  launch_nchw_to_nhwc(h->st, x, a.p, B, C, HW, C, 1.f, 0.f, 0);
+  a.stats = const_cast<float*>(stats_in);
+  GNW g; g.g = const_cast<float*>(gamma); g.b = const_cast<float*>(beta); g.C = C; g.eps = eps;
+  ConvOpts o; o.pad = 0; o.tile = kLinStreamTile; o.want_stats = stats_out != nullptr;
+  Act out;
+  if (fold) {
+    CD_CHECK(st_entry_shape_ok(0, false, w.wfrag != nullptr, 1, 1, w.Cpad, w.N, a.rows(), HW, a.ld),
+             "GroupNorm fold: H * W must be a multiple of 256 and the layer a K = 320 streaming shape");
+    o.gn_coef = groupnorm_coef_fwd(c, g, a);
+    out = conv_fwd(c, w, a, nullptr, o);
+  } else {
+    Act n = groupnorm_fwd(c, g, a, nullptr, false);
+    out = conv_fwd(c, w, n, nullptr, o);
+  }
+  launch_nhwc_to_nchw(h->st, out.p, 0, out.ld, y, B, N, HW, 1.f, 0.f);
+  if (stats_out) {
+    CD_CHECK(out.stats, "no statistics from this launch");
+    HIP_CHECK(hipMemcpyAsync(stats_out, out.stats, (size_t)(out.rows() / 32) * 2 * N * sizeof(float), hipMemcpyDeviceToDevice,
+                             h->st));
+  }
+  CD_API_END
+}
+
+int cd_op_qkv_vt_16(cd_handle h, const float* x, int B, int H, int W, const void* w_qkv, const void* w_qk, const void* w_v,
+                    int fused, float* qk, void* vt16) {
+  CD_API_BEGIN
+  enter_engine(h);
+  CD_CHECK(h && x && qk && vt16 && B > 0 && H > 0 && W > 0 && (fused ? w_qkv != nullptr : (w_qk && w_v)), "bad argument");
+  ArenaScope arena_scope(h->arena);
+  Ctx c = h->ctx();
+  const int C = 320, T = H * W;
+  Act a = alloc_act(c, B, H, W, C);
+  launch_nchw_to_nhwc(h->st, x, a.p, B, C, T, C, 1.f, 0.f, 0);
+  bf16_t* vt = (bf16_t*)c.arena->alloc((size_t)B * C * T * 2);
+  Act out;
+  if (fused) {
+    const ConvW& w = *(const ConvW*)w_qkv;
+    CD_CHECK(!w.b && st_entry_shape_ok(1, false, w.wfrag != nullptr, w.KH, w.KW, w.Cpad, w.N, a.rows(), T, a.ld),
+             "fused q | k | v^T: a [960][320] weight and H * W a multiple of 256");
+    ConvOpts o; o.pad = 0; o.vt_out = vt;
+    out = conv_fwd(c, w, a, nullptr, o);
+  } else {
+    const ConvW& wqk = *(const ConvW*)w_qk;
+    const ConvW& wv = *(const ConvW*)w_v;
+    CD_CHECK(wqk.N == 2 * C && wv.N == C && wqk.Cpad == C && wv.Cpad == C && T % 64 == 0, "q | k and v weights of 320 channels");
+    ConvOpts o; o.pad = 0; o.tile = kLinStreamTile;
+    out = conv_fwd(c, wqk, a, nullptr, o);
+    vt_gemm_fwd(c, wv, a.p, a.ld, B, T, T, vt);
+  }
+  launch_nhwc_to_nchw(h->st, out.p, 0, out.ld, qk, B, 2 * C, T, 1.f, 0.f);
+  HIP_CHECK(hipMemcpyAsync(vt16, vt, (size_t)B * C * T * 2, hipMemcpyDeviceToDevice, h->st));
+  CD_API_END
+}
+
 int cd_op_layernorm(cd_handle h, const float* x, int rows, int C, const float* gamma, const float* beta,
                     float eps, float* y) {
   CD_API_BEGIN
diff --git a/cycle-diffusion_amd/csrc/engine.h b/cycle-diffusion_amd/csrc/engine.h
--- a/cycle-diffusion_amd/csrc/engine.h
+++ b/cycle-diffusion_amd/csrc/engine.h
@@ -131,6 +131,8 @@
   int out_ld = 0;
   bool ln_fold = false;
   float ln_eps = 1e-5f;
+  const float* gn_coef = nullptr;
+  bf16_t* vt_out = nullptr;
   bool raw_geglu = false;
   bool want_stats = false;
   float* out_stats = nullptr;
@@ -148,6 +150,12 @@
 struct GNW { float* g = nullptr; float* b = nullptr; int C = 0; float eps = 1e-5f; };
 Act groupnorm_fwd(Ctx& c, const GNW& w, const Act& x, const Act* x2, bool silu, const float* film = nullptr,
                   int film_ld = 0);
+const float* groupnorm_coef_fwd(Ctx& c, const GNW& w, const Act& x);
+bool conv_gn_fold_available(const Ctx& c, const ConvW& w, const Act& x);
+bool conv_vt_fuse_available(const Ctx& c, const ConvW& w, const Act& x);
+bool st_entry_shape_ok(int part, bool f32, bool has_wfrag, int KH, int KW, int Cpad, int N, int64_t rows, int HW, int ld);
+int st_entry_override(int mode);
+void vt_gemm_fwd(Ctx& c, const ConvW& wv, const bf16_t* x, int ldx, int B, int T, int Tpad, bf16_t* vt);
 struct LNW { float* g = nullptr; float* b = nullptr; int C = 0; };
 Act layernorm_fwd(Ctx& c, const LNW& w, const Act& x);
 
diff --git a/cycle-diffusion_amd/csrc/engine.hip b/cycle-diffusion_amd/csrc/engine.hip
--- a/cycle-diffusion_amd/csrc/engine.hip
+++ b/cycle-diffusion_amd/csrc/engine.hip
@@ -1,4 +1,6 @@
 #include <stdlib.h>
+
+#include <atomic>
 
 #include "engine.h"
 
@@ -314,8 +316,30 @@
   return y;
 }
 
+static Act conv_vt_fwd(Ctx& c, const ConvW& w, const Act& x, const ConvOpts& o) {
+  CD_CHECK(!c.f32 && !x.split && w.N % 3 == 0 && !w.b && !o.resid && !o.out && !o.ln_fold && !o.gn_coef && o.act == ACT_NONE,
+           "conv: transposed V columns on a layer that is no plain q | k | v projection");
+  ConvGemmParams p;
+  p.src0 = x.p; p.C0 = w.Cpad; p.ld0 = x.ld;
+  p.B = x.B; p.Hs = x.H; p.Ws = x.W; p.Hin = x.H; p.Win = x.W; p.Hout = x.H; p.Wout = x.W;
+  p.M = x.B * x.H * x.W;
+  p.wgt = w.w; p.wgt_frag = w.wfrag; p.Ktot = w.Ktot(); p.N = w.N;
+  const int Nqk = w.N / 3 * 2;
+  Act y; y.B = x.B; y.H = x.H; y.W = x.W; y.C = Nqk; y.ld = Nqk; y.f32 = false;
+  y.p = (bf16_t*)c.arena->alloc((size_t)p.M * Nqk * 2);
+  p.out = y.p; p.out_ld = y.ld;
+  p.vt_out = o.vt_out; p.vt_cols = w.N / 3; p.vt_T = x.H * x.W;
+  p.zeros = c.zeros; p.tile = kLinStreamTile;
+  launch_conv_gemm(c.st, p);
+  return y;
+}
+
 Act conv_fwd(Ctx& c, const ConvW& w, const Act& x, const Act* x2, const ConvOpts& o) {
   if (conv_up_phase_taken(c, w, x, x2, o)) return conv_up_phase_fwd(c, w, x, o);
+  if (o.vt_out) {
+    CD_CHECK(!x2, "conv: transposed V columns with a concat source");
+    return conv_vt_fwd(c, w, x, o);
+  }
   if (x.split) {
     CD_CHECK(!x2, "conv: a split activation cannot be concatenated");
     return conv_split_fwd(c, w, x, o);
@@ -361,6 +385,10 @@
   p.out = y.p; p.out_ld = y.ld; p.out_f32 = o.out_f32 ? 1 : 0;
   p.zeros = c.zeros; p.tile = o.tile;
   if (o.ln_fold) { p.ln_fold = 1; p.ln_eps = o.ln_eps; p.tile = kLinStreamTile; }
+  if (o.gn_coef) {
+    CD_CHECK(!c.f32 && !x2 && !o.vt_out, "conv: GroupNorm fold operands");
+    p.gn_coef = o.gn_coef; p.gn_T = x.H * x.W; p.tile = kLinStreamTile;
+  }
   if (c.f32) {
     p.out_f32 = 1;
     launch_conv_gemm_f32(c.st, p);
@@ -377,11 +405,70 @@
   return y;
 }
 
+static int64_t stream_min_rows() {
+  static const int64_t min_rows = [] { const char* e = getenv("CYCLEDIFF_LN_FOLD_MIN_ROWS"); return e ? atoll(e) : 32768ll; }();
+  return min_rows;
+}
+
+static std::atomic<int> g_st_entry_override{-1};
+int st_entry_override(int mode) { return g_st_entry_override.exchange(mode < 0 ? -1 : (mode & 3)); }
+
+bool st_entry_shape_ok(int part, bool f32, bool has_wfrag, int KH, int KW, int Cpad, int N, int64_t rows, int HW, int ld) {
+  if (f32 || !has_wfrag || KH != 1 || KW != 1 || Cpad != 320 || ld != 320 || HW <= 0 || HW % 256 != 0 || rows % HW != 0) return false;
+  if (rows * 320 * 2 >= (1ll << 31)) return false;
+  if (part == 0) return N % 64 == 0 && N >= 320 && N <= 2560;
+  return N == 3 * 320;
+}
+
+static bool st_entry_on(int part, int64_t rows) {
+  static const bool on[2] = {[] { const char* e = getenv("CYCLEDIFF_GN_PROJ_FOLD"); return !(e && e[0] == '0'); }(),
+                             [] { const char* e = getenv("CYCLEDIFF_QKV_VT"); return !(e && e[0] == '0'); }()};
+  const int ov = g_st_entry_override.load(std::memory_order_relaxed);
+  if (ov >= 0) return (ov >> part) & 1;
+  return on[part] && rows >= stream_min_rows();
+}
+
+bool conv_gn_fold_available(const Ctx& c, const ConvW& w, const Act& x) {
+  return !x.split && !x.f32 && st_entry_shape_ok(0, c.f32, w.wfrag != nullptr, w.KH, w.KW, w.Cpad, w.N, x.rows(), x.H * x.W, x.ld) &&
+         st_entry_on(0, x.rows());
+}
+bool conv_vt_fuse_available(const Ctx& c, const ConvW& w, const Act& x) {
+  return !x.split && !x.f32 && !w.b && st_entry_shape_ok(1, c.f32, w.wfrag != nullptr, w.KH, w.KW, w.Cpad, w.N, x.rows(), x.H * x.W, x.ld) &&
+         st_entry_on(1, x.rows());
+}
+
+void vt_gemm_fwd(Ctx& c, const ConvW& wv, const bf16_t* x, int ldx, int B, int T, int Tpad, bf16_t* vt) {
+  ConvGemmParams p;
+  p.src0 = wv.w; p.C0 = wv.Cpad; p.ld0 = wv.Cpad;
+  p.B = 1; p.Hs = wv.N; p.Ws = 1; p.Hin = wv.N; p.Win = 1; p.Hout = wv.N; p.Wout = 1;
+  p.M = wv.N;
+  p.wgt = x; p.Ktot = wv.Cpad; p.N = T;
+  CD_CHECK(ldx == wv.Cpad, "vt_gemm: token row stride %d must equal K %d", ldx, wv.Cpad);
+  p.nbatch = B; p.a_bs = 0; p.w_bs = (int64_t)T * ldx; p.o_bs = (int64_t)wv.N * Tpad;
+  p.out = vt; p.out_ld = Tpad; p.zeros = c.zeros;
+  launch_conv_gemm(c.st, p);
+}
+
 bool conv_ln_fold_available(const Ctx& c, const ConvW& w, int64_t rows) {
   static const bool on = [] { const char* e = getenv("CYCLEDIFF_LN_FOLD"); return !(e && e[0] == '0'); }();
-  static const int64_t min_rows = [] { const char* e = getenv("CYCLEDIFF_LN_FOLD_MIN_ROWS"); return e ? atoll(e) : 32768ll; }();
+  const int64_t min_rows = stream_min_rows();
   return on && !c.f32 && w.wfrag && w.KH == 1 && w.KW == 1 && w.Cpad == 320 && rows >= min_rows && rows % 32 == 0 &&
          w.N % 64 == 0 && w.N <= 2560;
+}
+
+const float* groupnorm_coef_fwd(Ctx& c, const GNW& w, const Act& x) {
+  CD_CHECK(!c.f32 && !x.f32 && !x.split && x.C == w.C, "groupnorm coefficients: 16-bit path, channels %d against %d", x.C, w.C);
+  GroupNormParams p;
+  p.x = x.p; p.C0 = x.C; p.ld0 = x.ld;
+  p.B = x.B; p.HW = x.H * x.W; p.G = 32; p.eps = w.eps; p.gamma = w.g; p.beta = w.b;
+  p.S = groupnorm_slabs(p.B, p.HW, x.C);
+  const size_t part_floats = round_up((size_t)p.B * p.S * p.G * 2, (size_t)64);
+  CD_CHECK(part_floats + (size_t)p.B * 2 * x.C <= c.gn_partial_floats, "groupnorm: workspace too small");
+  p.partial = c.gn_partial;
+  p.coef = c.gn_partial + part_floats;
+  if (x.stats && x.ld == x.C) p.pre0 = x.stats;
+  launch_groupnorm(c.st, p, false);
+  return p.coef;
 }
 
 Act groupnorm_fwd(Ctx& c, const GNW& w, const Act& x, const Act* x2, bool silu, const float* film,
diff --git a/cycle-diffusion_amd/csrc/kernels.h b/cycle-diffusion_amd/csrc/kernels.h
--- a/cycle-diffusion_amd/csrc/kernels.h
+++ b/cycle-diffusion_amd/csrc/kernels.h
@@ -129,6 +129,10 @@
   const bf16_t* zeros = nullptr;
   int ln_fold = 0;
   float ln_eps = 1e-5f;
+  const float* gn_coef = nullptr;
+  int gn_T = 0;
+  bf16_t* vt_out = nullptr;
+  int vt_cols = 0, vt_T = 0;
   int tile = 0;
   float prof_flop_scale = 1.f;
   int splitk = 0;
@@ -176,6 +180,8 @@
   int M = 0, N = 0;
   float ln_eps = 1e-5f;
   int geglu_direct = 0;
+  const float* gn_coef = nullptr; int gn_T = 0;
+  bf16_t* vt = nullptr; int vt_col0 = 0, vt_T = 0;
 };
 constexpr int kLinStreamTile = 30;
 bool lin_stream_supports(const ConvGemmParams& p);
@@ -231,7 +237,7 @@
   const float* pre1 = nullptr;
 };
 int groupnorm_slabs(int B, int HW, int C);
-void launch_groupnorm(hipStream_t st, const GroupNormParams& p);
+void launch_groupnorm(hipStream_t st, const GroupNormParams& p, bool apply = true);
 
 void launch_layernorm(hipStream_t st, const bf16_t* x, int ldx, bf16_t* y, int ldy, int rows,
                       int C, const float* gamma, const float* beta, float eps);
diff --git a/cycle-diffusion_amd/csrc/lin_stream.hip b/cycle-diffusion_amd/csrc/lin_stream.hip
--- a/cycle-diffusion_amd/csrc/lin_stream.hip
+++ b/cycle-diffusion_amd/csrc/lin_stream.hip
@@ -19,7 +19,9 @@
 constexpr int BIAS_MAX = 2560;
 constexpr int OFF_A = WSLOTS * WPIECE, OFF_ST = OFF_A + ASLOTS * APIECE, OFF_BIAS = OFF_ST + 8 * ST_BYTES;
 constexpr int LDS_BYTES = OFF_BIAS + BIAS_MAX * 4;
-static_assert(LDS_BYTES <= 160 * 1024, "LDS");
+constexpr int OFF_COEF = LDS_BYTES, COEF_BYTES = 2 * K * 4, COEF_SLOT = 3 * 1024;
+constexpr int LDS_BYTES_GNA = OFF_COEF + 2 * COEF_SLOT;
+static_assert(LDS_BYTES_GNA <= 160 * 1024, "LDS");
 constexpr unsigned kNoLoad = 0x80000000u;
 constexpr int kGegluDirectDefault = 1;
 
@@ -69,11 +71,12 @@
   asm volatile("" : "+v"(a), "+v"(b), "+v"(c), "+v"(d)::"memory");
 }
 
-template <int ACT, bool RESID, bool STATS, bool LNF = false>
+template <int ACT, bool RESID, bool STATS, bool LNF = false, bool GNA = false, bool VT = false>
 __global__ __launch_bounds__(512, 2) void k_lin_stream(LinStreamParams p) {
 #if defined(__HIP_DEVICE_COMPILE__)
   constexpr bool GEGLU = (ACT == ACT_GEGLU);
   static_assert(!(GEGLU && (RESID || STATS)), "GEGLU has neither residual nor statistics");
+  static_assert(!(GNA && (LNF || GEGLU || RESID || VT)) && !(VT && (GEGLU || RESID || STATS)), "GNA / VT variants");
   extern __shared__ __attribute__((aligned(16))) char smem[];
   char* wring = smem;
   char* aring = smem + OFF_A;
@@ -99,6 +102,10 @@
       __builtin_amdgcn_make_buffer_rsrc((void*)p.wfrag, 0, (unsigned)((size_t)p.N * K * 2), 0x00020000);
   const __amdgpu_buffer_rsrc_t rs_o = __builtin_amdgcn_make_buffer_rsrc(
       (void*)p.out, 0, (unsigned)((size_t)p.M * p.ldo * 2), 0x00020000);
+  const __amdgpu_buffer_rsrc_t rs_vt = __builtin_amdgcn_make_buffer_rsrc(
+      (void*)p.vt, 0, VT ? (unsigned)((size_t)p.M * (p.N - p.vt_col0) * 2) : 0u, 0x00020000);
+  const __amdgpu_buffer_rsrc_t rs_c = __builtin_amdgcn_make_buffer_rsrc(
+      (void*)p.gn_coef, 0, GNA ? (unsigned)((size_t)(p.M / (GNA ? p.gn_T : 1)) * COEF_BYTES) : 0u, 0x00020000);
   u32x4 rs_r = {0u, 0u, 0u, 0x00020000u};
   if (RESID) {
     const uint64_t ra = (uint64_t)p.resid;
@@ -158,6 +165,35 @@
 #pragma unroll
       for (int e = 0; e < 8; ++e) f[e] = __builtin_fmaf(f[e], rstd, nmr);
       af[ks] = __builtin_bit_cast(bf16x8, pack8_sat(f));
+      __builtin_amdgcn_sched_barrier(0);
+    }
+  };
+  auto issue_coef = [&](int row0, int slot) {
+    const int img = row0 / p.gn_T;
+#pragma unroll
+    for (int u = 0; u < 3; ++u) {
+      const unsigned voff = u * 1024 + lane * 16 < COEF_BYTES ? (unsigned)(lane * 16) : kNoLoad;
+      __builtin_amdgcn_raw_ptr_buffer_load_lds(rs_c, (lptr_t)(smem + OFF_COEF + slot * COEF_SLOT + u * 1024), 16, voff,
+                                               img * COEF_BYTES + u * 1024, 0, 0);
+    }
+  };
+  auto gn_apply_rows = [&](int slot) __attribute__((always_inline)) {
+    int l2 = lane;
+    asm volatile("" : "+v"(l2));
+    const float* tab = (const float*)(smem + OFF_COEF + slot * COEF_SLOT) + 8 * (l2 >> 5);
+#pragma unroll
+    for (int ks = 0; ks < NKS; ++ks) {
+      float f[8];
+      unpack8(__builtin_bit_cast(uint4, af[ks]), f);
+      const f32x4 a0 = *(const f32x4*)(tab + 16 * ks), a1 = *(const f32x4*)(tab + 16 * ks + 4);
+      const f32x4 b0 = *(const f32x4*)(tab + K + 16 * ks), b1 = *(const f32x4*)(tab + K + 16 * ks + 4);
+#pragma unroll
+      for (int e = 0; e < 4; ++e) {
+        f[e] = f[e] * a0[e] + b0[e];
+        f[4 + e] = f[4 + e] * a1[e] + b1[e];
+      }
+            af[ks] = __builtin_bit_cast(bf16x8, pack8(f));
+      asm volatile("" : "+v"(af[ks]));
       __builtin_amdgcn_sched_barrier(0);
     }
   };
@@ -219,6 +255,8 @@
     cn_o += wrap ? 1 : 0;
   };
 
+  if (GNA && wave == 0) { issue_coef((int)blockIdx.x * 256, 0); seq += 3; }
+  const int cmark = seq;
   if (w_issuer) {
     issue_w(0, true, 0); seq += 5; wm0 = seq;
     issue_w(1, true, 1); seq += 5; wm1 = seq;
@@ -233,9 +271,14 @@
     a_step_issue(gi);
     if (due) take_a(ce_j, ce_slot);
   }
+  if (GNA) {
+    if (wave == 0) wait_vmcnt_le(seq - cmark);
+    asm volatile("s_waitcnt lgkmcnt(0)\n\ts_barrier" ::: "memory");
+  }
 #pragma unroll
   for (int ks = 0; ks < NKS; ++ks) af[ks] = afn[ks];
   if (LNF) normalise_rows();
+  if (GNA) gn_apply_rows(0);
 
   f32x16 acc[2];
   u32x4 rres[4];
@@ -279,6 +322,7 @@
           issue_w(nxt < I ? nxt : nxt - I, nxt < I || has_next, slot2);
           seq += 5;
           wm0 = wm1; wm1 = seq;
+                    if (GNA && wave == 0 && has_next && i == 0) { issue_coef(row0 + G * 256, (ord + 1) & 1); seq += 3; }
         }
         if (due) a_consume_step();
         a_step_issue(gi);
@@ -323,7 +367,36 @@
       asm volatile("" : "+v"(l2));
       const int prow = l2 >> 2, pcol = (l2 & 3) * 8, mi2 = l2 & 31, half2 = l2 >> 5;
       const unsigned o_lane = (unsigned)(((wave * 32 + prow) * p.ldo + pcol) * 2);
-      if (GEGLU && p.geglu_direct) {
+      if (VT && t * 64 >= p.vt_col0) {
+        const int img = row0 / p.vt_T;
+        const int tok0 = row0 - img * p.vt_T + wave * 32;
+        const unsigned v_lane = (unsigned)((prow * p.vt_T + pcol) * 2);
+#pragma unroll
+        for (int nb = 0; nb < 2; ++nb) {
+          const int c0 = img * (p.N - p.vt_col0) + t * 64 - p.vt_col0 + nb * 32;
+          __builtin_amdgcn_wave_barrier();
+#pragma unroll
+          for (int q = 0; q < 4; ++q) {
+            const f32x4 bv = *(const f32x4*)(bias_s + t * 64 + nb * 32 + 8 * q + 4 * half2);
+#pragma unroll
+            for (int j = 0; j < 4; ++j) stage[(8 * q + 4 * half2 + j) * ST_LD + mi2] = acc[nb][4 * q + j] + bv[j];
+          }
+          asm volatile("s_waitcnt lgkmcnt(0)" ::: "memory");
+          __builtin_amdgcn_wave_barrier();
+#pragma unroll
+          for (int ps = 0; ps < 2; ++ps) {
+            const float* srow = stage + (prow + 16 * ps) * ST_LD + pcol;
+            const f32x4 lo = *(const f32x4*)srow, hi = *(const f32x4*)(srow + 4);
+            const float v[8] = {lo[0], lo[1], lo[2], lo[3], hi[0], hi[1], hi[2], hi[3]};
+            if (rows_ok) {
+              const uint4 o = pack8_sat(v);
+              __builtin_amdgcn_raw_buffer_store_b128(__builtin_bit_cast(u32x4, o), rs_vt, v_lane,
+                                                     ((c0 + 16 * ps) * p.vt_T + tok0) * 2, 0);
+            }
+            __builtin_amdgcn_sched_barrier(0);
+          }
+        }
+      } else if (GEGLU && p.geglu_direct) {
         const unsigned od_lane = (unsigned)(((wave * 32 + mi2) * p.ldo + 4 * half2) * 2);
 #pragma unroll
         for (int q = 0; q < 4; ++q) {
@@ -416,6 +489,7 @@
 #pragma unroll
       for (int ks = 0; ks < NKS; ++ks) af[ks] = afn[ks];
       if (LNF) normalise_rows();
+      if (GNA) gn_apply_rows((ord + 1) & 1);
     }
   }
   asm volatile("s_waitcnt vmcnt(0)" ::: "memory");
@@ -447,14 +521,15 @@
   if (lane == 0) bias_out[n] = (bias ? bias[n] : 0.f) + acc;
 }
 
-template <int ACT, bool RESID, bool STATS, bool LNF = false>
+template <int ACT, bool RESID, bool STATS, bool LNF = false, bool GNA = false, bool VT = false>
 void launch_variant(hipStream_t st, const LinStreamParams& p, int grid) {
   static PerDeviceOnce attr_once;
-  auto kern = k_lin_stream<ACT, RESID, STATS, LNF>;
+  auto kern = k_lin_stream<ACT, RESID, STATS, LNF, GNA, VT>;
+  constexpr int lds = GNA ? LDS_BYTES_GNA : LDS_BYTES;
   attr_once([&]() {
-    HIP_CHECK(hipFuncSetAttribute((const void*)kern, hipFuncAttributeMaxDynamicSharedMemorySize, LDS_BYTES));
+    HIP_CHECK(hipFuncSetAttribute((const void*)kern, hipFuncAttributeMaxDynamicSharedMemorySize, lds));
   });
-  hipLaunchKernelGGL(kern, dim3(grid), dim3(512), LDS_BYTES, st, p);
+  hipLaunchKernelGGL(kern, dim3(grid), dim3(512), lds, st, p);
 }
 
 }
@@ -472,6 +547,14 @@
   if ((int64_t)p.M * p.ld0 * 2 >= (1ll << 31) || (int64_t)p.M * p.out_ld * 2 >= (1ll << 31)) return false;
   if (p.resid && (int64_t)p.M * p.resid_ld * 2 >= (1ll << 31)) return false;
   (void)nout;
+  if (p.gn_coef) {
+    if (p.gn_T <= 0 || p.gn_T % 256 != 0 || p.M % p.gn_T != 0 || p.act != ACT_NONE || p.resid || p.ln_fold || p.vt_out) return false;
+  }
+  if (p.vt_out) {
+    if (p.vt_T <= 0 || p.vt_T % 256 != 0 || p.M % p.vt_T != 0 || p.act != ACT_NONE || p.resid || p.stats || p.ln_fold) return false;
+    if (p.vt_cols <= 0 || p.vt_cols % 64 != 0 || p.vt_cols >= p.N) return false;
+    if ((int64_t)p.M * p.vt_cols * 2 >= (1ll << 31)) return false;
+  }
   return true;
 }
 
@@ -496,6 +579,17 @@
   const int grid = nstrips < ncu ? nstrips : ncu;
   static const int geglu_direct = [] { const char* e = getenv("CYCLEDIFF_GEGLU_DIRECT"); return e && e[0] ? atoi(e) : kGegluDirectDefault; }();
   p.geglu_direct = geglu_direct;
+  if (c.gn_coef) {
+    p.gn_coef = c.gn_coef; p.gn_T = c.gn_T;
+    if (c.stats) launch_variant<ACT_NONE, false, true, false, true>(st, p, grid);
+    else launch_variant<ACT_NONE, false, false, false, true>(st, p, grid);
+    return;
+  }
+  if (c.vt_out) {
+    p.vt = c.vt_out; p.vt_col0 = c.N - c.vt_cols; p.vt_T = c.vt_T;
+    launch_variant<ACT_NONE, false, false, false, false, true>(st, p, grid);
+    return;
+  }
   if (c.ln_fold) {
     p.ln_eps = c.ln_eps;
     CD_CHECK(!c.resid && !c.stats, "lin_stream: a LayerNorm-folded layer has neither residual nor statistics");
diff --git a/cycle-diffusion_amd/csrc/norm.hip b/cycle-diffusion_amd/csrc/norm.hip
--- a/cycle-diffusion_amd/csrc/norm.hip
+++ b/cycle-diffusion_amd/csrc/norm.hip
@@ -308,7 +308,7 @@
   return S;
 }
 
-void launch_groupnorm(hipStream_t st, const GroupNormParams& p) {
+void launch_groupnorm(hipStream_t st, const GroupNormParams& p, bool apply) {
   const int C = p.C0 + p.C1;
   CD_CHECK(C % 8 == 0 && C % p.G == 0 && p.G <= 64, "groupnorm: C=%d G=%d unsupported", C, p.G);
   CD_CHECK(p.C0 % 8 == 0, "groupnorm: concat split must be a multiple of 8");
@@ -328,6 +328,7 @@
     hipLaunchKernelGGL(k_gn_stats, dim3(p.S, p.B), dim3(256), lds, st, p, rows_per_slab);
     hipLaunchKernelGGL(k_gn_coef, dim3(p.B), dim3(256), 0, st, p);
   }
+  if (!apply) return;
   int rows_per_block = (int)(((int64_t)p.HW * p.B + 2047) / 2048);
   const int unit = 4 * rif;
   rows_per_block = ceil_div(rows_per_block, unit) * unit;
diff --git a/cycle-diffusion_amd/csrc/unet_openai.hip b/cycle-diffusion_amd/csrc/unet_openai.hip
--- a/cycle-diffusion_amd/csrc/unet_openai.hip
+++ b/cycle-diffusion_amd/csrc/unet_openai.hip
@@ -21,7 +21,7 @@
   GNW norm;
   ConvW *proj_in = nullptr, *proj_out = nullptr;
   LNW ln1, ln2, ln3;
-  ConvW *qkv1 = nullptr, *qk1 = nullptr, *v1 = nullptr, *o1 = nullptr;
+  ConvW *qkv1 = nullptr, *qk1 = nullptr, *v1 = nullptr, *qkv1_vt = nullptr, *o1 = nullptr;
   ConvW *q2 = nullptr, *k2 = nullptr, *v2 = nullptr, *o2 = nullptr;
   ConvW *ff1 = nullptr, *ff2 = nullptr;
   ConvW *q2_ln = nullptr, *ff1_ln = nullptr;
@@ -134,6 +134,12 @@
     params.conv_rows(tb + ".attn1.to_q.weight", {C, C}, s.qk1, 0, C, 0, C, 0, qscale);
     params.conv_rows(tb + ".attn1.to_k.weight", {C, C}, s.qk1, C, C, 0, C, 0);
     s.v1 = make_conv(params, tb + ".attn1.to_v", C, C, 1, false, false, 2);
+    if (s.qk1->wfrag) {
+      s.qkv1_vt = params.new_conv(3 * C, C, 1, 1, false);
+      params.conv_rows(tb + ".attn1.to_q.weight", {C, C}, s.qkv1_vt, 0, C, 0, C, 0, qscale);
+      params.conv_rows(tb + ".attn1.to_k.weight", {C, C}, s.qkv1_vt, C, C, 0, C, 0);
+      params.conv_rows(tb + ".attn1.to_v.weight", {C, C}, s.qkv1_vt, 2 * C, C, 0, C, 0);
+    }
   } else {
     s.qkv1 = params.new_conv(3 * C, C, 1, 1, false);
     params.conv_rows(tb + ".attn1.to_q.weight", {C, C}, s.qkv1, 0, C, 0, C, 0, qscale);
@@ -332,15 +338,7 @@
 }
 
 static void vt_gemm(Ctx& c, const ConvW& wv, const bf16_t* x, int ldx, int B, int T, int Tpad, bf16_t* vt) {
-  ConvGemmParams p;
-  p.src0 = wv.w; p.C0 = wv.Cpad; p.ld0 = wv.Cpad;
-  p.B = 1; p.Hs = wv.N; p.Ws = 1; p.Hin = wv.N; p.Win = 1; p.Hout = wv.N; p.Wout = 1;
-  p.M = wv.N;
-  p.wgt = x; p.Ktot = wv.Cpad; p.N = T;
-  CD_CHECK(ldx == wv.Cpad, "vt_gemm: token row stride %d must equal K %d", ldx, wv.Cpad);
-  p.nbatch = B; p.a_bs = 0; p.w_bs = (int64_t)T * ldx; p.o_bs = (int64_t)wv.N * Tpad;
-  p.out = vt; p.out_ld = Tpad; p.zeros = c.zeros;
-  launch_conv_gemm(c.st, p);
+  vt_gemm_fwd(c, wv, x, ldx, B, T, Tpad, vt);
 }
 
 void UNetOpenAI::set_context(Ctx& c, const bf16_t* ctx, int B, int L) {
@@ -505,13 +503,25 @@
   const float scale = 1.0f / sqrtf((float)s.dh);
   const bf16_t* k2c = s.k2c + (int64_t)b0 * ctx_L_ * C;
   const bf16_t* v2c = s.v2c + (int64_t)b0 * ctx_L_ * C;
-  Act n = groupnorm_fwd(c, s.norm, x_in, nullptr, false);
-  Act h = conv_fwd(c, *s.proj_in, n, nullptr, p0);
+  Act h;
+  if (conv_gn_fold_available(c, *s.proj_in, x_in)) {
+    ConvOpts pg; pg.pad = 0; pg.gn_coef = groupnorm_coef_fwd(c, s.norm, x_in);
+    h = conv_fwd(c, *s.proj_in, x_in, nullptr, pg);
+  } else {
+    Act n = groupnorm_fwd(c, s.norm, x_in, nullptr, false);
+    h = conv_fwd(c, *s.proj_in, n, nullptr, p0);
+  }
   {
     const size_t m2 = c.arena->mark();
     Act n1 = layernorm_fwd(c, s.ln1, h);
     Act a;
-    if (s.qkv1) {
+    if (s.qkv1_vt && conv_vt_fuse_available(c, *s.qkv1_vt, n1)) {
+      bf16_t* vt = (bf16_t*)c.arena->alloc((size_t)B * C * T * 2);
+      ConvOpts pv; pv.pad = 0; pv.vt_out = vt;
+      Act qk = conv_fwd(c, *s.qkv1_vt, n1, nullptr, pv);
+      a = attention_vt_fwd(c, qk.p, qk.ld, qk.p + C, qk.ld, vt, B, s.heads, T, T, T, s.dh, scale, x.H, x.W,
+                           true);
+    } else if (s.qkv1) {
       Act qkv = conv_fwd(c, *s.qkv1, n1, nullptr, p0);
       a = attention_fwd(c, qkv.p, qkv.ld, qkv.p + C, qkv.ld, qkv.p + 2 * C, qkv.ld, B, s.heads, T, T, s.dh, scale,
                         x.H, x.W, true);
diff --git a/include/cyclediff.h b/include/cyclediff.h
--- a/include/cyclediff.h
+++ b/include/cyclediff.h
@@ -153,6 +153,13 @@
 int cd_op_rows_prec(cd_handle h, int op, const float* x0, int64_t rows, int C0, int pad0, const float* x1, int C1, int pad1,
                     const float* gamma, const float* beta, int precision, void* y);
 int cd_op_resample_prec(cd_handle h, int op, const float* x, int B, int C, int H, int W, int precision, void* y);
+int cd_op_st_entry_mode(int mode, int* previous);
+int cd_op_st_entry_available(int part, int precision, int C, int N, int B, int H, int W, int* available);
+int cd_op_gn_proj_16(cd_handle h, const float* x, int B, int H, int W, float eps, const float* gamma, const float* beta,
+                     const float* stats_in, const void* packed_w, int N, const float* bias, int fold, float* y,
+                     float* stats_out);
+int cd_op_qkv_vt_16(cd_handle h, const float* x, int B, int H, int W, const void* w_qkv, const void* w_qk, const void* w_v,
+                    int fused, float* qk, void* vt16);
 int cd_op_layernorm(cd_handle h, const float* x, int rows, int C, const float* gamma, const float* beta,
                     float eps, float* y);
 int cd_op_attention(cd_handle h, const float* q, const float* k, const float* v, int B, int H, int Tq,
```
